# wcy199705/DfFintheWild

Hardware: AMD Instinct MI355X
Metric: focal-stacks/sec (10x3x256x256) (higher is better)
Workload: dtype bf16x3 (split-bf16 MFMA operands hi+lo, fp32 accumulate, fp32-accurate); 1 GPU; DFF_net forward, 10-slice 3x256x256 focal stacks, batch 32 per GPU (BASELINE.json config 3), dense focus_dists, synthetic weights seed 0; batch_per_gpu=32, global_batch=32, slices=10, height=256, width=256, parallelism=single GPU, precision=bf16x3, input=float32 (B,3,N,H,W), the reference's tensor contract

## Files before the change

dffinthewild_amd/csrc/dffw_device.h:

```cpp
#pragma once
#include <hip/hip_runtime.h>
#include <stdint.h>

#include <utility>

#include "dffw_internal.h"

namespace dffw {

template <class F, int... I>
__device__ __forceinline__ void static_for_impl(F &&f, std::integer_sequence<int, I...>) {
    (f(std::integral_constant<int, I>{}), ...);
}
template <int N, class F>
__device__ __forceinline__ void static_for(F &&f) {
    static_for_impl(f, std::make_integer_sequence<int, N>{});
}

typedef __attribute__((ext_vector_type(8))) short short8;
typedef __attribute__((ext_vector_type(4))) short short4v;
typedef __attribute__((ext_vector_type(8))) __bf16 bf16x8;
typedef __attribute__((ext_vector_type(8))) _Float16 f16x8;
typedef __attribute__((ext_vector_type(4))) float f32x4;

// ... 227 lines not shown
        if (a.res0) wide_add(a.res0, pre0);
        if (a.res1) wide_add(a.res1, pre1);
        if (a.relu == 1) {
#pragma unroll
            for (int i = 0; i < 4; ++i) v[i] = relu_bits(v[i]);
        }
        if (a.cls_w && cvalid) {
#pragma unroll
            for (int i = 0; i < 4; ++i) cls_partial = fmaf(a.cls_w[c0 + i], v[i], cls_partial);
        }
        if (a.out) wide_store(a.out);
    } else {
        const bool ok = pvalid && cvalid;
        const int64_t eo = FAST ? (int64_t)(voff + nt * 16) : opix * Cout + c0;
        auto store4 = [&](uint16_t *base_) {
            uint16_t *base = FAST ? base_ + ubase : base_;
            uint32_t h01, h23, l01, l23;
            Fmt<PREC>::split2(v[0], v[1], h01, l01);
            Fmt<PREC>::split2(v[2], v[3], h23, l23);
            if (ok) *reinterpret_cast<uint2 *>(base + eo) = make_uint2(h01, h23);
        };
        auto add4 = [&](const uint16_t *base_, uint4 q) {
            const uint16_t *base = FAST ? base_ + (a.res_bcast ? rbase : ubase) : base_;
            int64_t ro = eo;
            if (a.res_bcast) {
                if constexpr (FAST) ro = (int64_t)(rvoff + nt * 16);
                else {
                    const int64_t hw = (int64_t)a.Ho * a.Wo;
                    ro = ((opix / a.outf_plane) * hw + opix % hw) * Cout + c0;
                }
            }
            if constexpr (!PRE) {
                q = make_uint4(0, 0, 0, 0);
                if (ok) {
                    const uint2 h = *reinterpret_cast<const uint2 *>(base + ro);
                    q.x = h.x;
                    q.y = h.y;
                }
            }
            float r0, r1, r2, r3;
            Fmt<PREC>::join2(q.x, 0, r0, r1);
            Fmt<PREC>::join2(q.y, 0, r2, r3);
            v[0] += r0;
            v[1] += r1;
            v[2] += r2;
            v[3] += r3;
        };
        if (a.out_pre) store4(a.out_pre);
        if (a.relu == 2) {
#pragma unroll
            for (int i = 0; i < 4; ++i) v[i] = relu_bits(v[i]);
        }
        if (a.res0) add4(a.res0, pre0);
        if (a.res1) add4(a.res1, pre1);
        if (a.relu == 1) {
#pragma unroll
            for (int i = 0; i < 4; ++i) v[i] = relu_bits(v[i]);
        }
        if (a.cls_w && cvalid) {
#pragma unroll
            for (int i = 0; i < 4; ++i) cls_partial = fmaf(a.cls_w[c0 + i], v[i], cls_partial);
        }
        if (a.out) store4(a.out);
    }
}

__device__ __forceinline__ void dffw_store16(char *p, uint4 v) { *reinterpret_cast<uint4 *>(p) = v; }

template <int PREC, bool RES, bool CLS = false>
__device__ __forceinline__ float epilogue_lean(uint16_t *__restrict__ out, uint16_t *__restrict__ out_pre, int voff, const f32x4 &acc, uint4 rq,
                                               bool relu, const f32x4 &clsw) {
    static_assert(Fmt<PREC>::PARTS == 2, "split-bf16 storage only");
    float v0 = acc[0], v1 = acc[1], v2 = acc[2], v3 = acc[3];
    auto store = [&](uint16_t *base) {
        uint32_t h01, h23, l01, l23;
        Fmt<PREC>::split2(v0, v1, h01, l01);
        Fmt<PREC>::split2(v2, v3, h23, l23);
        swap16(h01, l01);
        swap16(h23, l23);
        dffw_store16(reinterpret_cast<char *>(base) + (uint32_t)(voff * 2), make_uint4(h01, h23, l01, l23));
    };
    if (out_pre) store(out_pre);
    if constexpr (RES) {
        swap16(rq.x, rq.z);
        swap16(rq.y, rq.w);
        float r0, r1, r2, r3;
        Fmt<PREC>::join2(rq.x, rq.z, r0, r1);
        Fmt<PREC>::join2(rq.y, rq.w, r2, r3);
        v0 += r0;
        v1 += r1;
        v2 += r2;
        v3 += r3;
    }
    if (relu) {
        v0 = relu_bits(v0);
        v1 = relu_bits(v1);
        v2 = relu_bits(v2);
        v3 = relu_bits(v3);
    }
    float cls = 0.f;
    if constexpr (CLS) {
        cls = fmaf(clsw[0], v0, cls);
        cls = fmaf(clsw[1], v1, cls);
        cls = fmaf(clsw[2], v2, cls);
        cls = fmaf(clsw[3], v3, cls);
    }
    if (out) store(out);
    return cls;
}

template <int PREC>
__device__ __forceinline__ void epilogue_lean_t(uint16_t *__restrict__ out, uint16_t *__restrict__ out_pre, int voff, float v0, float v1, float v2,
                                                float v3, bool has_res, uint4 rq, bool relu, bool has_cls, const f32x4 &clsw, float &cls, bool pv) {
    static_assert(Fmt<PREC>::PARTS == 2, "split-bf16 storage only");
    auto store = [&](uint16_t *base) {
        uint32_t h01, h23, l01, l23;
        Fmt<PREC>::split2(v0, v1, h01, l01);
        Fmt<PREC>::split2(v2, v3, h23, l23);
        swap16(h01, l01);
        swap16(h23, l23);
        if (pv) dffw_store16(reinterpret_cast<char *>(base) + (uint32_t)(voff * 2), make_uint4(h01, h23, l01, l23));
    };
    if (out_pre) store(out_pre);
    if (has_res) {
        swap16(rq.x, rq.z);
        swap16(rq.y, rq.w);
        float r0, r1, r2, r3;
        Fmt<PREC>::join2(rq.x, rq.z, r0, r1);
        Fmt<PREC>::join2(rq.y, rq.w, r2, r3);
        v0 += r0;
        v1 += r1;
        v2 += r2;
        v3 += r3;
    }
    if (relu) {
        v0 = relu_bits(v0);
        v1 = relu_bits(v1);
        v2 = relu_bits(v2);
        v3 = relu_bits(v3);
    }
    if (has_cls) {
        cls = fmaf(clsw[0], v0, cls);
        cls = fmaf(clsw[1], v1, cls);
        cls = fmaf(clsw[2], v2, cls);
        cls = fmaf(clsw[3], v3, cls);
    }
    if (out) store(out);
}

__device__ __forceinline__ void epilogue_cls(const ConvArgs &a, float partial, int g, int64_t opix, bool pvalid, int rows = 4) {
    if (!a.cls_w) return;
    partial += __shfl_xor(partial, 16);
    if (rows == 4) partial += __shfl_xor(partial, 32);
    if ((g & (rows - 1)) == 0 && pvalid) a.cls_out[opix] = partial;
}

__device__ __forceinline__ float softplus_fast(float v) {
    const float L2E = 1.44269502162933349609375f, L2E_LO = 1.925963033500414e-08f, LN2 = 0.693147182464599609375f;
    const float hi = v * L2E;
    const float lo = __builtin_fmaf(v, L2E, -hi) + v * L2E_LO;
    float e = __builtin_amdgcn_exp2f(hi);
    e = __builtin_fmaf(e, lo * LN2, e);
    const float w = 1.f + e, d = w - 1.f;
    const float r = (__builtin_amdgcn_logf(w) * LN2) * (e * __builtin_amdgcn_rcpf(d));
    const float sp = d == 0.f ? e : r;
    return v > 20.f ? v : sp;
}

__device__ __forceinline__ float sigmoid_fast(float v) {
    const float L2E = 1.44269502162933349609375f, L2E_LO = 1.925963033500414e-08f, LN2 = 0.693147182464599609375f;
    const float hi = v * L2E;
    const float lo = __builtin_fmaf(v, L2E, -hi) + v * L2E_LO;
    float e = __builtin_amdgcn_exp2f(hi);
    e = __builtin_fmaf(e, lo * LN2, e);
    return v > 20.f ? 1.f : e * __builtin_amdgcn_rcpf(1.f + e);
}

struct WarpPoint {
    float fx, fy, sx, sy;
};
__device__ __forceinline__ WarpPoint warp_point(int xx, int yy, int H, int W, float f, float a1, float a2) {
    const float stepx = 2.0f / (float)(W > 1 ? W - 1 : 1), stepy = 2.0f / (float)(H > 1 ? H - 1 : 1);
    const float lx = xx < W / 2 ? -1.0f + (float)xx * stepx : 1.0f - (float)(W - 1 - xx) * stepx;
    const float ly = yy < H / 2 ? -1.0f + (float)yy * stepy : 1.0f - (float)(H - 1 - yy) * stepy;
    WarpPoint p;
    p.fx = (float)(W / 2) * (f - 1.0f) * lx + a1;
    p.fy = (float)(H / 2) * (f - 1.0f) * ly + a2;
    const float gx = 2.0f * ((float)xx - p.fx) / (float)(W > 1 ? W - 1 : 1) - 1.0f;
    const float gy = 2.0f * ((float)yy - p.fy) / (float)(H > 1 ? H - 1 : 1) - 1.0f;
    p.sx = ((gx + 1.0f) * 0.5f) * (float)(W - 1);
    p.sy = ((gy + 1.0f) * 0.5f) * (float)(H - 1);
    return p;
}


struct SimWarpPoint {
    float sx, sy;
};
__device__ __forceinline__ SimWarpPoint sim_warp_point(int xx, int yy, int H, int W, float fm1, float beta, float gamma) {
#pragma clang fp contract(off)
    const float stepx = 2.0f / (float)(W - 1), stepy = 2.0f / (float)(H - 1);
    const float lx = xx < W / 2 ? fmaf(stepx, (float)xx, -1.0f) : fmaf(-stepx, (float)(W - 1 - xx), 1.0f);
    const float ly = yy < H / 2 ? fmaf(stepy, (float)yy, -1.0f) : fmaf(-stepy, (float)(H - 1 - yy), 1.0f);
    const float g2x = (float)(W / 2) * (fm1 * lx) - beta;
    const float g2y = (float)(H / 2) * (fm1 * ly) - gamma;
    const float gx = 2.0f * ((float)xx - g2x) / (float)(W - 1) - 1.0f;
    const float gy = 2.0f * ((float)yy - g2y) / (float)(H - 1) - 1.0f;
    SimWarpPoint p;
    p.sx = (gx + 1.0f) * ((float)(W - 1) / 2.0f);
    p.sy = (gy + 1.0f) * ((float)(H - 1) / 2.0f);
    return p;
}


template <int PREC>
__device__ __forceinline__ void warp_octet(const uint16_t *__restrict__ slice, int C, int H, int W, const WarpPoint &wp, float (&v)[8]) {
    constexpr int PARTS = Fmt<PREC>::PARTS;
    const float x0f = floorf(wp.sx), y0f = floorf(wp.sy);
    const int x0 = (int)x0f, y0 = (int)y0f;
    const float wx1 = wp.sx - x0f, wy1 = wp.sy - y0f;
    const float wx[2] = {1.0f - wx1, wx1}, wy[2] = {1.0f - wy1, wy1};
#pragma unroll
    for (int dy = 0; dy < 2; ++dy) {
        const int yc = y0 + dy;
        if (yc < 0 || yc >= H) continue;
#pragma unroll
        for (int dx = 0; dx < 2; ++dx) {
            const int xc = x0 + dx;
            if (xc < 0 || xc >= W) continue;
            const uint16_t *rec = slice + ((int64_t)yc * W + xc) * (PARTS * C);
            const uint4 h = *reinterpret_cast<const uint4 *>(rec);
            uint4 l = make_uint4(0, 0, 0, 0);
            if constexpr (PARTS == 2) l = *reinterpret_cast<const uint4 *>(rec + C);
            const float wgt = wx[dx] * wy[dy];
            float a, c;
            Fmt<PREC>::join2(h.x, l.x, a, c); v[0] += a * wgt; v[1] += c * wgt;
            Fmt<PREC>::join2(h.y, l.y, a, c); v[2] += a * wgt; v[3] += c * wgt;
            Fmt<PREC>::join2(h.z, l.z, a, c); v[4] += a * wgt; v[5] += c * wgt;
            Fmt<PREC>::join2(h.w, l.w, a, c); v[6] += a * wgt; v[7] += c * wgt;
        }
    }
}

}
```

dffinthewild_amd/csrc/dffw_dispatch.cpp:

```cpp
#include "dffw_run.h"
#include "dffw_stem.h"

namespace dffw {
namespace {

struct ConvLaunch {
    char kernel[96];
    const char *suffix;
    ConvArgs a;
    RollArgs r;
    int v0, v1;
    double flops, bytes;
};

enum { F_TILE = 100, F_GATHER = 101 };

struct ConvPlan {
    int family = -1;
    int n = 0;
    ConvLaunch l[4];
    bool clear_scores = false;
    const TileCfg *cfg = nullptr;
    TileArgs t;
    bool stem_pipe = false;
    int64_t partial_bytes = 0;
    int64_t M_out = 0;
    double finish_bytes = 0;
    int err = DFFW_OK;
    char msg[192];
};

struct Cols {
    int tiles_y, tiles_x;
    int64_t n;
    bool whole;
};

struct Planner;
struct StreamFamily {
    bool (Planner::*plan)(ConvPlan &p) const;
    void (*name)(int prec, const ConvLaunch &l, char *buf, int n);
    hipError_t (*go)(int prec, const ConvLaunch &l, hipStream_t s);
    bool step_trace;
};
extern const StreamFamily kStream[];
constexpr int kStreamBeforeStemPair = 5, kStreamCount = 10;

struct Planner {
    const std::string &name;
    const PackedConv &pc;
    const LayerDef &L;
    const Act &in0;
    const ConvOpt &o;
    const Switches &sw;
    const int prec;
    const Act &out;
    ConvArgs a;
    const int No, Ho, Wo, cin_pad;
    const double eb, opx, in_b;
    int fam = 0;

    double out_b(int k) const { return opx * L.cout * eb * k; }
    double w_b(double taps) const { return taps * L.cin * L.cout * eb; }
    double cls_b() const { return o.cls ? opx * 4.0 : 0.0; }
    double sums_b() const { return opx / 16.0 * 3.0 * L.cout * 4.0; }
    double mac(double points, double taps) const { return 2.0 * points * taps * L.cin * L.cout; }
    int res(const Act *r) const { return r ? 1 : 0; }

    Cols columns(bool in_grid, int ty, int tx) const {
        const int H = in_grid ? in0.H : Ho, W = in_grid ? in0.W : Wo;
        Cols g;
        g.tiles_y = (H + ty - 1) / ty;
        g.tiles_x = (W + tx - 1) / tx;
        g.n = (int64_t)g.tiles_y * g.tiles_x;
        g.whole = H % ty == 0 && W % tx == 0;
        return g;
    }
    ConvArgs on_grid(bool in_grid) const {
        ConvArgs g = a;
        g.Ng = in_grid ? in0.N : No;
        g.Hg = in_grid ? in0.H : Ho;
        g.Wg = in_grid ? in0.W : Wo;
        g.M = (int64_t)g.B * g.Ng * g.Hg * g.Wg;
        return g;
    }
    static ConvArgs masked(ConvArgs g) {
        g.dbg &= (6 | DFFW_ARGS_NO_LEAN_TILE | DFFW_ARGS_NO_LEAN_ROLL | DFFW_ARGS_NO_ROLLX | DFFW_ARGS_NO_ROLLK | DFFW_ARGS_NO_SLICE32);
        return g;
    }
    int zsplit(int64_t units, int64_t below) const {
        int z = (units < below && No >= 8) ? 2 : 1;
        if (sw.roll_zsplit >= 1 && sw.roll_zsplit <= No) z = sw.roll_zsplit;
        return z;
    }
    void add(ConvPlan &p, const ConvArgs &g, const uint16_t *filter, const Cols &c, int zs, int pair, double flops, double bytes,
             const char *suffix = "", int v0 = 0, int v1 = 0) const {
        p.family = fam;
        ConvLaunch &l = p.l[p.n++];
        l.a = g;
        l.r = roll_args(filter, in0.B, c.tiles_y, c.tiles_x, zs, sw.roll_wgs, pair);
        l.suffix = suffix;
        l.v0 = v0;
        l.v1 = v1;
        l.flops = flops;
        l.bytes = bytes;
        kStream[fam].name(prec, l, l.kernel, sizeof l.kernel);
    }

    bool rollt(ConvPlan &p) const {
        if (!(pc.wrollt && !o.in1 && !sw.on(SW_NO_ROLL) && !sw.on(SW_NO_ROLLT))) return false;
        int ty, tx;
        rollt_tile(L.cout, &ty, &tx);
        const Cols c = columns(true, ty, tx);
        const ConvArgs g = on_grid(true);
        const int64_t units = (int64_t)in0.B * c.n * std::max(1, L.cout / 32);
        const bool four = cin_pad == 32 && L.cout != 16;
        if (!(units >= (int64_t)sw.rollt_min_units * (four ? 3 : 2) / 2 && rollt_ok(prec, g))) return false;
        p.clear_scores = g.cls_w != nullptr;
        add(p, g, pc.wrollt, c, 1, 0, mac((double)g.M, 27.0),
            in_b + out_b((o.discard ? 0 : 1) + (o.out_pre ? 1 : 0) + res(o.res0)) + cls_b() + w_b(27.0));
        return true;
    }
    bool roll_t32(ConvPlan &p) const {
        if (!(pc.wroll_t32 && (in0.C == 32 || in0.C == 16) && !o.in1 && !o.res_bcast && !o.res1 && !o.outf && in0.H % 8 == 0 && in0.W % 16 == 0 &&
              (int64_t)in0.B * (in0.H / 8) * (in0.W / 16) >= sw.roll_min_units && !sw.on(SW_NO_ROLL)))
            return false;
        const ConvArgs g = masked(on_grid(true));
        for (int py = 0; py < 2; ++py) {
            int ty, tx;
            roll_t32_tile(py, &ty, &tx);
            const Cols c = columns(true, ty, tx);
            add(p, g, pc.wroll_t32 + (size_t)(py ? ROLL_CHUNKS_T32_0 : 0) * prec_parts(prec) * 512, c, 1, 0, mac((double)g.M, py ? 18.0 : 9.0),
                in_b + 0.5 * out_b((o.discard ? 0 : 1) + (o.out_pre ? 1 : 0) + res(o.res0)) + 0.5 * cls_b(), py ? " (odd rows)" : " (even rows)", py);
        }
        return true;
    }
    bool roll_s2(ConvPlan &p) const {
        if (!(pc.wroll_s2 && !L.transposed && L.sh == 2 && (in0.C == 16 || in0.C == 32) && !o.in1 && !o.res1 && !o.res_bcast && !o.outf && !o.out_pre &&
              !o.cls && !sw.on(SW_NO_ROLL) && !sw.on(SW_NO_ROLL_S2) &&
              (L.cout <= 32 || !sw.on(SW_NO_ROLL_S2_WIDE))))
            return false;
        const int khn = in0.C / 16;
        const int ntk = (khn == 2 || L.cout >= 32) ? 2 : 1;
        const int nlaunch = (L.cout / 16 + ntk - 1) / ntk;
        int ty, tx;
        s2_roll_tile(ntk, &ty, &tx);
        const Cols c = columns(false, ty, tx);
        if (!((L.cout / 16) % ntk == 0 && c.whole && in0.H == 2 * Ho && in0.W == 2 * Wo && (int64_t)in0.B * c.n >= sw.roll_min_units)) return false;
        const ConvArgs g = masked(on_grid(false));
        for (int li = 0; li < nlaunch; ++li)
            add(p, g, pc.wroll_s2, c, 1, li * ntk, mac(opx, 27.0) / nlaunch, in_b + out_b(1 + res(o.res0)) / nlaunch + w_b(27.0) / nlaunch,
                nlaunch > 1 ? (li ? " (upper output channels)" : " (lower output channels)") : "", ntk, khn);
        return true;
    }
    bool roll_efd(ConvPlan &p) const {
        int ty, tx;
        efd_roll_tile(&ty, &tx);
        const Cols c = columns(false, ty, tx);
        if (!(pc.wroll8 && !L.transposed && L.sh == 2 && in0.C == 8 && !o.in1 && !o.res0 && !o.res1 && !o.res_bcast && !o.outf && !o.out_pre &&
              !o.cls && c.whole && (int64_t)in0.B * c.n >= sw.roll_min_units && !sw.on(SW_NO_ROLL) && !sw.on(SW_NO_ROLL_S2)))
            return false;
        add(p, masked(on_grid(false)), pc.wroll8, c, 1, 0, mac(opx, 27.0), in_b + out_b(1) + w_b(27.0));
        return true;
    }
    bool roll_t(ConvPlan &p) const {
        int ty, tx;
        roll_tile(&ty, &tx);
        const Cols c = columns(true, ty, tx);
        if (!(pc.wroll_t && c.whole && in0.C == 16 && !o.in1 && !o.res_bcast && !o.res1 && !o.outf &&
              (int64_t)in0.B * c.n >= sw.roll_min_units && !sw.on(SW_NO_ROLL)))
            return false;
        const ConvArgs g = on_grid(true);
        add(p, g, pc.wroll_t, c, zsplit((int64_t)in0.B * c.n, 1024), 1, mac((double)g.M, 27.0),
            in_b + out_b((o.discard ? 0 : 1) + (o.out_pre ? 1 : 0)) + out_b(res(o.res0)) + cls_b() + w_b(27.0));
        return true;
    }
    bool rollx_k2(ConvPlan &p) const {
        const Cols c = columns(false, 8, 16);
        const bool halves = o.in1 ? (in0.C == 16 && o.in1->C == 16) : in0.C == 32;
        if (!(pc.wroll_k2 && halves && c.whole && (int64_t)in0.B * c.n >= sw.roll_min_units && !sw.on(SW_NO_ROLL) && !sw.on(SW_NO_ROLLX))) return false;
        const ConvArgs g = on_grid(false);
        if (!rollx_k2_ok(prec, g)) return false;
        add(p, g, pc.wroll_k2, c, zsplit((int64_t)in0.B * c.n, 512), 0, mac(opx, 27.0), in_b + out_b(1) + w_b(27.0));
        return true;
    }
    bool slice32(ConvPlan &p) const {
        if (!(pc.wslice32 && !o.in1 && !sw.on(SW_NO_ROLL) && !sw.on(SW_NO_SLICE32))) return false;
        int ty, tx;
        slice32_tile(&ty, &tx);
        const Cols c = columns(false, ty, tx);
        const ConvArgs g = on_grid(false);
        if (!(c.whole && (int64_t)in0.B * c.n >= sw.roll_min_units && slice32_ok(prec, g))) return false;
        add(p, g, pc.wslice32, c, 1, 0, mac(opx, 9.0), in_b + (o.sums ? sums_b() : out_b(1 + res(o.res0))) + w_b(9.0));
        return true;
    }
    bool slice64(ConvPlan &p) const {
        if (!(pc.wslice64 && (pc.slice_cat ? (o.in1 && o.in1->C == 32) : !o.in1) && !sw.on(SW_NO_ROLL) && !sw.on(SW_NO_SLICE32))) return false;
        int ty, tx;
        slice32_tile(&ty, &tx);
        const Cols c = columns(false, ty, tx);
        const ConvArgs g = on_grid(false);
        if (!(c.whole && (int64_t)in0.B * c.n >= sw.roll_min_units && slice64_ok(prec, g))) return false;
        add(p, g, pc.wslice64, c, 1, 0, mac(opx, 9.0), in_b + (o.sums ? sums_b() : out_b(1)) + w_b(9.0));
        return true;
    }
    bool rollk(ConvPlan &p) const {
        if (!(pc.wrollk && !sw.on(SW_NO_ROLL) && !sw.on(SW_NO_ROLLK))) return false;
        int ty, tx;
        rollk_tile(&ty, &tx);
        const Cols c = columns(false, ty, tx);
        const ConvArgs g = on_grid(false);
        const int npair = L.cout / 32;
        const bool merged = npair == 2 && (int64_t)in0.B * c.n < sw.rollk_merge_below;
        const int64_t units = (int64_t)in0.B * c.n * (merged ? npair : 1);
        if (!(units >= sw.roll_min_units && rollk_waves(prec, g) == cin_pad / 8)) return false;
        const int nlaunch = merged ? 1 : npair;
        for (int op = 0; op < nlaunch; ++op)
            add(p, g, pc.wrollk + (size_t)op * (cin_pad / 8) * ROLLK_CHUNKS * 2 * prec_parts(prec) * 512, c, zsplit(units, cin_pad == 64 && merged ? 256 : 512),
                merged ? -1 : op * 2, mac(opx, 27.0) / nlaunch, in_b + out_b(1 + res(o.res0)) / nlaunch + w_b(27.0) / nlaunch,
                nlaunch > 1 ? (op ? " (upper output channels)" : " (lower output channels)") : "");
        return true;
    }
    bool roll(ConvPlan &p) const {
        int ty, tx;
        roll_tile(&ty, &tx);
        const Cols c = columns(false, ty, tx);
        if (!(pc.wroll && c.whole && in0.C % 8 == 0 && (!o.in1 || o.in1->C == in0.C) && !o.res_bcast && !o.res1 &&
              (int64_t)in0.B * c.n >= sw.roll_min_units && !sw.on(SW_NO_ROLL)))
            return false;
        add(p, on_grid(false), pc.wroll, c, zsplit((int64_t)in0.B * c.n, 1024), pc.roll_pair ? 1 : 0, mac(opx, 27.0),
            in_b + (o.outf ? opx * L.cout * 4.0 : out_b(o.out_pre ? 2 : 1)) + out_b(res(o.res0) + res(o.res1)) + w_b(27.0), "", pc.roll_pair);
        return true;
    }

    void tile(ConvPlan &p, const TilePack &tp, bool stem_pair, int gH, int gW);
    void gather(ConvPlan &p);
};

const StreamFamily kStream[kStreamCount] = {
    {&Planner::rollt, [](int, const ConvLaunch &l, char *b, int n) { conv_rollt_kernel_name(l.a, b, n); },
     [](int, const ConvLaunch &l, hipStream_t s) { return launch_conv_rollt(l.a, l.r, s); }, false},
    {&Planner::roll_t32, [](int prec, const ConvLaunch &l, char *b, int n) { conv_roll_t32_kernel_name(prec, l.v0, l.a, b, n); },
     [](int prec, const ConvLaunch &l, hipStream_t s) { return launch_conv_roll_t32(prec, l.v0, l.a, l.r, s); }, false},
    {&Planner::roll_s2, [](int prec, const ConvLaunch &l, char *b, int n) { conv_roll_s2_kernel_name(prec, l.v0, l.v1, l.a, b, n); },
     [](int prec, const ConvLaunch &l, hipStream_t s) { return launch_conv_roll_s2(prec, l.v0, l.v1, l.a, l.r, s); }, false},
    {&Planner::roll_efd, [](int prec, const ConvLaunch &l, char *b, int n) { conv_roll_efd_kernel_name(prec, l.a, false, b, n); },
     [](int prec, const ConvLaunch &l, hipStream_t s) { return launch_conv_roll_efd(prec, l.a, l.r, s); }, false},
    {&Planner::roll_t, [](int prec, const ConvLaunch &l, char *b, int n) { conv_roll_t_kernel_name(prec, l.a, b, n); },
     [](int prec, const ConvLaunch &l, hipStream_t s) { return launch_conv_roll_t(prec, l.a, l.r, s); }, false},
    {&Planner::rollx_k2, [](int, const ConvLaunch &l, char *b, int n) { conv_rollx_k2_kernel_name(l.a, b, n); },
     [](int, const ConvLaunch &l, hipStream_t s) { return launch_conv_rollx_k2(l.a, l.r, s); }, false},
    {&Planner::slice32, [](int, const ConvLaunch &l, char *b, int n) { conv_slice32_kernel_name(l.a, b, n); },
     [](int, const ConvLaunch &l, hipStream_t s) { return launch_conv_slice32(l.a, l.r, s); }, false},
    {&Planner::slice64, [](int, const ConvLaunch &l, char *b, int n) { conv_slice64_kernel_name(l.a, b, n); },
     [](int, const ConvLaunch &l, hipStream_t s) { return launch_conv_slice64(l.a, l.r, s); }, false},
    {&Planner::rollk, [](int, const ConvLaunch &l, char *b, int n) { conv_rollk_kernel_name(l.a, b, n); },
     [](int, const ConvLaunch &l, hipStream_t s) { return launch_conv_rollk(l.a, l.r, s); }, false},
    {&Planner::roll, [](int prec, const ConvLaunch &l, char *b, int n) { conv_roll_kernel_name(prec, l.a, l.v0 != 0, b, n); },
     [](int prec, const ConvLaunch &l, hipStream_t s) { return launch_conv_roll(prec, l.a, l.r, s); }, true},
};

void Planner::tile(ConvPlan &p, const TilePack &tp, bool stem_pair, int gH, int gW) {
    const TileCfg *cfg = tp.cfg;
    a.Ng = L.transposed ? in0.N : No;
    a.Hg = gH;
    a.Wg = gW;
    a.sy = a.sx = L.transposed ? 1 : L.sh;
    a.osy = a.osx = L.transposed ? 2 : 1;
    a.M = (int64_t)a.B * a.Ng * a.Hg * a.Wg;
    TileArgs &t = p.t;
    memset(&t, 0, sizeof t);
    t.npass = tp.npass;
    t.nstage = tp.nstage;
    double flops = 0;
    for (int ps = 0; ps < tp.npass; ++ps) {
        t.KC[ps] = tp.KC[ps];
        t.tab[ps] = tp.tab[ps];
        t.wpk[ps] = tp.wpk[ps];
        t.ooy[ps] = tp.ooy[ps];
        t.oox[ps] = tp.oox[ps];
        flops += 2.0 * (double)a.M * (L.transposed ? tp.ntaps[ps] : L.kd * L.kh * L.kw) * L.cin * L.cout;
    }
    t.nt_total = pc.nt;
    t.nsplit = pc.nt / cfg->nt;
    auto set_tiles = [&](const TileCfg *c) {
        t.tiles_z = (a.Ng + c->tz - 1) / c->tz;
        t.tiles_y = (a.Hg + c->ty - 1) / c->ty;
        t.tiles_x = (a.Wg + c->tx - 1) / c->tx;
        t.total_tiles = a.B * t.tiles_z * t.tiles_y * t.tiles_x;
        t.grid = 8 * ((t.total_tiles + 7) / 8);
        t.warm = (t.total_tiles * t.nsplit <= sw.warm_max_wgs) ? 1 : 0;
    };
    auto team_wgs = [&](const TileCfg *c, int nsplit, int npass) {
        return (int64_t)a.B * ((a.Ng + c->tz - 1) / c->tz) * ((a.Hg + c->ty - 1) / c->ty) * ((a.Wg + c->tx - 1) / c->tx) * nsplit * npass;
    };
    set_tiles(cfg);
    const int split_below = (cfg->geo == G3T && pc.nt >= 4) ? sw.split_t64 : (cfg->geo == G3S1 && pc.nt == 4) || (cfg->geo == G3S2 && pc.nt >= 8) ? sw.split_s64 : ((cfg->geo == G3S1 || cfg->geo == G3T) ? 257 : 256);
    if (t.total_tiles < split_below && pc.nt > 1 && !o.cls && !sw.on(SW_NO_SPLIT)) {
        const int want = (256 + t.total_tiles - 1) / t.total_tiles;
        for (int nts = pc.nt / 2; nts >= 1; nts /= 2) {
            const TileCfg *c2 = pc.nt % nts == 0 ? tile_cfg_find_like(tp.cfg, nts) : nullptr;
            if (!c2) continue;
            cfg = c2;
            t.nsplit = pc.nt / nts;
            if (t.nsplit >= want) break;
        }
        set_tiles(cfg);
    }
    t.ksplit = 1;
    p.M_out = (int64_t)out.B * No * Ho * Wo;
    const int thr = sw.split_wg;
    t.pass_split = (L.transposed && t.total_tiles * t.nsplit <= thr && !sw.on(SW_NO_SPLITK)) ? 1 : 0;
    if (t.pass_split && tp.nstage >= 2 && !sw.on(SW_NO_TEAMS)) {
        for (int nts = cfg->nt; nts <= pc.nt && nts <= 2; nts *= 2) {
            const TileCfg *team = pc.nt % nts == 0 ? tile_cfg_find_team(cfg, tp.nstage, nts) : nullptr;
            if (!team || team_wgs(team, pc.nt / nts, 4) > sw.team_max_wgs) continue;
            cfg = team;
            t.nsplit = pc.nt / nts;
            set_tiles(cfg);
            break;
        }
    }
    if (!t.pass_split && tile_cfg_has_splitk(cfg) && t.total_tiles * t.nsplit <= thr * 3 / 4 && tp.nstage >= 2 && !o.cls && !o.out_pre && !o.outf && !o.discard && !o.res_bcast && L.cout % 4 == 0 &&
        !sw.on(SW_NO_SPLITK)) {
        const int want = (sw.ksplit_target + t.total_tiles * t.nsplit - 1) / (t.total_tiles * t.nsplit);
        t.ksplit = std::max(1, std::min(std::min(tp.nstage, want), 8));
        const TileCfg *team = (t.ksplit > 1 && !sw.on(SW_NO_TEAMS)) ? tile_cfg_find_team(cfg, tp.nstage, cfg->nt) : nullptr;
        if (team) {
            const int64_t wgs = team_wgs(team, t.nsplit, 1);
            if (wgs < sw.team_min_wgs || wgs > sw.team_max_wgs) team = nullptr;
        }
        if (team) {
            cfg = team;
            t.ksplit = 1;
            set_tiles(cfg);
        }
        if (t.ksplit > 1) {
            t.partial_stride = p.M_out * (int64_t)pc.nt * 16;
            p.partial_bytes = t.ksplit * t.partial_stride * (int64_t)sizeof(float);
            p.finish_bytes = (double)p.M_out * L.cout * (4.0 * t.ksplit + eb * (o.res0 ? 2 : 1));
        }
    }
    p.stem_pipe = stem_pair && !sw.on(SW_NO_STEM_PIPE) && !sw.tracing(name) && stem_pipe_ok(prec, cfg, a, t);
    p.family = F_TILE;
    p.cfg = cfg;
    p.n = 1;
    ConvLaunch &l = p.l[0];
    l.a = a;
    l.suffix = "";
    l.flops = flops;
    l.bytes = in_b + (o.outf ? opx * L.cout * 4.0 : out_b(o.out_pre ? 2 : 1)) + out_b(res(o.res0) + res(o.res1)) + w_b((double)L.kd * L.kh * L.kw);
    if (p.stem_pipe) stem_pipe_kernel_name(a, l.kernel, sizeof l.kernel);
    else conv_tile_kernel_name(prec, cfg, a, t, l.kernel, sizeof l.kernel);
}

void Planner::gather(ConvPlan &p) {
    p.family = F_GATHER;
    for (const Variant &v : pc.variants) {
        a.KC = v.KC;
        a.tab = v.tab;
        a.wpk = v.wpk;
        if (L.transposed) {
            a.Ng = in0.N; a.Hg = in0.H; a.Wg = in0.W;
            a.sy = a.sx = 1;
            a.osy = a.osx = 2;
            a.ooy = v.ooy; a.oox = v.oox;
        } else {
            a.Ng = No; a.Hg = Ho; a.Wg = Wo;
            a.sy = L.sh; a.sx = L.sw;
            a.osy = a.osx = 1;
            a.ooy = a.oox = 0;
        }
        a.M = (int64_t)a.B * a.Ng * a.Hg * a.Wg;
        if (sw.on(SW_NO_SMALL)) a.dbg |= DFFW_ARGS_NO_SMALL;
        ConvLaunch &l = p.l[p.n++];
        l.a = a;
        l.suffix = "";
        conv_kernel_name_for(prec, a, l.kernel, 64);
        const double nv = (double)pc.variants.size();
        const double px = (double)a.M;
        l.flops = 2.0 * (double)a.M * v.ntaps * L.cin * L.cout;
        l.bytes = in_b / nv
                  + px * L.cout * (o.outf ? 4.0 : eb * (o.out_pre ? 2 : 1))
                  + px * L.cout * eb * (res(o.res0) + res(o.res1))
                  + (double)v.ntaps * L.cin * L.cout * eb;
    }
}

void plan_conv(const std::string &name, const PackedConv &pc, const PackedConv *cls, const Act &in0, const ConvOpt &o, const Act &out, const Switches &sw,
               int prec, ConvPlan &p) {
    const LayerDef &L = pc.def;
    const int No = out.N, Ho = out.H, Wo = out.W;
    auto reject = [&](const char *fmt, const char *x, const char *y) {
        p.err = DFFW_EINVAL;
        snprintf(p.msg, sizeof p.msg, fmt, x, y);
    };
    if (o.cls && (!cls || !cls->w32 || cls->def.cin != L.cout || cls->def.cout != 1)) return reject("cannot fuse classifier %s into %s", o.cls, name.c_str());
    if (o.res_bcast && !(L.kd == 1 && L.kh == 3 && !L.transposed && L.sh == 1 && L.cout >= 16))
        return reject("slice-broadcast residual is only implemented for the per-slice 1x3x3 convs (layer %s)%s", name.c_str(), "");

    const double eb = 2.0 * prec_parts(prec);
    Planner pl{name, pc, L, in0, o, sw, prec, out, ConvArgs(), No, Ho, Wo, pc.cin_all, eb, (double)out.B * No * Ho * Wo, (double)in0.pixels() * L.cin * eb};
    ConvArgs &a = pl.a;
    memset(&a, 0, sizeof a);
    a.in0 = in0.p;
    a.C0 = in0.C;
    a.in1 = o.in1 ? o.in1->p : in0.p;
    a.C1 = o.in1 ? o.in1->C : 0;
    a.B = in0.B; a.Ni = in0.N; a.Hi = in0.H; a.Wi = in0.W;
    a.No = No; a.Ho = Ho; a.Wo = Wo;
    a.Cout = L.cout;
    a.bias = pc.bias;
    a.res0 = o.res0 ? o.res0->p : nullptr;
    a.res1 = o.res1 ? o.res1->p : nullptr;
    a.res_bcast = o.res_bcast ? 1 : 0;
    a.out = out.p;
    a.out_pre = o.out_pre ? o.out_pre->p : nullptr;
    a.outf = o.outf;
    a.fs32 = o.fs32;
    a.outf_ch = o.outf_ch;
    a.outf_plane = (int64_t)No * Ho * Wo;
    a.cls_w = cls ? cls->w32 : nullptr;
    a.cls_out = o.cls_out;
    a.relu = o.relu;
    a.dbg = (sw.debug_flags & 6) | sw.path_bits();
    if (o.raw) a.dbg |= DFFW_ARGS_RAW;
    if (o.sums) {
        if (!conv_sums_ok(pc, sw, in0.B, in0.N, in0.H, in0.W) || o.relu != 1 || o.res0 || o.res1 || o.cls || o.out_pre || o.in1)
            return reject("layer %s has no row-sums kernel for this shape / epilogue%s", name.c_str(), "");
        a.outf = o.sums;
        a.dbg |= DFFW_ARGS_SUMS;
    }

    for (pl.fam = 0; pl.fam < kStreamBeforeStemPair; ++pl.fam)
        if ((pl.*kStream[pl.fam].plan)(p)) return;
    const bool stem_pair = o.fs32 && pc.tile_pair.cfg && pc.bias_pair && Wo % pc.tile_pair.cfg->tx == 0 && Ho % pc.tile_pair.cfg->ty == 0 &&
                           !sw.on(SW_NO_STEM_PAIR);
    if (stem_pair) a.bias = pc.bias_pair;
    for (; pl.fam < kStreamCount; ++pl.fam)
        if ((pl.*kStream[pl.fam].plan)(p)) return;

    const int gW = L.transposed ? in0.W : Wo, gH = L.transposed ? in0.H : Ho;
    const bool narrow_splits = pc.tile_narrow.cfg && pc.nt > pc.tile_narrow.cfg->nt;
    const int gN = L.transposed ? in0.N : No;
    bool narrow = !stem_pair && pc.tile_narrow.cfg && !sw.on(SW_NO_NARROW) && !(narrow_splits && (o.cls || sw.on(SW_NO_SPLIT))) &&
                  (int64_t)in0.B * ((gN + 4) / 5) * ((gH + 7) / 8) * ((gW + 7) / 8) * pc.nt >= 256;
    if (narrow && !(gW <= 8 && gH <= 8)) narrow = !L.transposed && pc.nt >= 8 && gW <= sw.narrow_max && gH <= sw.narrow_max;
    const TilePack &tp = stem_pair ? pc.tile_pair : (narrow ? pc.tile_narrow : pc.tile);
    const int64_t small_units = ((int64_t)in0.B * gN * gH * gW + 15) / 16 * pc.nt;
    const bool prefer_small = small_units <= sw.small_max_units && !o.cls && !o.fs32 && !sw.on(SW_NO_SMALL) && !stem_pair;
    const bool use_tile = tp.cfg && !sw.on(SW_NO_TILE) && gW * 2 >= tp.cfg->tx && gH * 2 >= tp.cfg->ty &&
                          in0.C % 8 == 0 && (!o.in1 || o.in1->C % 8 == 0) && !prefer_small;
    if (use_tile) pl.tile(p, tp, stem_pair, gH, gW);
    else pl.gather(p);
}

}

Act Run::conv(const std::string &name, const Act &in0, const ConvOpt &o) {
    Act out;
    if (!ok()) return out;
    auto it = e->convs.find(name);
    if (it == e->convs.end()) {
        err = fail(DFFW_EINVAL, "no packed layer %s", name.c_str());
        return out;
    }
    const PackedConv &pc = it->second;
    const LayerDef &L = pc.def;
    const int cin = in0.C + (o.in1 ? o.in1->C : 0);
    if (cin != pc.cin_all) {
        err = fail(DFFW_EINVAL, "layer %s expects %d input channels, got %d", name.c_str(), pc.cin_all, cin);
        return out;
    }
    int Ho, Wo;
    if (L.transposed) {
        Ho = in0.H * 2;
        Wo = in0.W * 2;
    } else {
        const int win = (L.kh == 9 && L.cin == 3) ? in0.W - 2 : in0.W;
        Ho = (in0.H + 2 * L.ph - L.dh * (L.kh - 1) - 1) / L.sh + 1;
        Wo = (win + 2 * L.pw - L.dw * (L.kw - 1) - 1) / L.sw + 1;
    }
    const int No = in0.N + 2 * L.pd - (L.kd - 1);
    if (o.outf == nullptr && !o.discard && !o.sums) out = act(in0.B, No, Ho, Wo, L.cout);
    else { out.B = in0.B; out.N = No; out.H = Ho; out.W = Wo; out.C = L.cout; }
    if (o.out_pre) *o.out_pre = act(in0.B, No, Ho, Wo, L.cout);
    if (!ok()) return out;

    const PackedConv *cls = nullptr;
    if (o.cls) {
        auto ic = e->convs.find(o.cls);
        if (ic != e->convs.end()) cls = &ic->second;
    }
    ConvPlan p;
    plan_conv(name, pc, cls, in0, o, out, sw, e->prec, p);
    if (p.err != DFFW_OK) {
        err = fail(p.err, "%s", p.msg);
        return out;
    }
    float *partial = p.partial_bytes ? (float *)raw(p.partial_bytes) : nullptr;
    if (!ok()) return out;
    if (dry) {
        drop_raw(partial);
        return out;
    }

    const uint16_t *zero = zero_page();
    if (!zero) return out;
    if (p.clear_scores) check(hipMemsetAsync(o.cls_out, 0, (size_t)out.pixels() * 4, s), "score memset");
    const StreamFamily *f = p.family < kStreamCount ? &kStream[p.family] : nullptr;
    const size_t trace_words = p.family == F_TILE ? (size_t)p.t.total_tiles * 8 : (f && f->step_trace) ? STEP_TRACE_WORDS : 0;
    p.t.partial = partial;
    for (int i = 0; i < p.n; ++i) {
        ConvLaunch &l = p.l[i];
        l.a.zero = zero;
        launch(l.kernel, name, l.suffix, l.flops, l.bytes, name.c_str(), trace_words, [&](unsigned long long *trace) {
            l.a.trace = trace;
            if (f) return f->go(e->prec, l, s);
            if (p.family == F_GATHER) return launch_conv(e->prec, l.a, s);
            return p.stem_pipe ? launch_stem_pipe(l.a, p.t, sw.roll_wgs, s) : launch_conv_tile(e->prec, p.cfg, l.a, p.t, s);
        });
    }
    if (partial) {
        launch_unnamed("dffw::splitk_finish_kernel", name, " (split-K finish)", 0.0, p.finish_bytes, "splitk_finish", 0, [&](unsigned long long *) {
#if defined(DFFW_ABL_BUILD) && defined(DFFW_EXP_SKIP_FINISH)
            return hipSuccess;
#endif
            return launch_splitk_finish(e->prec, partial, p.t.ksplit, p.t.partial_stride, p.M_out, pc.nt * 16, L.cout, pc.bias, p.l[0].a.res0, o.relu, out.p, s);
        });
        drop_raw(partial);
    }
    trace_end();
    return out;
}

}
```

dffinthewild_amd/csrc/dffw_engine.cpp:

```cpp
#include <algorithm>
#include <cmath>
#include <cstdarg>
#include <cstdio>
#include <cstdlib>
#include <cstring>
#include <map>
#include <memory>
#include <string>
#include <vector>

#include "dffw_run.h"
#include "dffw_srd_roll.h"
#include "dffw_stem.h"

namespace dffw {

static thread_local std::string g_err;
static thread_local std::string g_last_kernel;
static thread_local std::string g_last_op_kernels;
}
int dffw_fail(int code, const char *fmt, ...) {
    char buf[1024];
    va_list ap;
    va_start(ap, fmt);
// ... 275 lines not shown
    };
    auto args = [&](int cout, uint16_t *out) {
        ConvArgs a;
        memset(&a, 0, sizeof a);
        a.in0 = x.p; a.C0 = x.C;
        a.in1 = pooled->p; a.C1 = x.C;
        a.B = x.B; a.Ni = x.N; a.Hi = x.H; a.Wi = x.W;
        a.Ng = x.N; a.Hg = Ho; a.Wg = Wo;
        a.No = x.N; a.Ho = Ho; a.Wo = Wo;
        a.Cout = cout;
        a.bias = ca->second.bias;
        a.out = out;
        a.relu = 1;
        a.M = (int64_t)x.B * x.N * Ho * Wo;
        return a;
    };
    int ty, tx;
    efd_roll_tile(&ty, &tx);
    if (fused(8, ty, tx) && ca->second.wroll8 && cb->second.wroll8) {
        Act out = r.act(x.B, x.N, Ho, Wo, 16);
        if (r.ok() && !r.dry) {
            ConvArgs a = args(16, out.p);
            if (!(a.zero = r.zero_page())) return out;
            a.dbg = (r.sw.debug_flags & 6) | r.sw.path_bits();
            RollArgs t = roll_args(ca->second.wroll8, x.B, Ho / ty, Wo / tx, 1, r.sw.roll_wgs);
            t.wroll2 = cb->second.wroll8;
            t.bias2 = cb->second.bias;
            char kn[64];
            conv_roll_efd_kernel_name(r.e->prec, a, true, kn, sizeof kn);
            r.launch(kn, p, "", 2.0 * opx * 27.0 * 8 * 16 * 2, ((double)x.pixels() * 8 + opx * 8 + opx * 16) * r.elem_bytes(), "conv_roll_efd", 0,
                     [&](unsigned long long *) { return launch_conv_roll_efd(r.e->prec, a, t, r.s); });
        }
        r.drop(*pooled);
        return out;
    }
    efd16_tile(&ty, &tx);
    if (fused(16, ty, tx) && ca->second.wroll_s2 && cb->second.wroll15 && ca->second.def.cout == 32) {
        ConvArgs a = args(32, (uint16_t *)16);
        RollArgs t = roll_args(ca->second.wroll_s2, x.B, Ho / ty, Wo / tx, 1, r.sw.roll_wgs);
        t.wroll2 = cb->second.wroll15;
        t.bias2 = cb->second.bias;
        if (efd16_ok(r.e->prec, a, t)) {
            Act out = r.act(x.B, x.N, Ho, Wo, 32);
            if (r.ok() && !r.dry) {
                a.out = out.p;
                char kn[64];
                conv_efd16_kernel_name(kn, sizeof kn);
                r.launch(kn, p, "", 2.0 * opx * 27.0 * 16 * 32 * 2, ((double)x.pixels() * 16 + opx * 16 + opx * 32) * r.elem_bytes(), "conv_efd16", 0,
                         [&](unsigned long long *) { return launch_conv_efd16(a, t, r.s); });
            }
            r.drop(*pooled);
            return out;
        }
    }
    Act a = r.conv(p + ".stride_conv.0", x);
    Act m = (pooled && pooled->p) ? *pooled : r.pool(x, 0, 2);
    ConvOpt o; o.relu = 1; o.res0 = &a;
    Act out = r.conv(p + ".max_pooling.1.0", m, o);
    r.drop(m);
    r.drop(a);
    return out;
}

static Act pyramid_scale(Run &r, const std::string &S, const char *tag, Act &t) {
    const std::string d = S + ".dres" + tag;
    ConvOpt rl; rl.relu = 1;
    Act a = r.conv(d + "_0.0.0", t, rl);
    Act r0 = r.conv(d + "_0.2.0", a, rl);
    r.drop(a);
    Act b = r.conv(d + "_1.0.0", r0, rl);
    ConvOpt o; o.res0 = &r0;
    Act out = r.conv(d + "_1.2.0", b, o);
    r.drop(b);
    r.drop(r0);
    return out;
}

static Act pyramid(Run &r, const std::string &S, const Act &v3) {
    ConvOpt rl; rl.relu = 1;
    Act p8, p16, p32;
    if (v3.H % 8 == 0 && v3.W % 8 == 0 && !r.sw.on(SW_NO_POOL3)) {
        p8 = r.act(v3.B, v3.N, v3.H / 2, v3.W / 2, v3.C);
        p16 = r.act(v3.B, v3.N, v3.H / 4, v3.W / 4, v3.C);
        p32 = r.act(v3.B, v3.N, v3.H / 8, v3.W / 8, v3.C);
        if (r.ok() && !r.dry) {
            char kn[48];
            snprintf(kn, sizeof kn, "dffw::pool3_kernel<%d>", r.e->prec);
            r.launch_unnamed(kn, "avgpool (1,2,2)+(1,4,4)+(1,8,8)", "", 0.0, (double)(v3.pixels() + p8.pixels() + p16.pixels() + p32.pixels()) * v3.C * r.elem_bytes(), "pool3", 0,
                             [&](unsigned long long *) { return launch_pool3(r.e->prec, v3.p, p8.p, p16.p, p32.p, v3.B, v3.N, v3.H, v3.W, v3.C, r.s); });
        }
    } else {
        p8 = r.pool(v3, 1, 2);
        p16 = r.pool(v3, 1, 4);
        p32 = r.pool(v3, 1, 8);
    }
    r.forked = r.concurrent;
    r.fork(0);
    r.fork(1);
    Act s8 = pyramid_scale(r, S, "8", p8);
    r.drop(p8);
    r.on(0);
    Act s16 = pyramid_scale(r, S, "16", p16);
    r.drop(p16);
    r.on(1);
    Act s32 = pyramid_scale(r, S, "32", p32);
    r.drop(p32);
    r.on(-1);
    r.join(0);
    r.join(1);
    r.forked = false;
    r.release_deferred();
    const bool redir_side = r.concurrent && (r.sw.redir_side == 1 || (r.sw.redir_side < 0 && (int64_t)v3.B * v3.N * v3.H * v3.W * 16 >= (2 << 20)));
    r.forked = redir_side;
    if (redir_side) {
        r.fork(0);
        r.on(0);
    }
    Act rd1 = r.conv(S + ".redir1.0", s8);
    r.on(-1);
    Act d1 = r.conv(S + ".conv1", s8);
    r.drop(s8);
    ConvOpt c1 = rl; c1.in1 = &s16;
    Act m1 = r.conv(S + ".combine1.0.0", d1, c1);
    r.drop(d1); r.drop(s16);
    Act c2 = r.conv(S + ".conv2.0.0", m1, rl);
    r.drop(m1);
    if (redir_side) {
        r.fork(1);
        r.on(1);
    }
    Act rd2 = r.conv(S + ".redir2.0", c2);
    r.on(-1);
    Act d2 = r.conv(S + ".conv3", c2);
    r.drop(c2);
    ConvOpt cc2 = rl; cc2.in1 = &s32;
    Act m2 = r.conv(S + ".combine2.0.0", d2, cc2);
    r.drop(d2); r.drop(s32);
    Act c4 = r.conv(S + ".conv4.0.0", m2, rl);
    r.drop(m2);
    if (redir_side) r.join(1);
    ConvOpt u8o = rl; u8o.res0 = &rd2;
    Act u8 = r.conv(S + ".conv8.0", c4, u8o);
    r.drop(c4); r.drop(rd2);
    if (redir_side) r.join(0);
    ConvOpt u9o = rl; u9o.res0 = &rd1;
    Act u9 = r.conv(S + ".conv9.0", u8, u9o);
    r.drop(u8); r.drop(rd1);
    r.forked = false;
    r.release_deferred();
    return u9;
}

static Act hourglass(Run &r, const std::string &p, const Act &xa, const Act &xb, const Act *presqu, const Act *postsqu,
                     const Act &skip, Act *pre1_out, Act *out_raw, const std::string &cls, float *cls_out, bool discard_sum) {
    ConvOpt rl; rl.relu = 1;
    ConvOpt c0 = rl; c0.in1 = &xb;
    Act pre1 = r.conv(p + ".conv0.0.0", xa, c0);
    Act o1 = r.conv(p + ".conv1.0.0", pre1, rl);
    ConvOpt c2 = rl; c2.res0 = postsqu;
    Act pre = r.conv(p + ".conv2.0", o1, c2);
    r.drop(o1);
    Act o3 = r.conv(p + ".conv3.0.0", pre, rl);
    Act o4 = r.conv(p + ".conv4.0.0", o3, rl);
    r.drop(o3);
    ConvOpt c5 = rl; c5.res0 = presqu ? presqu : &pre;
    Act o5 = r.conv(p + ".conv5.0", o4, c5);
    r.drop(o4); r.drop(pre);
    ConvOpt c6; c6.res0 = &skip; c6.out_pre = out_raw; c6.cls = cls.c_str(); c6.cls_out = cls_out; c6.discard = discard_sum;
    Act sum = r.conv(p + ".conv6.0", o5, c6);
    r.drop(o5);
    if (pre1_out) *pre1_out = pre1; else r.drop(pre1);
    return sum;
}

struct RegressQueue {
    RegressHeads hd{};
    void *keep[4] = {nullptr, nullptr, nullptr, nullptr};
    int nkeep = 0;
    double bytes = 0.0;
};
static void regress(Run &r, RegressQueue &q, const char *tag, float *score, int B, int N, int h, int w, int H, int W, const float *fd,
                    const int64_t fst[4], float *out, bool merge) {
    if (!merge) {
        if (r.ok() && !r.dry && out)
            r.launch_unnamed("dffw::regress_kernel", tag, "", 0.0, (double)B * N * h * w * 4.0 + (double)B * H * W * 4.0, tag, 0,
                             [&](unsigned long long *) { return launch_regress(score, B, N, h, w, H, W, fd, fst[0], fst[1], fst[2], fst[3], out, r.s); });
        r.drop_raw(score);
        return;
    }
    q.keep[q.nkeep++] = score;
    if (!out || r.dry) return;
    const int k = q.hd.n++;
    q.hd.score[k] = score;
    q.hd.depth[k] = out;
    q.hd.h[k] = h;
    q.hd.w[k] = w;
    q.bytes += (double)B * N * h * w * 4.0 + (double)B * H * W * 4.0;
}
static void flush_regress(Run &r, RegressQueue &q, int B, int N, int H, int W, const float *fd, const int64_t fst[4]) {
    if (q.hd.n && r.ok() && !r.dry) {
        q.hd.nofuse = r.sw.on(SW_NO_REGRESS_FUSED) ? 1 : 0;
        const bool fused = regress_form(q.hd, B, N, H, W) != 0;
        const double bytes = q.bytes + ((fst[2] || fst[3]) ? (double)B * N * H * W * 4.0 : 0.0);
        r.launch_unnamed(fused ? "dffw::regress_fused_kernel" : "dffw::regress_kernel", "regress.mid_out+pred1+pred2+pred3", "", 0.0, bytes, "regress", 0,
                         [&](unsigned long long *) { return launch_regress_heads(q.hd, B, N, H, W, fd, fst[0], fst[1], fst[2], fst[3], r.s); });
    }
    for (int k = 0; k < q.nkeep; ++k) r.drop_raw(q.keep[k]);
    q.hd.n = 0;
    q.nkeep = 0;
}

int run_depth(Run &r, const float *FS, const float *fd, const int64_t fst[4], int B, int N, int H, int W, float *const out[4], const RawStack *raw) {
    const std::string P = "DFF_net";
    const int prec = r.e->prec;
    ConvOpt rl; rl.relu = 1;
    {
        const int64_t z = r.sw.concurrent_max_pixels;
        const int64_t px = (int64_t)B * N * H * W;
        if ((z < 0 || px < z) && px >= r.sw.concurrent_min_pixels && !r.sw.on(SW_NO_CONCURRENT) && !r.e->profiling) r.enable_concurrency();
    }

    const std::string stem_name = P + ".FM_measure.Focus_extraction.0.0";
    Act stem;
    if (r.tiled(stem_name, H, W) && !r.sw.on(SW_NO_FUSED_STEM)) {
        Act geom;
        geom.B = B; geom.N = N; geom.H = H; geom.W = W + 2; geom.C = 8;
        ConvOpt so = rl;
        so.fs32 = FS;
        RawStack *rdev = nullptr;
        if (raw) {
            rdev = (RawStack *)r.raw(256);
            if (r.ok() && !r.dry) r.check(launch_set_raw(*raw, rdev, r.s), "set_raw");
            so.fs32 = (const float *)rdev;
            so.raw = true;
        }
        stem = r.conv(stem_name, geom, so);
        r.drop_raw(rdev);
    } else {
        float *tmp = nullptr;
        if (raw) {
            tmp = (float *)r.raw((int64_t)B * 3 * N * H * W * (int64_t)sizeof(float));
            if (r.ok() && !r.dry) {
                const int64_t st[5] = {raw->sb, raw->sn, raw->sy, raw->sx, raw->sc};
                if (dffw_pack_stack(r.e->device, raw->p, raw->dtype, st, B, N, raw->h, raw->w, H, W, tmp, r.s) != DFFW_OK) r.err = DFFW_EHIP;
            }
            FS = tmp;
        }
        Act in = r.act(B, N, H, W + 2, 8);
        if (r.ok() && !r.dry) {
            char kn[48];
            snprintf(kn, sizeof kn, "dffw::stack_in_kernel<%d>", prec);
            r.launch_unnamed(kn, "stack_in", "", 0.0, (double)B * N * H * W * 3 * 4.0 + (double)B * N * H * (W + 2) * 8 * r.elem_bytes(), "stack_in", 0,
                             [&](unsigned long long *) { return launch_stack_in(prec, FS, in.p, B, N, H, W, r.s); });
        }
        stem = r.conv(stem_name, in, rl);
        r.drop(in);
        r.drop_raw(tmp);
    }
    r.tap("stem", stem);
    Act v1p, v2p;
    Act v1 = srd(r, P + ".FM_measure.Focus_extraction.2", stem, true, &v1p);
    r.tap("V1", v1);
    Act e1 = efd(r, P + ".FM_conv1.0", v1, &v1p);
    r.tap("E1", e1);
    Act v2 = srd(r, P + ".FM_conv1.1", e1, true, &v2p);
    r.tap("V2", v2);
    Act e2 = efd(r, P + ".FM_conv2.0", v2, &v2p);
    r.tap("E2", e2);
    Act v3 = srd(r, P + ".FM_conv2.1", e2, true);
    r.tap("V3", v3);

    Act vol = pyramid(r, P + ".SPP_module", v3);
    r.tap("FS_volume", vol);

    RegressQueue rq;
    const bool merge_heads = true;
    const int h8 = H / 8, w8 = W / 8;
    float *conf = (float *)r.raw((int64_t)B * N * h8 * w8 * sizeof(float));
    const bool conf_side = r.concurrent && (int64_t)B * N * H * W < (16 << 20) && !r.sw.on(SW_NO_CONF_FORK);
    r.forked = conf_side;
    if (conf_side) {
        r.fork(0);
        r.on(0);
    }
    {
        Act c = r.conv(P + ".confidence.0.0", vol, rl);
        ConvOpt of; of.outf = conf;
        r.conv(P + ".confidence.2", c, of);
        r.drop(c);
        r.tap_f32("conf", conf, (int64_t)B * N * h8 * w8);
        regress(r, rq, "regress.mid_out", conf, B, N, h8, w8, H, W, fd, fst, out[0], merge_heads);
    }
    r.on(-1);

    Act d0 = r.conv(P + ".dres0.0.0", vol, rl);
    r.drop(vol);
    Act d1 = r.conv(P + ".dres0.2.0", d0, rl);
    r.drop(d0);
    Act x1 = r.conv(P + ".deconv_1.0", d1);
    r.drop(d1);
    if (conf_side) r.join(0);
    r.forked = false;
    r.release_deferred();

    Act pre_a, out_a;
    const int h4 = H / 4, w4 = W / 4;
    float *cost1 = (float *)r.raw((int64_t)B * N * h4 * w4 * sizeof(float));
    Act s1 = hourglass(r, P + ".dres2", x1, v3, nullptr, nullptr, x1, &pre_a, &out_a, P + ".classif1.0", cost1, false);
    r.drop(x1); r.drop(v3);
    r.tap_f32("cost1", cost1, (int64_t)B * N * h4 * w4);
    regress(r, rq, "regress.pred1", cost1, B, N, h4, w4, H, W, fd, fst, out[1], merge_heads);

    Act x2 = r.conv(P + ".deconv_2.0", s1);
    r.drop(s1);
    Act pre_b, out_b;
    const int h2 = H / 2, w2 = W / 2;
    float *cost2 = (float *)r.raw((int64_t)B * N * h2 * w2 * sizeof(float));
    Act s2 = hourglass(r, P + ".dres3", x2, v2, &pre_a, &out_a, x2, &pre_b, &out_b, P + ".classif2.0", cost2, false);
    r.drop(x2); r.drop(v2); r.drop(pre_a); r.drop(out_a);
    r.tap_f32("cost2", cost2, (int64_t)B * N * h2 * w2);
    regress(r, rq, "regress.pred2", cost2, B, N, h2, w2, H, W, fd, fst, out[2], merge_heads);

    Act x3 = r.conv(P + ".deconv_3.0", s2);
    r.drop(s2);
    float *cost3 = (float *)r.raw((int64_t)B * N * H * W * sizeof(float));
    Act s3 = hourglass(r, P + ".dres4", x3, v1, &pre_b, &out_b, x3, nullptr, nullptr, P + ".classif3.0", cost3, true);
    r.drop(x3); r.drop(v1); r.drop(pre_b); r.drop(out_b);
    r.drop(s3);
    r.tap_f32("cost3", cost3, (int64_t)B * N * H * W);
    regress(r, rq, "regress.pred3", cost3, B, N, H, W, H, W, fd, fst, out[3], merge_heads);
    flush_regress(r, rq, B, N, H, W, fd, fst);
    return r.err;
}

static int check_dims(int B, int N, int H, int W) {
    if (B < 1 || N < 1) return fail(DFFW_EINVAL, "B and N must be >= 1 (got B=%d N=%d)", B, N);
    if (H < 32 || W < 32 || H % 32 || W % 32)
        return fail(DFFW_EINVAL, "H and W must be positive multiples of 32 (got %dx%d); pad with -1 as the reference loaders do", H, W);
    return DFFW_OK;
}

}

extern "C" {

const char *dffw_version(void) { return "dffw 0.1 (gfx950)"; }
const char *dffw_last_error(void) { return g_err.c_str(); }
const char *dffw_last_conv_kernel(void) { return g_last_kernel.c_str(); }

int dffw_param_count(int net) {
    if (!known_net(net)) return fail(DFFW_EINVAL, "unknown net %d", net);
    return (int)table_for(net).params.size();
}

int dffw_param_info(int net, int index, const char **name, int64_t shape[5], int *ndim, int *flags) {
    if (!known_net(net)) return fail(DFFW_EINVAL, "unknown net %d", net);
    const Table &t = table_for(net);
    if (index < 0 || index >= (int)t.params.size()) return fail(DFFW_EINVAL, "param index %d out of range", index);
    const ParamInfo &p = t.params[index];
    if (name) *name = p.name.c_str();
    if (shape) memcpy(shape, p.shape, sizeof p.shape);
    if (ndim) *ndim = p.ndim;
    if (flags) *flags = p.flags;
    return DFFW_OK;
}

int dffw_engine_create(int device, int net, const dffw_tensor *tensors, int n_tensors, int precision, dffw_engine **out) {
    if (!out) return fail(DFFW_EINVAL, "out is null");
    *out = nullptr;
    if (!known_net(net)) return fail(DFFW_EINVAL, "unknown net %d", net);
    if (precision < 0 || precision > 2) return fail(DFFW_EINVAL, "unknown precision %d", precision);
    if (!tensors || n_tensors <= 0) return fail(DFFW_EINVAL, "no tensors given");
    HIPCHK(hipSetDevice(device));
    std::map<std::string, const dffw_tensor *> by;
    for (int i = 0; i < n_tensors; ++i) {
        if (!tensors[i].name) return fail(DFFW_EINVAL, "tensor %d has no name", i);
        std::string nm = tensors[i].name;
        if (nm.rfind("module.", 0) == 0) nm = nm.substr(7);
        by[nm] = &tensors[i];
    }
    auto need = [&](const std::string &nm, int64_t numel, const float **p) -> int {
        auto it = by.find(nm);
        if (it == by.end()) return fail(DFFW_EMISSING, "state dict has no entry '%s'", nm.c_str());
        if (it->second->numel != numel)
            return fail(DFFW_EINVAL, "'%s' has %lld elements, expected %lld", nm.c_str(), (long long)it->second->numel, (long long)numel);
        if (!it->second->data) return fail(DFFW_EINVAL, "'%s' has null data", nm.c_str());
        *p = it->second->data;
        return DFFW_OK;
    };
    std::unique_ptr<dffw_engine> e(new dffw_engine);
    e->device = device;
    e->net = net;
    e->prec = precision;
    const Table &t = table_for(net);
    for (const LayerDef &L : t.layers) {
        if (!L.live) continue;
        const float *w = nullptr, *cb = nullptr, *sw = nullptr;
        int scin = 0;
        if (!L.shortcut.empty()) {
            const LayerDef &S = t.layers[t.by_name.at(L.shortcut)];
            scin = S.cin;
            int rc2 = need(S.conv + ".weight", (int64_t)S.cin * S.cout, &sw);
            if (rc2) return rc2;
        }
        if (L.folded) continue;
        int rc = need(L.conv + ".weight", (int64_t)L.cin * L.cout * L.kd * L.kh * L.kw, &w);
        if (rc) return rc;
        if (L.bias && (rc = need(L.conv + ".bias", L.cout, &cb))) return rc;
        std::vector<float> bn;
        if (!L.bn.empty()) {
            const char *sfx[4] = {".weight", ".bias", ".running_mean", ".running_var"};
            bn.resize(4 * (size_t)L.cout);
            for (int k = 0; k < 4; ++k) {
                const float *p = nullptr;
                if ((rc = need(L.bn + sfx[k], L.cout, &p))) return rc;
                memcpy(bn.data() + (size_t)k * L.cout, p, L.cout * sizeof(float));
            }
        }
        PackedConv &pc = e->convs[L.conv];
        rc = pack_conv(L, precision, w, bn.empty() ? nullptr : bn.data(), cb, pc, sw, scin);
        if (rc) return rc;
        if (L.head_split > 0 && !bn.empty()) {
            const int C = L.head_split, kv = L.kd * L.kh * L.kw;
            auto slice = [&](int c0, int c1) {
                std::vector<float> ws((size_t)L.cout * (c1 - c0) * kv);
                for (int co = 0; co < L.cout; ++co)
                    memcpy(ws.data() + (size_t)co * (c1 - c0) * kv, w + ((size_t)co * L.cin + c0) * kv, (size_t)(c1 - c0) * kv * sizeof(float));
                return ws;
            };
            LayerDef Lr = L, Lc = L;
            Lr.conv = L.conv + "#ref"; Lr.cin = C; Lr.head_split = 0;
            Lc.conv = L.conv + "#cur"; Lc.cin = L.cin - C; Lc.head_split = 0;
            std::vector<float> bn_scale_only = bn;
            for (int c = 0; c < L.cout; ++c) bn_scale_only[L.cout + c] = bn_scale_only[2 * L.cout + c] = 0.f;
            const std::vector<float> wr = slice(0, C), wc = slice(C, L.cin);
            if ((rc = pack_conv(Lr, precision, wr.data(), bn_scale_only.data(), nullptr, e->convs[Lr.conv]))) return rc;
            if ((rc = pack_conv(Lc, precision, wc.data(), bn.data(), nullptr, e->convs[Lc.conv]))) return rc;
        }
    }
    *out = e.release();
    return DFFW_OK;
}

void dffw_engine_destroy(dffw_engine *e) {
    if (!e) return;
    (void)hipSetDevice(e->device);
    delete e;
}

int dffw_engine_precision(const dffw_engine *e) { return e ? e->prec : fail(DFFW_EINVAL, "null engine"); }

int64_t dffw_workspace_bytes(const dffw_engine *e, int B, int N, int H, int W) {
    if (!e) return fail(DFFW_EINVAL, "null engine");
    int rc = check_dims(B, N, H, W);
    if (rc) return rc;
    if (e->net == DFFW_NET_E2E && N != DFFW_E2E_SLICES)
        return fail(DFFW_EINVAL, "the alignment network is built for %d focal slices (End_to_End.py:46), got %d", DFFW_E2E_SLICES, N);
    Run r(const_cast<dffw_engine *>(e), nullptr, true, nullptr, INT64_MAX / 2);
    const int64_t st[4] = {0, 0, 0, 0};
    float *outs[4] = {nullptr, nullptr, nullptr, nullptr};
    rc = e->net == DFFW_NET_E2E ? run_e2e(r, nullptr, nullptr, st, nullptr, B, N, H, W, outs, nullptr)
                                : run_depth(r, nullptr, nullptr, st, B, N, H, W, outs);
    if (rc) return rc;
    return r.arena.peak();
}

int dffw_forward_e2e(dffw_engine *e, const float *FS, const float *focus_dists, const int64_t fd_strides[4], const float *fovs,
                     int B, int N, int H, int W, float *const out[4], float *aligned, void *workspace, int64_t workspace_bytes,
                     void *hip_stream, const dffw_tap *taps, int n_taps) {
    if (!e || !FS || !focus_dists || !fd_strides || !fovs || !out || !aligned) return fail(DFFW_EINVAL, "null argument");
    if (e->net != DFFW_NET_E2E) return fail(DFFW_EINVAL, "engine was not created with DFFW_NET_E2E");
    int rc = check_dims(B, N, H, W);
    if (rc) return rc;
    if (N != DFFW_E2E_SLICES)
        return fail(DFFW_EINVAL, "the alignment network is built for %d focal slices (End_to_End.py:46), got %d", DFFW_E2E_SLICES, N);
    if (!workspace) return fail(DFFW_ENOMEM, "workspace is null");
    HIPCHK(hipSetDevice(e->device));
    if (e->profiling) e->clear_recs();
    Run r(e, (hipStream_t)hip_stream, false, (char *)workspace, workspace_bytes);
// ... 74 lines not shown
```

dffinthewild_amd/csrc/dffw_internal.h:

```cpp
#pragma once
#include <hip/hip_runtime.h>
#include <stdint.h>

int dffw_fail(int code, const char *fmt, ...);
void dffw_set_last_op_kernels(const char *names);

namespace dffw {

struct Act {
    uint16_t *p = nullptr;
    int B = 0, N = 0, H = 0, W = 0, C = 0;
    int64_t pixels() const { return (int64_t)B * N * H * W; }
};

enum Prec { P_BF16X3 = 0, P_FP16 = 1, P_BF16 = 2 };
inline int prec_parts(int prec) { return prec == P_BF16X3 ? 2 : 1; }

struct TapEntry {
    int dz, dy, dx;
    int coff;
};
static_assert(sizeof(TapEntry) == 16, "TapEntry must be 16 bytes");

#define DFFW_TAP_INVALID (1 << 20)

struct RawStack {
    const void *p;
    int dtype;
    int64_t sb, sn, sy, sx, sc;
    int h, w;
};

#define DFFW_RAW_NORM_F64_BIT 16
#define DFFW_ARGS_RAW 8
#define DFFW_ARGS_SUMS 128
#define DFFW_ARGS_NO_SMALL 32
#define DFFW_ARGS_NO_LEAN_TILE 16
#define DFFW_ARGS_NO_LEAN_ROLL 64
#define DFFW_ARGS_NO_ROLLX 256
#define DFFW_ARGS_NO_SLICE32 1024
#define DFFW_ARGS_NO_ROLLT 2048
#define DFFW_ARGS_NO_ROLLK 512
struct ConvArgs {
    const uint16_t *in0, *in1;
    int C0, C1;
    int B, Ni, Hi, Wi;
    int Ng, Hg, Wg;
    int sy, sx;
    int No, Ho, Wo;
    int osy, osx, ooy, oox;
    int Cout, KC;
    const TapEntry *tab;
    const uint16_t *wpk;
    const float *bias;
    const uint16_t *res0, *res1;
    int res_bcast;
    uint16_t *out;
    uint16_t *out_pre;
    float *outf;
    int outf_ch;
    int64_t outf_plane;
    const float *cls_w;
    float *cls_out;
    int relu;
    int dbg;
    const uint16_t *zero;
    const float *fs32;
    unsigned long long *trace;
    int64_t M;
};

int conv_nt_for(int cout);
hipError_t launch_conv(int prec, const ConvArgs &a, hipStream_t s);
void conv_kernel_name_for(int prec, const ConvArgs &a, char *buf, int n);
hipError_t launch_set_raw(const RawStack &rs, RawStack *dst, hipStream_t s);
hipError_t launch_stack_in(int prec, const float *FS, uint16_t *out, int B, int N, int H, int W, hipStream_t s);
hipError_t launch_from_ncdhw(int prec, const float *x, uint16_t *out, int B, int C, int N, int H, int W, hipStream_t s);
hipError_t launch_to_ncdhw(int prec, const uint16_t *x, float *out, int B, int C, int N, int H, int W, hipStream_t s);
hipError_t launch_pool(int prec, int mode, int k, const uint16_t *x, uint16_t *out, int B, int N, int H, int W, int C, hipStream_t s);
hipError_t launch_pool3(int prec, const uint16_t *x, uint16_t *o2, uint16_t *o4, uint16_t *o8, int B, int N, int H, int W, int C, hipStream_t s);
bool srd_attention_supported(int C);
hipError_t launch_srd_attention(int prec, const uint16_t *feat, uint16_t *out, const float *w3, const float *w1, int B, int N,
                                int H, int W, int C, uint16_t *pooled, hipStream_t s);
hipError_t launch_splitk_finish(int prec, const float *partial, int ksplit, int64_t stride, int64_t M, int cpad, int Cout,
                                const float *bias, const uint16_t *res0, int relu, uint16_t *out, hipStream_t s);
hipError_t launch_from_ncdhw_pad(int prec, const float *x, uint16_t *out, int B, int Cs, int C, int N, int H, int W, hipStream_t s);
hipError_t launch_flow_volume(int prec, const uint16_t *fe, uint16_t *out, const float *alpha, const float *fov, int B, int N,
                              int H, int W, int C, int mode, hipStream_t s);
hipError_t launch_alpha_mean(const float *head, float *alpha, float *raw, int B, int N, int64_t hw, hipStream_t s);
int head_tail_chunks(int B, int N, int64_t hw);
hipError_t launch_head_tail_rows(const float *rows, double *seg, int tiles_x, const float *w, float *alpha, float *raw, int B, int N, int H, int W,
                                 int C, hipStream_t s);
int64_t head_tail_tiles_scratch_bytes(int B, int N, int C);
hipError_t launch_head_tail_tiles(const float *tsum, double *seg, int tiles_y, int tiles_x, const float *w, float *alpha, float *raw, int B,
                                  int N, int H, int W, int C, hipStream_t s);
hipError_t launch_head_tail(int prec, const uint16_t *v, double *partial, const float *w, float *alpha, float *raw, int B, int N, int H, int W,
                            int C, hipStream_t s);
hipError_t launch_fov_warp(const float *x, const float *alpha, const float *fov, float *out, float *flow, int B, int C, int N,
                           int H, int W, int alpha_from_sample0, hipStream_t s);
struct RegressHeads {
    const float *score[4];
    float *depth[4];
    int h[4], w[4];
    int n;
    int nofuse;
};
int regress_form(const RegressHeads &hd, int B, int N, int H, int W);
const char *regress_kernel_name(const RegressHeads &hd, int B, int N, int H, int W);
hipError_t launch_regress_heads(const RegressHeads &hd, int B, int N, int H, int W, const float *fd, int64_t fsb, int64_t fsn, int64_t fsh,
                                int64_t fsw, hipStream_t s);
hipError_t launch_regress(const float *score, int B, int N, int h, int w, int H, int W, const float *fd,
                          int64_t fsb, int64_t fsn, int64_t fsh, int64_t fsw, float *depth, hipStream_t s);

}
```

dffinthewild_amd/csrc/dffw_ops.cpp:

```cpp
#include <functional>
#include <string>
#include <vector>

#include "dffw_bn.h"
#include "dffw_conv_pw_wgrad.h"
#include "dffw_conv_wgrad.h"
#include "dffw_pool_grad.h"
#include "dffw_run.h"
#include "dffw_score_grad.h"
#include "dffw_stem_wgrad.h"

using namespace dffw;

namespace {

struct OpEngine : dffw_engine {
    OpEngine(int device_, int prec_) { device = device_; prec = prec_; }
};

struct OpBlock {
    char *p = nullptr;
    hipStream_t s;
    explicit OpBlock(hipStream_t s_) : s(s_) {}
    OpBlock(const OpBlock &) = delete;
    OpBlock &operator=(const OpBlock &) = delete;
    hipError_t alloc(int64_t bytes) { return hipMalloc((void **)&p, bytes); }
    ~OpBlock() {
        if (!p) return;
        (void)hipStreamSynchronize(s);
        (void)hipFree(p);
    }
};

int run_op(dffw_engine &eng, hipStream_t s, bool record, const std::function<void(Run &)> &body) {
    int64_t need;
    {
        Run d(&eng, s, true, nullptr, INT64_MAX / 2);
        body(d);
        if (!d.ok()) return d.err;
        need = d.arena.peak();
    }
    const int64_t bytes = need + 65536;
    OpBlock ws(s);
    HIPCHK(ws.alloc(bytes));
    HIPCHK(hipMemsetAsync(ws.p, 0xFF, bytes, s));
    eng.profiling = record;
    int rc;
    {
        Run r(&eng, s, false, ws.p, bytes);
        body(r);
        rc = r.err;
    }
    const hipError_t se = hipStreamSynchronize(s);
    if (rc == DFFW_OK && se != hipSuccess) rc = fail(DFFW_EHIP, "sync: %s", hipGetErrorString(se));
    if (record) {
        std::string names;
        for (const ProfRec &pr : eng.recs) names += (names.empty() ? "" : ";") + pr.kernel;
        dffw_set_last_op_kernels(names.c_str());
    }
    return rc;
}

bool real(const Run &r) { return r.ok() && !r.dry; }

Act stage_in(Run &r, const float *x, int B, int C, int N, int H, int W) {
    Act a = r.act(B, N, H, W, C);
    if (real(r)) r.check(launch_from_ncdhw(r.e->prec, x, a.p, B, C, N, H, W, r.s), "from_ncdhw");
    return a;
}
void stage_out(Run &r, const Act &a, float *y) {
    if (real(r)) r.check(launch_to_ncdhw(r.e->prec, a.p, y, a.B, a.C, a.N, a.H, a.W, r.s), "to_ncdhw");
}
void copy_out(Run &r, const float *score, float *y, int64_t n) {
    if (real(r)) r.check(hipMemcpyAsync(y, score, n * sizeof(float), hipMemcpyDeviceToDevice, r.s), "copy");
}

std::vector<float> adjoint_filter(const float *weight, int Cout, int Cin, int64_t taps) {
    std::vector<float> wa((size_t)Cin * Cout * taps);
    for (int co = 0; co < Cout; ++co)
        for (int ci = 0; ci < Cin; ++ci)
            for (int64_t t = 0; t < taps; ++t) wa[((size_t)ci * Cout + co) * taps + (taps - 1 - t)] = weight[((size_t)co * Cin + ci) * taps + t];
    return wa;
}

struct Staged {
    const float *t;
    int C, H, W;
};
int run_wgrad_op(int device, int precision, int B, int N, Staged x, Staged gy, int64_t wsb, hipStream_t s,
                 const std::function<int(const void *, const void *, void *, hipStream_t)> &call) {
    HIPCHK(hipSetDevice(device));
    OpEngine eng(device, precision);
    return run_op(eng, s, false, [&](Run &r) {
        Act xa = x.t ? stage_in(r, x.t, B, x.C, N, x.H, x.W) : Act(), ya = gy.t ? stage_in(r, gy.t, B, gy.C, N, gy.H, gy.W) : Act();
        void *ws = r.raw(wsb);
        if (real(r)) r.err = call(xa.p, ya.p, ws, r.s);
    });
}
int run_wgrad_op(int device, int precision, int B, int N, Staged xa, Staged xb, Staged gy, int64_t wsb, hipStream_t s,
                 const std::function<int(const void *, const void *, const void *, void *, hipStream_t)> &call) {
    HIPCHK(hipSetDevice(device));
    OpEngine eng(device, precision);
    return run_op(eng, s, false, [&](Run &r) {
        Act aa = stage_in(r, xa.t, B, xa.C, N, xa.H, xa.W), ba = stage_in(r, xb.t, B, xb.C, N, xb.H, xb.W), ya = stage_in(r, gy.t, B, gy.C, N, gy.H, gy.W);
        void *ws = r.raw(wsb);
        if (real(r)) r.err = call(aa.p, ba.p, ya.p, ws, r.s);
    });
}

}

extern "C" {

int dffw_op_conv3d(int device, int precision, const float *x, int B, int Cin, int N, int H, int W, const float *weight,
                   int Cout, const int kernel[3], const int stride[3], const int pad[3], const int dilation[3], int transposed,
                   const float *bn, const float *conv_bias, const float *residual, int relu, float *y, void *hip_stream) {
    return dffw_op_conv3d_ex(device, precision, x, B, Cin, N, H, W, weight, Cout, kernel, stride, pad, dilation, transposed, bn, conv_bias, residual, relu, y,
                             nullptr, nullptr, nullptr, hip_stream);
}

int dffw_op_conv3d_ex(int device, int precision, const float *x, int B, int Cin, int N, int H, int W, const float *weight,
                      int Cout, const int kernel[3], const int stride[3], const int pad[3], const int dilation[3], int transposed,
                      const float *bn, const float *conv_bias, const float *residual, int relu, float *y, float *y_pre, const float *cls_weight,
                      float *cls_score, void *hip_stream) {
    if (!x || !weight || !y || !kernel || !stride || !pad || !dilation) return fail(DFFW_EINVAL, "null argument");
    if (precision < 0 || precision > 2) return fail(DFFW_EINVAL, "unknown precision %d", precision);
    if (stride[0] != 1 || dilation[0] != 1) return fail(DFFW_EINVAL, "slice stride/dilation must be 1");
    if (stride[1] != stride[2] || dilation[1] != dilation[2]) return fail(DFFW_EINVAL, "row/col stride and dilation must match");
    if (Cout != 1 && Cout % 4) return fail(DFFW_EINVAL, "Cout must be 1 or a multiple of 4");
    if (Cout > 128) return fail(DFFW_EINVAL, "Cout > 128 unsupported");
    HIPCHK(hipSetDevice(device));
    LayerDef L{"op", "", Cin, Cout, kernel[0], kernel[1], kernel[2], stride[1], stride[2], pad[0], pad[1], pad[2],
               dilation[1], dilation[2], transposed != 0, true, false};
    if (transposed && !(kernel[0] == 3 && kernel[1] == 3 && kernel[2] == 3 && stride[1] == 2 && pad[0] == 1 && pad[1] == 1 && pad[2] == 1))
        return fail(DFFW_EINVAL, "transposed conv supports only k3 s(1,2,2) p1 op(0,1,1)");
    OpEngine eng(device, precision);
    int rc = pack_conv(L, precision, weight, bn, conv_bias, eng.convs["op"]);
    if (rc) return rc;
    if ((cls_weight != nullptr) != (cls_score != nullptr)) return fail(DFFW_EINVAL, "cls_weight and cls_score go together");
    if ((y_pre || cls_weight) && (Cout == 1 || Cout % 8)) return fail(DFFW_EINVAL, "second output / fused classifier need Cout %% 8 == 0");
    if (cls_weight) {
        LayerDef C{"cls", "", Cout, 1, 1, 1, 1, 1, 1, 0, 0, 0, 1, 1, false, true, false};
        rc = pack_conv(C, precision, cls_weight, nullptr, nullptr, eng.convs["cls"]);
        if (rc) return rc;
    }
    const int cpad = (Cin + 7) / 8 * 8;
    const bool stem = (!transposed && kernel[0] == 1 && kernel[1] == 9 && kernel[2] == 9 && dilation[1] == 2 && pad[0] == 0 && pad[1] == 8 &&
                       stride[1] == 1 && Cin == 3);
    return run_op(eng, (hipStream_t)hip_stream, false, [&](Run &r) {
        Act in = r.act(B, N, H, stem ? W + 2 : W, cpad);
        const int64_t plane = (int64_t)N * H * W;
        float *xp = !stem && cpad != Cin ? (float *)r.raw(B * cpad * plane * (int64_t)sizeof(float)) : nullptr;
        if (real(r)) {
            if (stem || xp) r.check(hipMemsetAsync(in.p, 0, (size_t)in.pixels() * prec_parts(precision) * cpad * 2, r.s), "input memset");
            if (stem) {
                r.check(launch_stack_in(precision, x, in.p, B, N, H, W, r.s), "stack_in");
            } else if (!xp) {
                r.check(launch_from_ncdhw(precision, x, in.p, B, Cin, N, H, W, r.s), "from_ncdhw");
            } else {
                r.check(hipMemsetAsync(xp, 0, (size_t)B * cpad * plane * sizeof(float), r.s), "input memset");
                for (int b = 0; b < B && r.ok(); ++b)
                    r.check(hipMemcpyAsync(xp + (int64_t)b * cpad * plane, x + (int64_t)b * Cin * plane, (size_t)Cin * plane * sizeof(float),
                                           hipMemcpyDeviceToDevice, r.s), "copy");
                if (r.ok()) r.check(launch_from_ncdhw(precision, xp, in.p, B, cpad, N, H, W, r.s), "from_ncdhw");
            }
        }
        const int No = N + 2 * pad[0] - (kernel[0] - 1);
        const int Ho = transposed ? 2 * H : (H + 2 * pad[1] - dilation[1] * (kernel[1] - 1) - 1) / stride[1] + 1;
        const int Wo = transposed ? 2 * W : (W + 2 * pad[2] - dilation[2] * (kernel[2] - 1) - 1) / stride[2] + 1;
        const int64_t opix = (int64_t)B * No * Ho * Wo;
        ConvOpt o;
        o.relu = relu;
        Act res, pre;
        if (Cout == 1) {
            o.outf = (float *)r.raw(opix * sizeof(float));
        } else if (residual) {
            res = stage_in(r, residual, B, Cout, No, Ho, Wo);
            o.res0 = &res;
        }
        if (y_pre) o.out_pre = &pre;
        if (cls_weight) {
            o.cls = "cls";
            o.cls_out = (float *)r.raw(opix * sizeof(float));
        }
        Act out = r.conv("op", in, o);
        if (Cout == 1) copy_out(r, o.outf, y, opix);
        else stage_out(r, out, y);
        if (y_pre) stage_out(r, pre, y_pre);
        if (cls_weight) copy_out(r, o.cls_out, cls_score, opix);
    });
}

int dffw_op_pool(int device, int precision, int mode, int k, const float *x, int B, int C, int N, int H, int W, float *y,
                 void *hip_stream) {
    if (!x || !y) return fail(DFFW_EINVAL, "null argument");
    if (precision < 0 || precision > 2) return fail(DFFW_EINVAL, "unknown precision %d", precision);
    if (C % 8 || k < 1 || H % k || W % k) return fail(DFFW_EINVAL, "pool needs C %% 8 == 0 and H,W divisible by k");
    HIPCHK(hipSetDevice(device));
    OpEngine eng(device, precision);
    return run_op(eng, (hipStream_t)hip_stream, false, [&](Run &r) {
        Act in = stage_in(r, x, B, C, N, H, W);
        stage_out(r, r.pool(in, mode, k), y);
    });
}

int dffw_op_srd(int device, int precision, const float *x, int B, int C, int N, int H, int W, const float *w0, const float *bn0,
                const float *w2, const float *bn2, const float *w3, const float *w1, float *y, float *pooled, void *hip_stream) {
    dffw_set_last_op_kernels("");
    if (!x || !w0 || !bn0 || !w2 || !bn2 || !w3 || !w1 || !y) return fail(DFFW_EINVAL, "null argument");
    if (precision < 0 || precision > 2) return fail(DFFW_EINVAL, "unknown precision %d", precision);
    if (C != 8 && C != 16 && C != 32) return fail(DFFW_EINVAL, "the SRD blocks have 8, 16 or 32 channels, got %d", C);
    if (B < 1 || N < 1 || H < 1 || W < 1) return fail(DFFW_EINVAL, "bad shape");
    if (pooled && (H % 2 || W % 2)) return fail(DFFW_EINVAL, "the pooled copy needs even H and W, got %dx%d", H, W);
    HIPCHK(hipSetDevice(device));
    const std::string p = C == 8 ? "DFF_net.FM_measure.Focus_extraction.2" : C == 16 ? "DFF_net.FM_conv1.1" : "DFF_net.FM_conv2.1";
    const std::vector<LayerDef> layers = srd_layers(p, C);
    const float *const wts[4] = {w0, w2, w3, w1}, *const bns[4] = {bn0, bn2, nullptr, nullptr};
    OpEngine eng(device, precision);
    for (int i = 0; i < 4; ++i) {
        const int rc = pack_conv(layers[i], precision, wts[i], bns[i], nullptr, eng.convs[layers[i].conv]);
        if (rc) return rc;
    }
    return run_op(eng, (hipStream_t)hip_stream, true, [&](Run &r) {
        Act in = stage_in(r, x, B, C, N, H, W);
        Act pl;
        Act out = srd(r, p, in, true, pooled ? &pl : nullptr);
        if (pooled && !pl.p) pl = r.pool(out, 0, 2);
        stage_out(r, out, y);
        if (pooled) stage_out(r, pl, pooled);
    });
}

int dffw_op_efd(int device, int precision, const float *x, int B, int Cin, int N, int H, int W, const float *ws, const float *bns,
                const float *wp, const float *bnp, int pooled_at_hand, float *y, void *hip_stream) {
    dffw_set_last_op_kernels("");
    if (!x || !ws || !bns || !wp || !bnp || !y) return fail(DFFW_EINVAL, "null argument");
    if (precision < 0 || precision > 2) return fail(DFFW_EINVAL, "unknown precision %d", precision);
    if (Cin != 8 && Cin != 16) return fail(DFFW_EINVAL, "the EFD blocks have 8 or 16 input channels, got %d", Cin);
    if (B < 1 || N < 1 || H < 2 || W < 2 || H % 2 || W % 2) return fail(DFFW_EINVAL, "bad shape (H and W must be even)");
    HIPCHK(hipSetDevice(device));
    const std::string p = Cin == 8 ? "DFF_net.FM_conv1.0" : "DFF_net.FM_conv2.0";
    const std::vector<LayerDef> layers = efd_layers(p, Cin, 2 * Cin);
    const float *const wts[2] = {ws, wp}, *const bnv[2] = {bns, bnp};
    OpEngine eng(device, precision);
    for (int i = 0; i < 2; ++i) {
        const int rc = pack_conv(layers[i], precision, wts[i], bnv[i], nullptr, eng.convs[layers[i].conv]);
        if (rc) return rc;
    }
    return run_op(eng, (hipStream_t)hip_stream, true, [&](Run &r) {
        Act in = stage_in(r, x, B, Cin, N, H, W);
        Act m;
        if (pooled_at_hand) m = r.pool(in, 0, 2);
        stage_out(r, efd(r, p, in, &m), y);
    });
}

int dffw_op_of_block(int device, int precision, const float *x, int B, int Cin, int N, int H, int W, int Cout, int stride,
                     const float *w0, const float *bn0, const float *w2, const float *bn2, const float *wf, float *y, void *hip_stream) {
    dffw_set_last_op_kernels("");
    if (!x || !w0 || !bn0 || !w2 || !bn2 || !wf || !y) return fail(DFFW_EINVAL, "null argument");
    if (precision < 0 || precision > 2) return fail(DFFW_EINVAL, "unknown precision %d", precision);
    static const struct { int cin, cout, s; const char *name; } blocks[] = {
        {3, 8, 1, "OF_feature.0"}, {8, 8, 1, "OF_feature.1"}, {8, 16, 2, "OF_feature1.0"},
        {16, 16, 1, "OF_feature1.1"}, {16, 32, 2, "OF_feature2.0"}, {32, 32, 1, "OF_feature2.1"}};
    const char *name = nullptr;
    for (const auto &b : blocks)
        if (b.cin == Cin && b.cout == Cout && b.s == stride) name = b.name;
    if (!name) return fail(DFFW_EINVAL, "no alignment feature block has (Cin, Cout, stride) = (%d, %d, %d)", Cin, Cout, stride);
    if (B < 1 || N < 1 || H < 1 || W < 1 || H % stride || W % stride) return fail(DFFW_EINVAL, "bad shape (H and W must be multiples of the stride)");
    HIPCHK(hipSetDevice(device));
    const std::string p = std::string("optical_flow_aggregation.") + name;
    OpEngine eng(device, precision);
    for (const LayerDef &L : of_block_layers(p, Cin, Cout, stride)) {
        if (L.folded) continue;
        const bool sc = !L.shortcut.empty();
        const float *w = L.conv == p + ".conv.0.0" ? w0 : L.conv == p + ".conv.2.0" ? w2 : wf;
        const float *bn = L.conv == p + ".conv.0.0" ? bn0 : L.conv == p + ".conv.2.0" ? bn2 : nullptr;
        const int rc = pack_conv(L, precision, w, bn, nullptr, eng.convs[L.conv], sc ? wf : nullptr, sc ? Cin : 0);
        if (rc) return rc;
    }
    return run_op(eng, (hipStream_t)hip_stream, true, [&](Run &r) {
        Act out;
        if (Cin == 3) {
            out = of_first_block(r, p, x, B, N, H, W);
        } else {
            Act in = stage_in(r, x, B, Cin, N, H, W);
            out = of_block(r, p, in);
        }
        stage_out(r, out, y);
    });
}

int dffw_op_head_tail(int device, int precision, const float *x, int B, int C, int N, int H, int W, const float *w2, const float *bn2,
                      const float *w4, const float *bn4, const float *w6, const float *bias6, int start, float *alpha, float *raw, void *hip_stream) {
    dffw_set_last_op_kernels("");
    if (!x || !w2 || !bn2 || !w4 || !bn4 || !w6 || !bias6 || !alpha || !raw) return fail(DFFW_EINVAL, "null argument");
    if (precision < 0 || precision > 2) return fail(DFFW_EINVAL, "unknown precision %d", precision);
    if (C != 16 && C != 32 && C != 64) return fail(DFFW_EINVAL, "the alpha heads have 16, 32 or 64 channels, got %d", C);
    if (start != 0 && start != 2) return fail(DFFW_EINVAL, "start must be 0 (x is y0) or 2 (x is y2), got %d", start);
    if (B < 1 || N < 1 || H < 1 || W < 1) return fail(DFFW_EINVAL, "bad shape B=%d N=%d H=%d W=%d", B, N, H, W);
    if ((int64_t)B * N * 3 > 65535) return fail(DFFW_EINVAL, "B * N * 3 = %lld planes do not fit one launch grid dimension (65535)", (long long)B * N * 3);
    HIPCHK(hipSetDevice(device));
    const char *head = C == 16 ? "conv3" : C == 32 ? "conv2" : "conv1";
    const std::string hp = std::string("optical_flow_aggregation.") + head, label = std::string("flow.") + head;
    OpEngine eng(device, precision);
    for (const LayerDef &L : alpha_head_layers(hp, C + 2, C)) {
        const bool l2 = L.conv == hp + ".2.0", l4 = L.conv == hp + ".4.0", l6 = L.conv == hp + ".6";
        if (!l2 && !l4 && !l6) continue;
        const int rc = pack_conv(L, precision, l2 ? w2 : l4 ? w4 : w6, l2 ? bn2 : l4 ? bn4 : nullptr, l6 ? bias6 : nullptr, eng.convs[L.conv]);
        if (rc) return rc;
    }
    return run_op(eng, (hipStream_t)hip_stream, true, [&](Run &r) {
        Act in = stage_in(r, x, B, C, N, H, W);
        if (start == 0) head_tail(r, hp, label, in, alpha, raw);
        else head_tail_stored(r, hp, label, in, alpha, raw);
    });
}

static int regress_check(int n_heads, const float *const *score, const int *h, const int *w, float *const *depth, int B, int N, int H, int W,
                         const float *focus_dists, const int64_t *fd_strides) {
    if (!score || !h || !w || !depth || !focus_dists || !fd_strides) return fail(DFFW_EINVAL, "null argument");
    if (n_heads < 1 || n_heads > 4) return fail(DFFW_EINVAL, "n_heads must be 1..4, got %d", n_heads);
    if (B < 1 || N < 1 || H < 1 || W < 1) return fail(DFFW_EINVAL, "bad shape B=%d N=%d H=%d W=%d", B, N, H, W);
    for (int k = 0; k < n_heads; ++k) {
        if (!score[k] || !depth[k]) return fail(DFFW_EINVAL, "null argument (head %d)", k);
        if (h[k] < 1 || w[k] < 1) return fail(DFFW_EINVAL, "bad shape: head %d is %dx%d", k, h[k], w[k]);
    }
    return DFFW_OK;
}

int dffw_op_regress(int device, const float *score, int B, int N, int h, int w, int H, int W, const float *focus_dists,
                    const int64_t fd_strides[4], float *depth, void *hip_stream) {
    if (int rc = regress_check(1, &score, &h, &w, &depth, B, N, H, W, focus_dists, fd_strides)) return rc;
    HIPCHK(hipSetDevice(device));
    hipStream_t s = (hipStream_t)hip_stream;
    HIPCHK(launch_regress(score, B, N, h, w, H, W, focus_dists, fd_strides[0], fd_strides[1], fd_strides[2], fd_strides[3], depth, s));
    HIPCHK(hipStreamSynchronize(s));
    return DFFW_OK;
}

int dffw_op_regress_heads(int device, int n_heads, const float *const score[4], const int h[4], const int w[4], float *const depth[4], int B, int N,
                          int H, int W, const float *focus_dists, const int64_t fd_strides[4], int fused, void *hip_stream) {
    dffw_set_last_op_kernels("");
// ... 249 lines not shown
```

dffinthewild_amd/csrc/dffw_run.h:

```cpp
#pragma once
#include <algorithm>
#include <climits>
#include <cstdio>
#include <cstdlib>
#include <cstring>
#include <initializer_list>
#include <map>
#include <string>
#include <vector>

#include "../../include/dffw.h"
#include "dffw_align.h"
#include "dffw_conv_roll.h"
#include "dffw_conv_tile.h"
#include "dffw_internal.h"
#include "dffw_pack.h"

void dffw_set_last_conv_kernel(const char *name);

extern "C" char **environ;

namespace dffw {

static constexpr auto &fail = dffw_fail;
int check_volume(const char *family, int precision, int B, int N, int H, int W, std::initializer_list<int> channels, int div, int64_t units, const char *unit);

inline bool aligned(const void *p, uintptr_t n) { return ((uintptr_t)p & (n - 1)) == 0; }

#define HIPCHK(expr)                                                                          \
    do {                                                                                      \
        hipError_t _e = (expr);                                                               \
        if (_e != hipSuccess) return dffw::fail(DFFW_EHIP, "%s -> %s", #expr, hipGetErrorString(_e)); \
    } while (0)

class Arena {
  public:
    explicit Arena(int64_t cap = INT64_MAX) { free_.push_back({0, cap}); }
    int64_t alloc(int64_t bytes) {
        bytes = (bytes + 255) & ~(int64_t)255;
        for (size_t i = 0; i < free_.size(); ++i) {
            if (free_[i].second >= bytes) {
                const int64_t off = free_[i].first;
                free_[i].first += bytes;
                free_[i].second -= bytes;
                if (free_[i].second == 0) free_.erase(free_.begin() + i);
                live_[off] = bytes;
                peak_ = std::max(peak_, off + bytes);
                return off;
            }
        }
        return -1;
    }
    void release(int64_t off) {
        auto it = live_.find(off);
        if (it == live_.end()) return;
        std::pair<int64_t, int64_t> blk{off, it->second};
        live_.erase(it);
        auto pos = std::lower_bound(free_.begin(), free_.end(), blk);
        pos = free_.insert(pos, blk);
        size_t i = pos - free_.begin();
        if (i + 1 < free_.size() && free_[i].first + free_[i].second == free_[i + 1].first) {
            free_[i].second += free_[i + 1].second;
            free_.erase(free_.begin() + i + 1);
        }
        if (i > 0 && free_[i - 1].first + free_[i - 1].second == free_[i].first) {
            free_[i - 1].second += free_[i].second;
            free_.erase(free_.begin() + i);
        }
    }
    int64_t peak() const { return peak_; }

  private:
    int64_t peak_ = 0;
    std::vector<std::pair<int64_t, int64_t>> free_;
    std::map<int64_t, int64_t> live_;
};

}

struct ProfRec {
    std::string kernel, layer;
    double flops = 0, bytes = 0;
    hipEvent_t e0 = nullptr, e1 = nullptr;
};

struct dffw_engine {
    int device = 0, net = 0, prec = 0;
    std::map<std::string, dffw::PackedConv> convs;
    bool profiling = false;
    std::vector<ProfRec> recs;
    uint16_t *zero_page = nullptr;
    static constexpr int NSIDE = 2, NEV = 16;
    hipStream_t side[NSIDE] = {nullptr, nullptr};
    hipEvent_t ev[NEV] = {};
    int ensure_side() {
        if (side[0]) return DFFW_OK;
        for (int i = 0; i < NSIDE; ++i) HIPCHK(hipStreamCreateWithFlags(&side[i], hipStreamNonBlocking));
        for (int i = 0; i < NEV; ++i) HIPCHK(hipEventCreateWithFlags(&ev[i], hipEventDisableTiming));
        return DFFW_OK;
    }
    int ensure_zero_page() {
        if (zero_page) return DFFW_OK;
        HIPCHK(hipMalloc((void **)&zero_page, 256));
        HIPCHK(hipMemset(zero_page, 0, 256));
        return DFFW_OK;
    }
    void clear_recs() {
        for (auto &r : recs) {
            if (r.e0) (void)hipEventDestroy(r.e0);
            if (r.e1) (void)hipEventDestroy(r.e1);
        }
        recs.clear();
    }
    ~dffw_engine() {
        clear_recs();
        if (zero_page) (void)hipFree(zero_page);
        for (int i = 0; i < NSIDE; ++i)
            if (side[i]) (void)hipStreamDestroy(side[i]);
        for (int i = 0; i < NEV; ++i)
            if (ev[i]) (void)hipEventDestroy(ev[i]);
        for (auto &kv : convs) dffw::free_packed(kv.second);
    }
};

namespace dffw {

inline bool getenv_flag(const char *name) {
    const char *v = getenv(name);
    return v && *v && *v != '0';
}

#define DFFW_SWITCHES(X)                                                                                                 \
    X(NO_CONCURRENT) X(NO_CONF_FORK) X(NO_FUSED_ATTENTION) X(NO_FUSED_EFD) X(NO_FUSED_OF) X(NO_FUSED_POOL) X(NO_FUSED_SRD) \
    X(NO_FUSED_STEM) X(NO_HEAD_SPLIT) X(NO_ROLL) X(NO_ROLL_S2) X(NO_SPLIT) X(NO_SPLITK)  \
    X(NO_STEM_PAIR) X(NO_TILE) X(NO_SMALL) X(NO_ROLL_S2_WIDE) X(NO_HEAD_SUMS) X(NO_HEAD_SUMS_FUSED) X(NO_HEAD_WARP) X(NO_OF_FIRST) \
    X(NO_LEAN_TILE) X(NO_LEAN_ROLL) X(NO_ROLLX) X(NO_ROLLK) X(NO_ROLLT) X(NO_TEAMS) X(NO_SLICE32) X(NO_REGRESS_FUSED) X(NO_STEM_PIPE) X(NO_POOL3) X(NO_NARROW)
enum SwitchId {
#define X_ID(n) SW_##n,
    DFFW_SWITCHES(X_ID)
#undef X_ID
    SW_COUNT
};
#define DFFW_INT_KNOBS(X)                                                                                                                                  \
    X(ROLL_WGS, roll_wgs, 8, 0)                                                                                                                            \
    X(SRD_WGS, srd_wgs, 8, 0)                                                                                                                              \
                                                                                                                                         \
    X(SMALL_MAX_UNITS, small_max_units, 0, 0)                                                                                                              \
    X(ROLL_ZSPLIT, roll_zsplit, 1, 0)                                                                                                                      \
    X(KSPLIT_TARGET, ksplit_target, 1, 512)                                                                                                                \
                                                                  \
    X(REDIR_SIDE, redir_side, 0, -1)                                                                                                                       \
    X(TEAM_MIN_WGS, team_min_wgs, 0, 0)                                                                                                                    \
    X(TEAM_MAX_WGS, team_max_wgs, 1, 320)                                                                                                                  \
     \
    X(SPLIT_S64, split_s64, 1, 1025)                                                                                                                       \
                                                 \
    X(SPLIT_T64, split_t64, 1, 1025)                                                                                                                       \
                                   \
    X(NARROW_MAX, narrow_max, 1, 40)                                                                                                                       \
                                      \
    X(WARM_MAX_WGS, warm_max_wgs, 0, 1024)                                                                                                                 \
                                                                                            \
    X(ROLLK_MERGE_BELOW, rollk_merge_below, 0, 1 << 30)                                                                                                    \
                                                                                                \
    X(ROLLT_MIN_UNITS, rollt_min_units, 1, 128)                                                                                                            \
                                                                                                                \
    X(ROLL_MIN_UNITS, roll_min_units, 1, 192)                                                                                                              \
                                                                                                     \
    X(SPLIT_WG, split_wg, INT_MIN, 256)                                                                                                                    \
                        \
    X(WGRAD_WGS, wgrad_wgs, 8, 0)                                                                                                                          \
    X(WGRAD_FLUSH_UNITS, wgrad_flush_units, 1, 256)                                                                                                        \
                                                                 \
    X(PWGRAD_WGS, pwgrad_wgs, 8, 0)                                                                                                                        \
    X(PWGRAD_FLUSH_STEPS, pwgrad_flush_steps, 1, 512)                                                                                                      \
                                                                                                                       \
    X(BN_WGS, bn_wgs, 1, 0)                                                                                                                                \
                                                                                               \
    X(SCORE_WGS, score_wgs, 1, 0)                                                                                                                          \
    X(DEBUG_FLAGS, debug_flags, INT_MIN, 0)
#define DFFW_INT64_KNOBS(X)                                                                                                                                \
                                                                                                                                        \
    X(CONCURRENT_MAX_PIXELS, concurrent_max_pixels, -1)                                                                                                    \
                            \
    X(CONCURRENT_MIN_PIXELS, concurrent_min_pixels, 400000)

inline void warn_unknown_switches() {
    static const bool once = [] {
        static const char *const known[] = {
#define X_NM(n) "DFFW_" #n,
            DFFW_SWITCHES(X_NM)
#undef X_NM
#define X_NM(n, ...) "DFFW_" #n,
            DFFW_INT_KNOBS(X_NM) DFFW_INT64_KNOBS(X_NM)
#undef X_NM
            "DFFW_SRD_PIPE", "DFFW_TRACE_LAYER", "DFFW_TRACE_OUT", "DFFW_RCCL_LIB", "DFFW_LIB_PATH", "DFFW_NO_PROBE", "DFFW_PRECISION",
            "DFFW_BENCH_ONE_DEVICE", "DFFW_BENCH_TIMEOUT_S",
            "DFFW_SRD_ABL", "DFFW_ROLLX_ABL", "DFFW_ROLLX_NTS", "DFFW_ROLLK_ABL", "DFFW_ROLLK_SKEW"};
        for (char **e = ::environ; e && *e; ++e) {
            if (strncmp(*e, "DFFW_", 5) != 0) continue;
            const char *eq = strchr(*e, '=');
            const size_t n = eq ? (size_t)(eq - *e) : strlen(*e);
            bool ok = false;
            for (const char *k : known) ok = ok || (strlen(k) == n && strncmp(k, *e, n) == 0);
            if (!ok) fprintf(stderr, "libdffw: environment variable %.*s is not a switch this library reads (retired or misspelt?) -- ignored\n", (int)n, *e);
        }
        return true;
    }();
    (void)once;
}

struct Switches {
    bool f[SW_COUNT];
#define X_FIELD(n, field, lo, dflt) int field = dflt;
    DFFW_INT_KNOBS(X_FIELD)
#undef X_FIELD
#define X_FIELD(n, field, dflt) int64_t field = dflt;
    DFFW_INT64_KNOBS(X_FIELD)
#undef X_FIELD
    bool srd_pipe = false;
    const char *trace_layer = nullptr, *trace_out = nullptr;
    bool on(int id) const { return f[id]; }
    bool tracing(const std::string &layer) const { return trace_layer && trace_out && layer == trace_layer; }
    int path_bits() const;
    static Switches read() {
        Switches s;
        int i = 0;
#define X_RD(n) s.f[i++] = getenv_flag("DFFW_" #n);
        DFFW_SWITCHES(X_RD)
#undef X_RD
#define X_RD(n, field, lo, dflt) if (const char *z = getenv("DFFW_" #n)) if (atoi(z) >= lo) s.field = atoi(z);
        DFFW_INT_KNOBS(X_RD)
#undef X_RD
#define X_RD(n, field, dflt) if (const char *z = getenv("DFFW_" #n)) s.field = atoll(z);
        DFFW_INT64_KNOBS(X_RD)
#undef X_RD
        s.rollt_min_units = std::min(s.rollt_min_units, s.roll_min_units);
        s.srd_pipe = getenv_flag("DFFW_SRD_PIPE");
        warn_unknown_switches();
        s.trace_layer = getenv("DFFW_TRACE_LAYER");
        s.trace_out = getenv("DFFW_TRACE_OUT");
        return s;
    }
};

inline int Switches::path_bits() const {
    return (f[SW_NO_LEAN_TILE] ? DFFW_ARGS_NO_LEAN_TILE : 0) | (f[SW_NO_LEAN_ROLL] ? DFFW_ARGS_NO_LEAN_ROLL : 0) | (f[SW_NO_ROLLX] ? DFFW_ARGS_NO_ROLLX : 0) |
           (f[SW_NO_ROLLK] ? DFFW_ARGS_NO_ROLLK : 0) | (f[SW_NO_SLICE32] ? DFFW_ARGS_NO_SLICE32 : 0) | (f[SW_NO_ROLLT] ? DFFW_ARGS_NO_ROLLT : 0);
}

struct ConvOpt {
    const Act *in1 = nullptr;
    const Act *res0 = nullptr, *res1 = nullptr;
    bool res_bcast = false;
    int relu = 0;
    Act *out_pre = nullptr;
    float *outf = nullptr;
    int outf_ch = 1;
    const float *fs32 = nullptr;
    bool raw = false;
    float *sums = nullptr;
    const char *cls = nullptr;
    float *cls_out = nullptr;
    bool discard = false;
};

inline bool conv_tiled(const PackedConv &pc, const Switches &sw, int gH, int gW) {
    const TileCfg *c = pc.tile.cfg;
    return c && !sw.on(SW_NO_TILE) && gW * 2 >= c->tx && gH * 2 >= c->ty;
}
inline bool conv_sums_ok(const PackedConv &pc, const Switches &sw, int B, int N, int H, int W) {
    if (!conv_tiled(pc, sw, H, W)) return false;
    const TileCfg *c = pc.tile.cfg;
    if (!tile_cfg_has_sums(c) || W % c->tx) return false;
    const int64_t tiles = (int64_t)B * ((N + c->tz - 1) / c->tz) * ((H + c->ty - 1) / c->ty) * (W / c->tx);
    return tiles >= 256;
}

inline RollArgs roll_args(const uint16_t *filter, int B, int tiles_y, int tiles_x, int zsplit, int wgs, int pair = 0) {
    RollArgs t;
    memset(&t, 0, sizeof t);
    t.wroll = filter;
    t.tiles_y = tiles_y;
    t.tiles_x = tiles_x;
    t.zsplit = zsplit;
    t.total_tiles = B * zsplit * tiles_y * tiles_x;
    t.wgs = wgs;
    t.pair = pair;
    return t;
}

inline SrdArgs srd_args(const uint16_t *x, uint16_t *out, const PackedConv &c0, const PackedConv &c2, int B, int N, int H, int W, int ty, int tx, int wgs) {
    SrdArgs a;
    memset(&a, 0, sizeof a);
    a.x = x; a.out = out;
    a.w0 = c0.wsrd; a.w2 = c2.wsrd;
    a.b0 = c0.bias; a.b2 = c2.bias;
    a.B = B; a.N = N; a.H = H; a.W = W;
    a.tiles_y = H / ty; a.tiles_x = W / tx;
    a.total_tiles = B * a.tiles_y * a.tiles_x;
    a.wgs = wgs;
    return a;
}
inline HeadWarpArgs head_warp_args(const Act &fe, const uint16_t *ref, uint16_t *out, const PackedConv &cur, const float *alpha, const float *fov, int wgs) {
    HeadWarpArgs a;
    memset(&a, 0, sizeof a);
    a.fe = fe.p; a.ref = ref; a.out = out;
    a.w = cur.wsrd; a.bias = cur.bias;
    a.alpha = alpha; a.fov = fov;
    a.B = fe.B; a.N = fe.N; a.H = fe.H; a.W = fe.W;
    a.tiles_y = fe.H / 8; a.tiles_x = fe.W / 16;
    a.total_tiles = fe.B * a.tiles_y * a.tiles_x;
    a.wgs = wgs;
    return a;
}

struct Run {
    dffw_engine *e;
    hipStream_t s;
    Arena arena;
    bool dry;
    char *ws;
    int err = DFFW_OK;
    const dffw_tap *taps = nullptr;
    int n_taps = 0;

    hipStream_t main_s;
    bool concurrent = false;
    bool forked = false;
    int ev_next = 0;
    unsigned side_open = 0;
    std::vector<void *> deferred;

    const Switches sw;

    Run(dffw_engine *e_, hipStream_t s_, bool dry_, char *ws_, int64_t cap)
        : e(e_), s(s_), arena(cap), dry(dry_), ws(ws_), main_s(s_), sw(Switches::read()) {
        if (sw.debug_flags & 1) err = fail(DFFW_EINVAL, "DFFW_DEBUG_FLAGS bit 0 (skip the footprint fill) is not supported; use 2 (no MFMA loop), 4 (no stores) or 6");
    }

    bool ok() const { return err == DFFW_OK; }

    void enable_concurrency() {
        concurrent = true;
        if (!dry && ok() && e->ensure_side() != DFFW_OK) err = DFFW_EHIP;
    }
    void fork(int k) {
        if (!concurrent || dry || !ok()) return;
        hipEvent_t v = e->ev[ev_next++ % dffw_engine::NEV];
        check(hipEventRecord(v, main_s), "fork record");
        check(hipStreamWaitEvent(e->side[k], v, 0), "fork wait");
        fork_mark(k);
    }
    void on(int k) { s = (concurrent && !dry && k >= 0) ? e->side[k] : main_s; }
    void fork_mark(int k) { side_open |= 1u << k; }
    void join(int k) {
        if (!concurrent || dry || !e->side[k]) return;
        hipEvent_t v = e->ev[ev_next++ % dffw_engine::NEV];
        const hipError_t h1 = hipEventRecord(v, e->side[k]);
        const hipError_t h2 = h1 == hipSuccess ? hipStreamWaitEvent(main_s, v, 0) : h1;
        side_open &= ~(1u << k);
        if (ok()) check(h2, "join");
    }
    ~Run() {
        for (int k = 0; k < dffw_engine::NSIDE; ++k)
            if (side_open & (1u << k)) join(k);
    }
    void release_deferred() {
        for (void *p : deferred) arena.release(dry ? (int64_t)(uintptr_t)p - 256 : (int64_t)((char *)p - ws));
        deferred.clear();
    }

    void *raw(int64_t bytes) {
        if (!ok()) return nullptr;
        const int64_t off = arena.alloc(bytes);
        if (off < 0) {
            err = fail(DFFW_ENOMEM, "workspace too small (need more than the %lld bytes given)", (long long)bytes);
            return nullptr;
        }
        return dry ? (void *)(uintptr_t)(off + 256) : (void *)(ws + off);
    }
    void drop_raw(void *p) {
        if (!p) return;
        if (forked) {
            deferred.push_back(p);
            return;
        }
        arena.release(dry ? (int64_t)(uintptr_t)p - 256 : (int64_t)((char *)p - ws));
    }
    Act act(int B, int N, int H, int W, int C) {
        Act a;
        a.B = B; a.N = N; a.H = H; a.W = W; a.C = C;
        a.p = (uint16_t *)raw(a.pixels() * prec_parts(e->prec) * C * (int64_t)sizeof(uint16_t));
        return a;
    }
    void drop(Act &a) {
        drop_raw(a.p);
        a.p = nullptr;
    }
    void check(hipError_t h, const char *what) {
        if (ok() && h != hipSuccess) err = fail(DFFW_EHIP, "%s: %s", what, hipGetErrorString(h));
    }
    void prof_begin(const char *kernel, const std::string &layer, double flops, double bytes, const char *suffix = "") {
        if (!e->profiling || dry || !ok()) return;
        ProfRec pr;
        pr.kernel = kernel;
        pr.layer = layer + suffix;
        pr.flops = flops;
        pr.bytes = bytes;
        check(hipEventCreate(&pr.e0), "hipEventCreate");
        check(hipEventCreate(&pr.e1), "hipEventCreate");
        if (ok()) check(hipEventRecord(pr.e0, s), "hipEventRecord");
        e->recs.push_back(pr);
    }
    void prof_end() {
        if (!e->profiling || dry || !ok() || e->recs.empty()) return;
        check(hipEventRecord(e->recs.back().e1, s), "hipEventRecord");
    }
    double elem_bytes() const { return 2.0 * prec_parts(e->prec); }
    template <class Go>
    void launch_unnamed(const char *kernel, const std::string &layer, const char *suffix, double flops, double bytes, const char *what, size_t trace_words, Go &&go) {
        prof_begin(kernel, layer, flops, bytes, suffix);
        unsigned long long *trace = trace_words ? trace_begin(layer, trace_words) : nullptr;
        check(go(trace), what);
        prof_end();
    }
    template <class Go>
    void launch(const char *kernel, const std::string &layer, const char *suffix, double flops, double bytes, const char *what, size_t trace_words, Go &&go) {
        dffw_set_last_conv_kernel(kernel);
        launch_unnamed(kernel, layer, suffix, flops, bytes, what, trace_words, go);
    }
    const uint16_t *zero_page() {
        if (e->ensure_zero_page() != DFFW_OK) err = DFFW_EHIP;
        return ok() ? e->zero_page : nullptr;
    }
    const PackedConv *layer(const std::string &name) const {
        auto it = e->convs.find(name);
        return it == e->convs.end() ? nullptr : &it->second;
    }

    unsigned long long *trace_dev = nullptr;
    size_t trace_n = 0;
    static constexpr size_t STEP_TRACE_WORDS = (size_t)1024 * 4 * 32 * 8;
    unsigned long long *trace_begin(const std::string &layer, size_t words) {
        if (dry || !ok() || !sw.tracing(layer)) return nullptr;
        trace_n = words;
        check(hipMalloc((void **)&trace_dev, trace_n * 8), "trace alloc");
        if (ok()) check(hipMemsetAsync(trace_dev, 0, trace_n * 8, s), "trace memset");
        return ok() ? trace_dev : nullptr;
    }
    void trace_end() {
        if (!trace_dev) return;
        if (ok()) {
            std::vector<unsigned long long> host(trace_n);
            check(hipStreamSynchronize(s), "trace sync");
            check(hipMemcpy(host.data(), trace_dev, trace_n * 8, hipMemcpyDeviceToHost), "trace copy");
            if (FILE *f = fopen(sw.trace_out, "wb")) {
                fwrite(host.data(), 8, host.size(), f);
                fclose(f);
            }
        }
        (void)hipFree(trace_dev);
        trace_dev = nullptr;
    }

    bool tiled(const std::string &name, int gH, int gW) const {
        const PackedConv *pc = layer(name);
        return pc && conv_tiled(*pc, sw, gH, gW);
    }
    bool sums_conv_ok(const std::string &name, int B, int N, int H, int W) const {
        const PackedConv *pc = layer(name);
        return pc && conv_sums_ok(*pc, sw, B, N, H, W);
    }

    Act conv(const std::string &name, const Act &in0, const ConvOpt &o = ConvOpt());

    Act pool(const Act &x, int mode, int k) {
        Act out = act(x.B, x.N, x.H / k, x.W / k, x.C);
        if (ok() && !dry) {
            char kn[48];
            snprintf(kn, sizeof kn, "dffw::pool_kernel<%d>", e->prec);
            launch_unnamed(kn, mode == 0 ? "maxpool" : "avgpool", "", 0.0, (double)(x.pixels() + out.pixels()) * x.C * elem_bytes(), "pool", 0,
                           [&](unsigned long long *) { return launch_pool(e->prec, mode, k, x.p, out.p, x.B, x.N, x.H, x.W, x.C, s); });
        }
        return out;
    }

    void tap(const char *name, const Act &a) {
        if (!ok() || dry) return;
        for (int i = 0; i < n_taps; ++i)
            if (!strcmp(taps[i].name, name)) {
                const int64_t n = a.pixels() * a.C;
                if (taps[i].numel != n) {
                    err = fail(DFFW_EINVAL, "tap %s holds %lld elements, caller gave %lld", name, (long long)n, (long long)taps[i].numel);
                    return;
                }
                check(launch_to_ncdhw(e->prec, a.p, taps[i].dst, a.B, a.C, a.N, a.H, a.W, s), name);
            }
    }
    void tap_f32(const char *name, const float *p, int64_t n) {
        if (!ok() || dry) return;
        for (int i = 0; i < n_taps; ++i)
            if (!strcmp(taps[i].name, name)) {
                if (taps[i].numel != n) {
                    err = fail(DFFW_EINVAL, "tap %s holds %lld elements, caller gave %lld", name, (long long)n, (long long)taps[i].numel);
                    return;
                }
                check(hipMemcpyAsync(taps[i].dst, p, n * sizeof(float), hipMemcpyDeviceToDevice, s), name);
            }
    }
};

int run_depth(Run &r, const float *FS, const float *fd, const int64_t fst[4], int B, int N, int H, int W, float *const out[4], const RawStack *raw = nullptr);
int run_e2e(Run &r, const float *FS, const float *fd, const int64_t fst[4], const float *fov, int B, int N, int H, int W, float *const out[4], float *aligned);
Act of_block(Run &r, const std::string &p, const Act &x);
Act of_first_block(Run &r, const std::string &p0, const float *FS, int B, int N, int H, int W);
void head_tail(Run &r, const std::string &hp, const std::string &label, Act &y0, float *alpha, float *rawh);
void head_tail_stored(Run &r, const std::string &hp, const std::string &label, Act &y2, float *alpha, float *rawh);
Act srd(Run &r, const std::string &p, Act &x, bool drop_x, Act *pooled = nullptr);
Act efd(Run &r, const std::string &p, const Act &x, Act *pooled = nullptr);
std::vector<LayerDef> srd_layers(const std::string &p, int c);
std::vector<LayerDef> efd_layers(const std::string &p, int cin, int cout);
std::vector<LayerDef> of_block_layers(const std::string &p, int cin, int cout, int s);
std::vector<LayerDef> alpha_head_layers(const std::string &p, int cin, int c);

}
```

dffinthewild_amd/engine.py:

```python
import ctypes
import os
import threading
import types
from ctypes import POINTER, byref, c_char_p, c_float, c_int, c_int64, c_void_p

import numpy as np
import torch

_HERE = os.path.dirname(os.path.abspath(__file__))
LIB_PATH = os.environ.get("DFFW_LIB_PATH") or os.path.join(_HERE, "libdffw.so")

PRECISIONS = {"bf16x3": 0, "fp16": 1, "bf16": 2}
NET_DEPTH = 0
NET_E2E = 1


class DffwError(RuntimeError):
    pass


class _Tensor(ctypes.Structure):
    _fields_ = [("name", c_char_p), ("data", POINTER(c_float)), ("numel", c_int64)]


class _Tap(ctypes.Structure):
    _fields_ = [("name", c_char_p), ("dst", c_void_p), ("numel", c_int64)]


class _Prof(ctypes.Structure):
    _fields_ = [("kernel", c_char_p), ("layer", c_char_p), ("flops", ctypes.c_double), ("bytes", ctypes.c_double),
                ("ms", c_float)]


class AdamTensor(ctypes.Structure):
    _fields_ = [("param", c_void_p), ("grad", c_void_p), ("exp_avg", c_void_p), ("exp_avg_sq", c_void_p), ("numel", c_int64)]


assert ctypes.sizeof(AdamTensor) == 40


class SimParams(ctypes.Structure):
    _fields_ = [("pixel_per_meter", ctypes.c_double), ("min_depth", ctypes.c_double), ("max_depth", ctypes.c_double),
                ("min_focus", ctypes.c_double), ("max_focus", ctypes.c_double), ("num_planes", c_int), ("max_radius", c_int)]


def _load():
    if not os.path.exists(LIB_PATH):
        raise DffwError(
            f"{LIB_PATH} not found: build the HIP extension first "
            "(python -c 'import __graft_entry__ as g; g.build()' or make -C dffinthewild_amd/csrc). "
            "dffinthewild_amd has no CPU fallback.")
    lib = ctypes.CDLL(LIB_PATH)
    lib.dffw_version.restype = c_char_p
    lib.dffw_last_error.restype = c_char_p
    lib.dffw_last_conv_kernel.restype = c_char_p
    lib.dffw_param_count.argtypes = [c_int]
    lib.dffw_param_info.argtypes = [c_int, c_int, POINTER(c_char_p), POINTER(c_int64), POINTER(c_int), POINTER(c_int)]
    lib.dffw_engine_create.argtypes = [c_int, c_int, POINTER(_Tensor), c_int, c_int, POINTER(c_void_p)]
    lib.dffw_engine_destroy.argtypes = [c_void_p]
    lib.dffw_engine_destroy.restype = None
    lib.dffw_engine_precision.argtypes = [c_void_p]
    lib.dffw_workspace_bytes.argtypes = [c_void_p, c_int, c_int, c_int, c_int]
    lib.dffw_workspace_bytes.restype = c_int64
    fwd = [c_void_p, c_void_p, c_void_p, POINTER(c_int64), c_int, c_int, c_int, c_int,
           POINTER(c_void_p), c_void_p, c_int64, c_void_p]
    lib.dffw_forward.argtypes = fwd
    lib.dffw_forward_taps.argtypes = fwd + [POINTER(_Tap), c_int]
    lib.dffw_forward_e2e.argtypes = [c_void_p, c_void_p, c_void_p, POINTER(c_int64), c_void_p, c_int, c_int, c_int, c_int,
                                     POINTER(c_void_p), c_void_p, c_void_p, c_int64, c_void_p, POINTER(_Tap), c_int]
    lib.dffw_forward_raw.argtypes = [c_void_p, c_void_p, c_int, POINTER(c_int64), c_int, c_int, c_void_p, POINTER(c_int64), c_int, c_int, c_int,
                                     c_int, POINTER(c_void_p), c_void_p, c_int64, c_void_p]
    lib.dffw_profile_enable.argtypes = [c_void_p, c_int]
    lib.dffw_profile_collect.argtypes = [c_void_p, POINTER(_Prof), c_int]
    lib.dffw_op_conv3d.argtypes = [c_int, c_int, c_void_p, c_int, c_int, c_int, c_int, c_int, POINTER(c_float), c_int,
                                   POINTER(c_int), POINTER(c_int), POINTER(c_int), POINTER(c_int), c_int,
                                   POINTER(c_float), POINTER(c_float), c_void_p, c_int, c_void_p, c_void_p]
    lib.dffw_op_conv3d_ex.argtypes = [c_int, c_int, c_void_p, c_int, c_int, c_int, c_int, c_int, POINTER(c_float), c_int,
                                      POINTER(c_int), POINTER(c_int), POINTER(c_int), POINTER(c_int), c_int,
                                      POINTER(c_float), POINTER(c_float), c_void_p, c_int, c_void_p, c_void_p, POINTER(c_float), c_void_p, c_void_p]
    lib.dffw_op_pool.argtypes = [c_int, c_int, c_int, c_int, c_void_p, c_int, c_int, c_int, c_int, c_int, c_void_p, c_void_p]
    lib.dffw_op_srd.argtypes = [c_int, c_int, c_void_p, c_int, c_int, c_int, c_int, c_int] + [POINTER(c_float)] * 6 + [c_void_p] * 3
    lib.dffw_op_efd.argtypes = [c_int, c_int, c_void_p, c_int, c_int, c_int, c_int, c_int] + [POINTER(c_float)] * 4 + [c_int, c_void_p, c_void_p]
    lib.dffw_op_of_block.argtypes = [c_int, c_int, c_void_p] + [c_int] * 7 + [POINTER(c_float)] * 5 + [c_void_p] * 2
    lib.dffw_op_head_tail.argtypes = [c_int, c_int, c_void_p] + [c_int] * 5 + [POINTER(c_float)] * 6 + [c_int] + [c_void_p] * 3
    lib.dffw_last_op_kernels.restype = c_char_p
    lib.dffw_op_fov_warp.argtypes = [c_int, c_void_p, c_int, c_int, c_int, c_int, c_int, c_void_p, c_void_p, c_int,
                                     c_void_p, c_void_p, c_void_p]
    lib.dffw_op_regress.argtypes = [c_int, c_void_p, c_int, c_int, c_int, c_int, c_int, c_int, c_void_p,
                                    POINTER(c_int64), c_void_p, c_void_p]
    lib.dffw_op_regress_heads.argtypes = [c_int, c_int, POINTER(c_void_p), POINTER(c_int), POINTER(c_int), POINTER(c_void_p), c_int, c_int, c_int, c_int,
                                          c_void_p, POINTER(c_int64), c_int, c_void_p]
    c_u8p = POINTER(ctypes.c_uint8)
    lib.dffw_pack_stack.argtypes = [c_int, c_void_p, c_int, POINTER(c_int64), c_int, c_int, c_int, c_int, c_int, c_int, c_void_p, c_void_p]
    lib.dffw_augment_stack.argtypes = [c_int, c_void_p, c_int, POINTER(c_int64)] + [c_int] * 6 + [c_void_p, c_int] + [c_void_p] * 6 + \
                                      [c_int, c_float, c_float, c_float, c_void_p]
    lib.dffw_unpack_stack.argtypes = [c_int, c_void_p, c_int, c_int, c_int, c_int, c_int, c_int, c_void_p, c_void_p]
    lib.dffw_colorize.argtypes = [c_int, c_void_p, c_int, c_int, c_int, c_int, c_int, c_int, c_float, c_float, c_void_p, c_void_p, c_void_p]
    lib.dffw_jet_lut.argtypes = [c_u8p]
    lib.dffw_metrics_scratch_bytes.argtypes = [c_int]
    lib.dffw_metrics_scratch_bytes.restype = c_int64
    lib.dffw_metrics.argtypes = [c_int, c_void_p, c_int, c_int, c_int, c_void_p, c_void_p, c_void_p, c_int, c_int, c_void_p, c_void_p,
                                 c_int64, c_void_p]
    lib.dffw_comm_unique_id.argtypes = [ctypes.c_char_p]
    lib.dffw_comm_init_rank.argtypes = [c_int, c_int, c_int, ctypes.c_char_p, POINTER(c_void_p)]
    lib.dffw_comm_init_all.argtypes = [c_int, POINTER(c_int), POINTER(c_void_p)]
    lib.dffw_comm_destroy.argtypes = [c_void_p]
    lib.dffw_comm_destroy.restype = None
    lib.dffw_comm_rank.argtypes = [c_void_p]
    lib.dffw_comm_size.argtypes = [c_void_p]
    lib.dffw_allgather.argtypes = [c_void_p, c_void_p, c_void_p, c_int64, c_void_p]
    lib.dffw_probe_peaks.argtypes = [c_int, POINTER(c_float), POINTER(c_float), c_void_p]
    lib.dffw_sim_workspace_bytes.argtypes = [c_int, c_int, c_int, c_int, c_int]
    lib.dffw_sim_workspace_bytes.restype = c_int64
    lib.dffw_sim_render.argtypes = [c_int, SimParams, c_void_p, c_void_p, c_void_p, c_void_p, c_int, c_int, c_int, c_int] + [c_void_p] * 7 + [c_int64, c_void_p]
    lib.dffw_sim_plan_host.argtypes = [POINTER(SimParams), POINTER(ctypes.c_double), ctypes.c_double, ctypes.c_double, c_int,
                                       POINTER(ctypes.c_double), POINTER(c_int), POINTER(ctypes.c_double), POINTER(ctypes.c_double), POINTER(c_int)]
    lib.dffw_sim_disk_rows.argtypes = [c_int, POINTER(c_int)]
    lib.dffw_loss_workspace_bytes.argtypes = [c_int, c_int, c_int, c_int]
    lib.dffw_loss_workspace_bytes.restype = c_int64
    lib.dffw_loss_heads.argtypes = [c_int, c_int, POINTER(c_void_p), POINTER(c_int), POINTER(c_int), c_int, c_int, c_int, c_int, c_void_p, POINTER(c_int64),
                                    c_void_p, c_void_p, c_void_p, POINTER(c_float), c_int, c_float, c_float, POINTER(c_void_p), POINTER(c_void_p),
                                    c_void_p, c_void_p, c_int64, c_void_p]
    lib.dffw_heads_backward.argtypes = [c_int, c_int, POINTER(c_void_p), POINTER(c_int), POINTER(c_int), c_int, c_int, c_int, c_int, c_void_p, POINTER(c_int64),
                                        POINTER(c_void_p), POINTER(c_void_p), c_void_p]
    lib.dffw_op_conv3d_backward.argtypes = [c_int, c_int, c_void_p, c_int, c_int, c_int, c_int, c_int, POINTER(c_float), c_int,
                                            POINTER(c_int), POINTER(c_int), POINTER(c_int), c_int, c_void_p, c_void_p, c_void_p, c_void_p]
    lib.dffw_conv_wgrad_workspace_bytes.argtypes = [c_int] * 6 + [POINTER(c_int)] * 3 + [c_int]
    lib.dffw_conv_wgrad_workspace_bytes.restype = c_int64
    lib.dffw_conv_wgrad.argtypes = [c_int, c_int, c_void_p, c_int, c_int, c_int, c_int, c_int, c_void_p, c_int,
                                    POINTER(c_int), POINTER(c_int), POINTER(c_int), c_int, c_void_p, c_void_p, c_int64, c_void_p]
    lib.dffw_conv_cat_wgrad_workspace_bytes.argtypes = [c_int] * 7
    lib.dffw_conv_cat_wgrad_workspace_bytes.restype = c_int64
    lib.dffw_conv_cat_wgrad.argtypes = [c_int, c_int, c_void_p, c_int, c_void_p, c_int] + [c_int] * 4 + [c_void_p, c_int, c_void_p, c_void_p, c_int64, c_void_p]
    lib.dffw_op_conv_cat_backward.argtypes = [c_int, c_int, c_void_p, c_int, c_void_p, c_int] + [c_int] * 4 + [POINTER(c_float), c_int] + [c_void_p] * 5
    c_double = ctypes.c_double
    lib.dffw_bn_train_workspace_bytes.argtypes = [c_int] * 5
    lib.dffw_bn_train_workspace_bytes.restype = c_int64
    lib.dffw_bn_train_forward.argtypes = [c_int, c_int, c_void_p] + [c_int] * 5 + [c_void_p, c_void_p, c_double, c_double] + [c_void_p] * 3 + \
                                         [c_int] + [c_void_p] * 4 + [c_int64, c_void_p]
    lib.dffw_bn_train_backward.argtypes = [c_int, c_int] + [c_void_p] * 3 + [c_int] * 5 + [c_void_p] * 3 + [c_int] + [c_void_p] * 5 + [c_int64, c_void_p]
    lib.dffw_op_bn_train.argtypes = [c_int, c_int, c_void_p] + [c_int] * 5 + [c_void_p, c_void_p, c_double, c_double] + [c_void_p] * 3 + \
                                    [c_int] + [c_void_p] * 4
    lib.dffw_op_bn_train_backward.argtypes = [c_int, c_int] + [c_void_p] * 3 + [c_int] * 5 + [c_void_p] * 3 + [c_int] + [c_void_p] * 5
    lib.dffw_op_conv_pw_backward.argtypes = [c_int, c_int, c_void_p, c_int, c_int, c_int, c_int, c_int, POINTER(c_float), c_int,
                                             POINTER(c_int), POINTER(c_int), c_void_p, c_void_p, c_void_p, c_void_p]
    lib.dffw_conv_pw_wgrad_workspace_bytes.argtypes = [c_int] * 6 + [POINTER(c_int)] * 2
    lib.dffw_conv_pw_wgrad_workspace_bytes.restype = c_int64
    lib.dffw_conv_pw_wgrad.argtypes = [c_int, c_int, c_void_p, c_int, c_int, c_int, c_int, c_int, c_void_p, c_int,
                                       POINTER(c_int), POINTER(c_int), c_void_p, c_void_p, c_int64, c_void_p]
    lib.dffw_grad_combine.argtypes = [c_int, c_int] + [c_void_p] * 3 + [c_int] * 5 + [c_void_p] * 2
    lib.dffw_op_grad_combine.argtypes = [c_int, c_int] + [c_void_p] * 3 + [c_int] * 5 + [c_void_p] * 2
    lib.dffw_pool_backward.argtypes = [c_int] * 4 + [c_void_p] * 3 + [c_int] * 5 + [c_void_p] * 2
    lib.dffw_op_pool_backward.argtypes = [c_int] * 4 + [c_void_p] * 3 + [c_int] * 5 + [c_void_p] * 2
    lib.dffw_pool3_backward.argtypes = [c_int, c_int] + [c_void_p] * 4 + [c_int] * 5 + [c_void_p] * 2
    lib.dffw_op_pool3_backward.argtypes = [c_int, c_int] + [c_void_p] * 4 + [c_int] * 5 + [c_void_p] * 2
    lib.dffw_stem_wgrad_workspace_bytes.argtypes = [c_int] * 4
    lib.dffw_stem_wgrad_workspace_bytes.restype = c_int64
    lib.dffw_stem_wgrad.argtypes = [c_int, c_int, c_void_p, c_void_p] + [c_int] * 4 + [c_void_p, c_void_p, c_int64, c_void_p]
    lib.dffw_op_stem_backward.argtypes = [c_int, c_int, c_void_p, c_void_p] + [c_int] * 4 + [c_void_p, c_void_p]
    lib.dffw_score_conv_dgrad.argtypes = [c_int, c_int, c_void_p] + [c_int] * 5 + [c_void_p, POINTER(c_int), POINTER(c_int)] + [c_void_p] * 3
    lib.dffw_score_conv_wgrad_workspace_bytes.argtypes = [c_int] * 5 + [POINTER(c_int)] * 2
    lib.dffw_score_conv_wgrad_workspace_bytes.restype = c_int64
    lib.dffw_score_conv_wgrad.argtypes = [c_int, c_int, c_void_p, c_void_p] + [c_int] * 5 + [POINTER(c_int), POINTER(c_int), c_void_p, c_void_p, c_int64, c_void_p]
    lib.dffw_op_score_conv_backward.argtypes = [c_int, c_int, c_void_p] + [c_int] * 5 + [c_void_p, POINTER(c_int), POINTER(c_int)] + [c_void_p] * 5
    lib.dffw_adam_tensors_per_launch.argtypes = []
    lib.dffw_adam_step.argtypes = [c_int, POINTER(AdamTensor), c_int, c_int64, ctypes.c_double, ctypes.c_double, ctypes.c_double, ctypes.c_double, c_void_p]
    return lib


lib = _load()
ADAM_TENSORS_PER_LAUNCH = lib.dffw_adam_tensors_per_launch()
COMM_ID_BYTES = 128
RAW_NORM_F64 = 16
AUG_NPARAMS = 8

ABI_SYMBOLS = (
    "dffw_version", "dffw_last_error", "dffw_param_count", "dffw_param_info", "dffw_engine_create",
    "dffw_engine_destroy", "dffw_engine_precision", "dffw_workspace_bytes", "dffw_forward",
    "dffw_forward_taps", "dffw_profile_enable", "dffw_profile_collect", "dffw_op_conv3d", "dffw_op_conv3d_ex", "dffw_op_pool", "dffw_op_regress",
    "dffw_op_regress_heads",
    "dffw_op_fov_warp", "dffw_forward_e2e", "dffw_last_conv_kernel", "dffw_op_srd", "dffw_op_efd", "dffw_last_op_kernels",
    "dffw_op_of_block", "dffw_op_head_tail",
    "dffw_forward_raw", "dffw_pack_stack", "dffw_augment_stack", "dffw_unpack_stack", "dffw_colorize", "dffw_jet_lut", "dffw_metrics_scratch_bytes", "dffw_metrics",
    "dffw_comm_unique_id", "dffw_comm_init_rank", "dffw_comm_init_all", "dffw_comm_destroy", "dffw_comm_rank", "dffw_comm_size",
    "dffw_allgather", "dffw_comm_group_start", "dffw_comm_group_end", "dffw_probe_peaks",
    "dffw_sim_workspace_bytes", "dffw_sim_render", "dffw_sim_plan_host", "dffw_sim_disk_rows",
    "dffw_loss_workspace_bytes", "dffw_loss_heads",
    "dffw_op_conv3d_backward", "dffw_conv_wgrad_workspace_bytes", "dffw_conv_wgrad",
    "dffw_bn_train_workspace_bytes", "dffw_bn_train_forward", "dffw_bn_train_backward", "dffw_op_bn_train", "dffw_op_bn_train_backward",
    "dffw_op_conv_pw_backward", "dffw_conv_pw_wgrad_workspace_bytes", "dffw_conv_pw_wgrad", "dffw_grad_combine", "dffw_op_grad_combine",
    "dffw_pool_backward", "dffw_pool3_backward", "dffw_op_pool_backward", "dffw_op_pool3_backward",
    "dffw_stem_wgrad_workspace_bytes", "dffw_stem_wgrad", "dffw_op_stem_backward",
    "dffw_score_conv_dgrad", "dffw_score_conv_wgrad_workspace_bytes", "dffw_score_conv_wgrad", "dffw_op_score_conv_backward",
    "dffw_adam_tensors_per_launch", "dffw_adam_step",
    "dffw_conv_cat_wgrad_workspace_bytes", "dffw_conv_cat_wgrad", "dffw_op_conv_cat_backward",
    "dffw_heads_backward",
)


def _check(rc, what):
    if rc < 0:
        msg = lib.dffw_last_error().decode("utf-8", "replace")
        if rc == -1:
            raise ValueError(f"{what}: {msg}")
        raise DffwError(f"{what} failed ({rc}): {msg}")
    return rc


def param_table(net=NET_DEPTH):
    n = _check(lib.dffw_param_count(net), "dffw_param_count")
    out = []
    for i in range(n):
        name, shape, ndim, flags = c_char_p(), (c_int64 * 5)(), c_int(), c_int()
        _check(lib.dffw_param_info(net, i, byref(name), shape, byref(ndim), byref(flags)), "dffw_param_info")
        out.append((name.value.decode(), tuple(shape[:ndim.value]), flags.value))
    return out


def _stream_ptr(device):
    return c_void_p(torch.cuda.current_stream(device).cuda_stream)


def _f32(t):
    return ctypes.cast(t.data_ptr(), POINTER(c_float))


def _dev(t):
    return t.device.index if t.device.index is not None else torch.cuda.current_device()


def _ptr(t):
    return c_void_p(t.data_ptr()) if t is not None else None


class Engine:

    def __init__(self, state_dict, device, precision="bf16x3", net=NET_DEPTH):
        if precision not in PRECISIONS:
            raise ValueError(f"precision must be one of {sorted(PRECISIONS)}, got {precision!r}")
        self.device = torch.device(device)
        if self.device.type != "cuda":
            raise DffwError("the HIP engine needs a GPU device (no CPU fallback)")
        self.index = self.device.index if self.device.index is not None else torch.cuda.current_device()
        self.precision = precision
        keep, arr = [], (_Tensor * len(state_dict))()
        i = 0
        for key, t in state_dict.items():
            if not torch.is_floating_point(t):
                continue
            h = t.detach().to("cpu", torch.float32).contiguous()
            keep.append(h)
            arr[i] = _Tensor(key.encode(), _f32(h), h.numel())
            i += 1
        self._h = c_void_p()
        _check(lib.dffw_engine_create(self.index, net, arr, i, PRECISIONS[precision], byref(self._h)), "dffw_engine_create")
        self._ws = {}
        self._ws_stream = None
        self._lock = threading.Lock()

    def __copy__(self):
        raise TypeError("dffinthewild_amd.engine.Engine cannot be copied: build a new one from the state dict")

    def __deepcopy__(self, memo):
        raise TypeError("dffinthewild_amd.engine.Engine cannot be copied: build a new one from the state dict")

    def __reduce__(self):
        raise TypeError("dffinthewild_amd.engine.Engine cannot be pickled: save the model's state_dict instead")

    def __del__(self, _destroy=lib.dffw_engine_destroy):
        h = getattr(self, "_h", None)
        if h:
            _destroy(h)
            self._h = None

    def profile(self, on=True):
        _check(lib.dffw_profile_enable(self._h, int(on)), "dffw_profile_enable")

    def profile_collect(self):
        n = _check(lib.dffw_profile_collect(self._h, None, 0), "dffw_profile_collect")
        arr = (_Prof * n)()
        _check(lib.dffw_profile_collect(self._h, arr, n), "dffw_profile_collect")
        return [(e.kernel.decode(), e.layer.decode(), e.flops, e.bytes, e.ms) for e in arr]

    def workspace_bytes(self, B, N, H, W):
        return _check(lib.dffw_workspace_bytes(self._h, B, N, H, W), "dffw_workspace_bytes")

    def _workspace(self, B, N, H, W, extra=0):
        key = (B, N, H, W, extra)
        ws = self._ws.get(key)
        if ws is None:
            nbytes = self.workspace_bytes(B, N, H, W) + extra
            self._ws.clear()
            ws = torch.empty(nbytes, dtype=torch.uint8, device=self.device)
            self._ws[key] = ws
        return ws

    def _call_ws(self, B, N, H, W, extra, call):
        cur = torch.cuda.current_stream(self.index)
        if self._ws_stream is not None and self._ws_stream != cur and self._ws:
            ev = torch.cuda.Event()
            ev.record(self._ws_stream)
            cur.wait_event(ev)
        self._ws_stream = cur
        rc = call(self._workspace(B, N, H, W, extra))
        if rc == -3:
            cur.synchronize()
            self._ws.clear()
            rc = call(self._workspace(B, N, H, W, extra))
        return rc

    def forward(self, FS, focus_dists, taps=None):
        B, C, N, H, W = FS.shape
        FS = FS.contiguous()
        fd = focus_dists.expand(B, N, H, W)
        strides = (c_int64 * 4)(*fd.stride())
        outs = [torch.empty((B, H, W), dtype=torch.float32, device=FS.device) for _ in range(4)]
        optrs = (c_void_p * 4)(*[o.data_ptr() for o in outs])
        with self._lock, torch.cuda.device(self.index):
            def args(ws):
                return [self._h, _ptr(FS), _ptr(fd), strides, B, N, H, W, optrs, _ptr(ws), ws.numel(), _stream_ptr(self.index)]
            if not taps:
                _check(self._call_ws(B, N, H, W, 0, lambda ws: lib.dffw_forward(*args(ws))), "dffw_forward")
                return tuple(outs)
            shapes = _tap_shapes(B, N, H, W)
            bufs = {nm: torch.empty(shapes[nm], dtype=torch.float32, device=FS.device) for nm in taps}
            tarr = (_Tap * len(bufs))(*[_Tap(nm.encode(), _ptr(t), t.numel()) for nm, t in bufs.items()])
            _check(self._call_ws(B, N, H, W, 0, lambda ws: lib.dffw_forward_taps(*args(ws), tarr, len(bufs))), "dffw_forward_taps")
            return tuple(outs), bufs


    def forward_raw(self, raw, strides, dtype, h, w, focus_dists, B, N, H, W):
        fd = focus_dists.expand(B, N, H, W)
        fst = (c_int64 * 4)(*fd.stride())
        outs = [torch.empty((B, H, W), dtype=torch.float32, device=fd.device) for _ in range(4)]
        optrs = (c_void_p * 4)(*[o.data_ptr() for o in outs])
        with self._lock, torch.cuda.device(self.index):
            st5 = (c_int64 * 5)(*strides)
            _check(self._call_ws(B, N, H, W, B * 3 * N * H * W * 4 + 256,
                                 lambda ws: lib.dffw_forward_raw(self._h, c_void_p(raw), dtype, st5, h, w, _ptr(fd), fst,
                                                                 B, N, H, W, optrs, _ptr(ws), ws.numel(), _stream_ptr(self.index))),
                   "dffw_forward_raw")
        return tuple(outs)

    def forward_e2e(self, FS, focus_dists, fovs, taps=None):
        B, C, N, H, W = FS.shape
        FS = FS.contiguous()
        fd = focus_dists.expand(B, N, H, W)
        fov = fovs.reshape(B, N).contiguous()
        strides = (c_int64 * 4)(*fd.stride())
        outs = [torch.empty((B, H, W), dtype=torch.float32, device=FS.device) for _ in range(4)]
        aligned = torch.empty_like(FS)
        optrs = (c_void_p * 4)(*[o.data_ptr() for o in outs])
        with self._lock, torch.cuda.device(self.index):
            bufs, tarr, nt = {}, None, 0
            if taps:
                shapes = _tap_shapes(B, N, H, W)
                bufs = {nm: torch.empty(shapes[nm], dtype=torch.float32, device=FS.device) for nm in taps}
                tarr = (_Tap * len(bufs))(*[_Tap(nm.encode(), _ptr(t), t.numel()) for nm, t in bufs.items()])
                nt = len(bufs)
            _check(self._call_ws(B, N, H, W, 0,
                                 lambda ws: lib.dffw_forward_e2e(self._h, _ptr(FS), _ptr(fd), strides, _ptr(fov), B, N, H, W, optrs, _ptr(aligned),
                                                                 _ptr(ws), ws.numel(), _stream_ptr(self.index), tarr, nt)),
                   "dffw_forward_e2e")
        res = tuple(outs) + (aligned,)
        return (res, bufs) if taps else res


def _tap_shapes(B, N, H, W):
    return {
        "head3": (B, 3, N), "head2": (B, 3, N), "head1": (B, 3, N), "alpha": (B, 3, N),
        "alpha3": (B, 3, N), "alpha2": (B, 3, N),
        "fe1": (B, 8, N, H, W), "fe2": (B, 16, N, H // 2, W // 2), "fe3": (B, 32, N, H // 4, W // 4),
        "stem": (B, 8, N, H, W), "V1": (B, 8, N, H, W), "E1": (B, 16, N, H // 2, W // 2), "V2": (B, 16, N, H // 2, W // 2),
        "E2": (B, 32, N, H // 4, W // 4), "V3": (B, 32, N, H // 4, W // 4),
        "FS_volume": (B, 32, N, H // 8, W // 8), "conf": (B, N, H // 8, W // 8),
        "cost1": (B, N, H // 4, W // 4), "cost2": (B, N, H // 2, W // 2), "cost3": (B, N, H, W),
    }


def _i3(v):
    v = (v, v, v) if isinstance(v, int) else tuple(v)
    return (c_int * 3)(*v)


def op_conv3d(x, weight, *, stride=1, pad=0, dilation=1, transposed=False, bn=None, bias=None,
              residual=None, relu=0, precision="bf16x3", want_pre=False, cls_weight=None):
    B, Cin, N, H, W = x.shape
    w = weight.detach().to("cpu", torch.float32).contiguous()
    Cout = w.shape[1] if transposed else w.shape[0]
    k = tuple(w.shape[2:])
    s, p, d = _i3(stride), _i3(pad), _i3(dilation)
    if transposed:
        No, Ho, Wo = N, 2 * H, 2 * W
    else:
        No = N + 2 * p[0] - (k[0] - 1)
        Ho = (H + 2 * p[1] - d[1] * (k[1] - 1) - 1) // s[1] + 1
        Wo = (W + 2 * p[2] - d[2] * (k[2] - 1) - 1) // s[2] + 1
    bnh = None
    if bn is not None:
        bnh = torch.cat([t.detach().to("cpu", torch.float32).reshape(-1) for t in bn]).contiguous()
    bh = bias.detach().to("cpu", torch.float32).contiguous() if bias is not None else None
    y = torch.empty((B, No, Ho, Wo) if Cout == 1 else (B, Cout, No, Ho, Wo), dtype=torch.float32, device=x.device)
    x = x.contiguous()
    res = residual.contiguous() if residual is not None else None
    dev = _dev(x)
    ex = want_pre or cls_weight is not None
    y_pre = torch.empty_like(y) if want_pre else None
    cw = cls_weight.detach().to("cpu", torch.float32).reshape(-1).contiguous() if cls_weight is not None else None
    score = torch.empty((B, No, Ho, Wo), dtype=torch.float32, device=x.device) if cw is not None else None
    with torch.cuda.device(dev):
        args = (dev, PRECISIONS[precision], _ptr(x), B, Cin, N, H, W, _f32(w), Cout,
                (c_int * 3)(*k), s, p, d, int(transposed),
                _f32(bnh) if bnh is not None else None, _f32(bh) if bh is not None else None, _ptr(res), relu, _ptr(y))
        if ex:
            _check(lib.dffw_op_conv3d_ex(*args, _ptr(y_pre), _f32(cw) if cw is not None else None, _ptr(score), _stream_ptr(dev)), "dffw_op_conv3d_ex")
            return y, y_pre, score
        _check(lib.dffw_op_conv3d(*args, _stream_ptr(dev)), "dffw_op_conv3d")
    return y


def conv3d_output_shape(x_shape, weight_shape, stride, pad, transposed):
    B, Cin, N, H, W = x_shape
    k, s, p = tuple(weight_shape[2:]), tuple(_i3(stride)), tuple(_i3(pad))
    if transposed:
        return (B, weight_shape[1], N, 2 * H, 2 * W)
    return (B, weight_shape[0], N + 2 * p[0] - (k[0] - 1), (H + 2 * p[1] - k[1]) // s[1] + 1, (W + 2 * p[2] - k[2]) // s[2] + 1)


def _conv_backward(fn, x, weight, grad, need, precision, *, checks, layout, want, what, b=None, weight_on_gpu=False):
    name = fn.__name__[len("dffw_"):]
    if any(t.device.type != "cuda" for t in (x, grad, b) if t is not None):
        raise DffwError(f"{name} needs GPU tensors (no CPU fallback)")
    for check in checks:
        msg = check()
        if msg:
            raise ValueError(f"{name}: {msg}")
    w = weight.detach().to(x.device if weight_on_gpu else "cpu", torch.float32).contiguous()
    x, grad, b = (t.detach().float().contiguous() if t is not None else None for t in (x, grad, b))
    dev = _dev(x)
    gx = torch.empty_like(x) if "x" in need else None
    gw = torch.empty(tuple(w.shape), dtype=torch.float32, device=x.device) if "w" in need else None
    B, Cin, N, H, W = x.shape

    def call(with_x, with_w):
        t = types.SimpleNamespace(x=_ptr(x), w=_ptr(w) if weight_on_gpu else _f32(w), grad=_ptr(grad), b=_ptr(b) if with_x else None,
                                  gx=_ptr(gx) if with_x else None, gw=_ptr(gw) if with_w else None, B=B, Cin=Cin, N=N, H=H, W=W)
        return fn(dev, PRECISIONS[precision], *layout(t), _stream_ptr(dev))
    with torch.cuda.device(dev):
        _check(call(False, False), fn.__name__)
        if tuple(grad.shape) != want():
            raise ValueError(f"{name}: {what[0]} {tuple(grad.shape)} is not the {what[1]} {want()}")
        _check(call(gx is not None, gw is not None), fn.__name__)
    return gx, gw


def op_conv3d_backward(x, weight, grad_y, *, stride=1, pad=0, dilation=1, transposed=False, precision="bf16x3", need=("x", "w")):
    checks = (lambda: tuple(_i3(dilation)) != (1, 1, 1) and f"dilation must be 1, got {dilation}",
              lambda: (x.dim() != 5 or weight.dim() != 5 or grad_y.dim() != 5) and "x, weight and grad_y must have 5 dimensions",
              lambda: weight.shape[0 if transposed else 1] != x.shape[1] and f"weight {tuple(weight.shape)} does not take {x.shape[1]} input channels")
    return _conv_backward(
        lib.dffw_op_conv3d_backward, x, weight, grad_y, need, precision, checks=checks,
        layout=lambda t: (t.x, t.B, t.Cin, t.N, t.H, t.W, t.w, weight.shape[1 if transposed else 0], _i3(weight.shape[2:]), _i3(stride), _i3(pad),
                          int(transposed), t.grad, t.gx, t.gw),
        want=lambda: conv3d_output_shape(x.shape, weight.shape, stride, pad, transposed), what=("grad_y", "conv's output shape"))


def op_conv_pw_backward(x, weight, grad_y, *, pad, stride=1, dilation=1, precision="bf16x3", need=("x", "w")):
    checks = (lambda: (tuple(_i3(stride)) != (1, 1, 1) or tuple(_i3(dilation)) != (1, 1, 1)) and f"stride and dilation must be 1, got {stride} and {dilation}",
              lambda: (x.dim() != 5 or weight.dim() != 5 or grad_y.dim() != 5) and "x, weight and grad_y must have 5 dimensions",
              lambda: weight.shape[1] != x.shape[1] and f"weight {tuple(weight.shape)} does not take {x.shape[1]} input channels")
    return _conv_backward(
        lib.dffw_op_conv_pw_backward, x, weight, grad_y, need, precision, checks=checks,
        layout=lambda t: (t.x, t.B, t.Cin, t.N, t.H, t.W, t.w, weight.shape[0], _i3(weight.shape[2:]), _i3(pad), t.grad, t.gx, t.gw),
        want=lambda: (x.shape[0], weight.shape[0]) + tuple(x.shape[2:]), what=("grad_y", "conv's output shape"))


def op_conv_cat_backward(xa, xb, weight, grad_y, *, precision="bf16x3", need=("xa", "xb", "w")):
    name = "op_conv_cat_backward"
    checks = (lambda: any(t.dim() != 5 for t in (xa, xb, weight, grad_y)) and "xa, xb, weight and grad_y must have 5 dimensions",
              lambda: (xa.shape[0], *xa.shape[2:]) != (xb.shape[0], *xb.shape[2:]) and
              f"xa {tuple(xa.shape)} and xb {tuple(xb.shape)} differ outside the channel axis",
              lambda: tuple(weight.shape[2:]) != (3, 3, 3) and f"the conv over a concatenation is 3x3x3 stride 1 pad 1, got a {tuple(weight.shape[2:])} kernel",
              lambda: weight.shape[1] != xa.shape[1] + xb.shape[1] and
              f"weight {tuple(weight.shape)} does not take {xa.shape[1]} + {xb.shape[1]} input channels",
              lambda: tuple(grad_y.shape) != (xa.shape[0], weight.shape[0], *xa.shape[2:]) and
              f"grad_y {tuple(grad_y.shape)} is not the conv's output shape {(xa.shape[0], weight.shape[0], *xa.shape[2:])}",
              lambda: set(need) - {"xa", "xb", "w"} and f"need {tuple(need)} names something other than 'xa', 'xb', 'w'")
    for check in checks:
        msg = check()
        if msg:
            raise ValueError(f"{name}: {msg}")
    if any(t.device.type != "cuda" for t in (xa, xb, grad_y)):
        raise DffwError(f"{name} needs GPU tensors (no CPU fallback)")
    if len({t.device for t in (xa, xb, grad_y)}) != 1:
        raise ValueError(f"{name}: xa, xb and grad_y must be on one GPU")
    w = weight.detach().to("cpu", torch.float32).contiguous()
    xa, xb, grad_y = (t.detach().float().contiguous() for t in (xa, xb, grad_y))
    dev = _dev(xa)
    B, Ca, N, H, W = xa.shape
    Cb, Cout = xb.shape[1], w.shape[0]
    gxa = torch.empty_like(xa) if "xa" in need else None
    gxb = torch.empty_like(xb) if "xb" in need else None
    gw = torch.empty(tuple(w.shape), dtype=torch.float32, device=xa.device) if "w" in need else None
    with torch.cuda.device(dev):
        _check(lib.dffw_op_conv_cat_backward(dev, PRECISIONS[precision], _ptr(xa), Ca, _ptr(xb), Cb, B, N, H, W, _f32(w), Cout, _ptr(grad_y), _ptr(gxa),
                                             _ptr(gxb), _ptr(gw), _stream_ptr(dev)), "dffw_op_conv_cat_backward")
    return gxa, gxb, gw


def op_grad_combine(a, y=None, b=None, *, precision="bf16x3"):
    tensors = [a] + [t for t in (y, b) if t is not None]
    if any(t.device.type != "cuda" for t in tensors):
        raise DffwError("op_grad_combine needs GPU tensors (no CPU fallback)")
    if a.dim() != 5 or any(t.shape != a.shape for t in tensors):
        raise ValueError("op_grad_combine: a, y and b must be 5-dimensional tensors of one shape")
    if y is None and b is None:
        raise ValueError("op_grad_combine: neither a mask (y) nor a second gradient (b): a copy is no operation")
    B, C, N, H, W = a.shape
    a, y, b = (t.detach().float().contiguous() if t is not None else None for t in (a, y, b))
    dev = _dev(a)
    out = torch.empty_like(a)
    with torch.cuda.device(dev):
        _check(lib.dffw_op_grad_combine(dev, PRECISIONS[precision], _ptr(a), _ptr(y), _ptr(b), B, C, N, H, W, _ptr(out), _stream_ptr(dev)),
               "dffw_op_grad_combine")
    return out


POOL_MODES = {"max": 0, "avg": 1}


def op_pool_backward(grad_y, x=None, b=None, *, k, mode, precision="bf16x3"):
    if mode not in POOL_MODES:
        raise ValueError(f"op_pool_backward: mode must be one of {sorted(POOL_MODES)}, got {mode!r}")
    tensors = [grad_y] + [t for t in (x, b) if t is not None]
    if any(t.device.type != "cuda" for t in tensors):
        raise DffwError("op_pool_backward needs GPU tensors (no CPU fallback)")
    if grad_y.dim() != 5:
        raise ValueError("op_pool_backward: grad_y must have 5 dimensions")
    B, C, N, Ho, Wo = grad_y.shape
    k = int(k)
    shape = (B, C, N, Ho * k, Wo * k)
    for t, what in ((x, "x"), (b, "b")):
        if t is not None and tuple(t.shape) != shape:
            raise ValueError(f"op_pool_backward: {what} {tuple(t.shape)} is not the pool's input shape {shape}")
    grad_y, x, b = (t.detach().float().contiguous() if t is not None else None for t in (grad_y, x, b))
    dev = _dev(grad_y)
    out = torch.empty(shape, dtype=torch.float32, device=grad_y.device)
    with torch.cuda.device(dev):
        _check(lib.dffw_op_pool_backward(dev, PRECISIONS[precision], POOL_MODES[mode], k, _ptr(grad_y), _ptr(x), _ptr(b), B, C, N, shape[3], shape[4],
                                         _ptr(out), _stream_ptr(dev)), "dffw_op_pool_backward")
    return out


def op_pool3_backward(g2, g4, g8, b=None, *, precision="bf16x3"):
    tensors = [g2, g4, g8] + ([b] if b is not None else [])
    if any(t is None for t in tensors):
        raise ValueError("op_pool3_backward needs all of g2, g4 and g8")
    if any(t.device.type != "cuda" for t in tensors):
        raise DffwError("op_pool3_backward needs GPU tensors (no CPU fallback)")
    if g8.dim() != 5:
        raise ValueError("op_pool3_backward: g8 must have 5 dimensions")
    B, C, N, H8, W8 = g8.shape
    shape = (B, C, N, 8 * H8, 8 * W8)
    for t, what, f in ((g2, "g2", 4), (g4, "g4", 2), (b, "b", None)):
        want = shape if f is None else (B, C, N, f * H8, f * W8)
        if t is not None and tuple(t.shape) != want:
            raise ValueError(f"op_pool3_backward: {what} {tuple(t.shape)} does not go with g8 {tuple(g8.shape)}: expected {want}")
    g2, g4, g8, b = (t.detach().float().contiguous() if t is not None else None for t in (g2, g4, g8, b))
    dev = _dev(g8)
    out = torch.empty(shape, dtype=torch.float32, device=g8.device)
# ... 427 lines not shown
```

include/dffw.h:

```cpp
#ifndef DFFW_H
#define DFFW_H

#include <stdint.h>

#ifdef __cplusplus
extern "C" {
#endif

#define DFFW_OK 0
#define DFFW_EINVAL (-1)
#define DFFW_EHIP (-2)
#define DFFW_ENOMEM (-3)
#define DFFW_EMISSING (-4)

#define DFFW_PREC_BF16X3 0
#define DFFW_PREC_FP16 1
#define DFFW_PREC_BF16 2

#define DFFW_NET_DEPTH 0
#define DFFW_NET_E2E 1
#define DFFW_E2E_SLICES 10

typedef struct dffw_engine dffw_engine;

typedef struct dffw_tensor {
    const char *name;
    const float *data;
    int64_t numel;
} dffw_tensor;

typedef struct dffw_tap {
    const char *name;
    float *dst;
    int64_t numel;
} dffw_tap;

const char *dffw_version(void);
const char *dffw_last_error(void);
const char *dffw_last_conv_kernel(void);

int dffw_param_count(int net);
int dffw_param_info(int net, int index, const char **name, int64_t shape[5], int *ndim, int *flags);

int dffw_engine_create(int device, int net, const dffw_tensor *tensors, int n_tensors,
                       int precision, dffw_engine **out);
void dffw_engine_destroy(dffw_engine *e);
int dffw_engine_precision(const dffw_engine *e);

int64_t dffw_workspace_bytes(const dffw_engine *e, int B, int N, int H, int W);

int dffw_forward(dffw_engine *e, const float *FS, const float *focus_dists,
                 const int64_t fd_strides[4], int B, int N, int H, int W, float *const out[4],
                 void *workspace, int64_t workspace_bytes, void *hip_stream);

int dffw_forward_taps(dffw_engine *e, const float *FS, const float *focus_dists,
                      const int64_t fd_strides[4], int B, int N, int H, int W, float *const out[4],
                      void *workspace, int64_t workspace_bytes, void *hip_stream,
                      const dffw_tap *taps, int n_taps);

int dffw_forward_e2e(dffw_engine *e, const float *FS, const float *focus_dists,
                     const int64_t fd_strides[4], const float *fovs, int B, int N, int H, int W,
                     float *const out[4], float *aligned, void *workspace, int64_t workspace_bytes,
                     void *hip_stream, const dffw_tap *taps, int n_taps);

typedef struct dffw_prof_entry {
    const char *kernel;
    const char *layer;
    double flops;
    double bytes;
    float ms;
} dffw_prof_entry;
int dffw_profile_enable(dffw_engine *e, int on);
int dffw_profile_collect(dffw_engine *e, dffw_prof_entry *out, int capacity);


int dffw_op_conv3d(int device, int precision, const float *x, int B, int Cin, int N, int H, int W,
                   const float *weight, int Cout, const int kernel[3], const int stride[3],
                   const int pad[3], const int dilation[3], int transposed, const float *bn,
                   const float *conv_bias, const float *residual, int relu, float *y,
                   void *hip_stream);

int dffw_op_conv3d_ex(int device, int precision, const float *x, int B, int Cin, int N, int H, int W,
                      const float *weight, int Cout, const int kernel[3], const int stride[3],
                      const int pad[3], const int dilation[3], int transposed, const float *bn,
                      const float *conv_bias, const float *residual, int relu, float *y, float *y_pre,
                      const float *cls_weight, float *cls_score, void *hip_stream);

int dffw_op_pool(int device, int precision, int mode, int k, const float *x, int B, int C, int N,
                 int H, int W, float *y, void *hip_stream);

int dffw_op_srd(int device, int precision, const float *x, int B, int C, int N, int H, int W,
                const float *w0, const float *bn0, const float *w2, const float *bn2, const float *w3,
                const float *w1, float *y, float *pooled, void *hip_stream);

int dffw_op_efd(int device, int precision, const float *x, int B, int Cin, int N, int H, int W,
                const float *ws, const float *bns, const float *wp, const float *bnp, int pooled_at_hand,
                float *y, void *hip_stream);

int dffw_op_of_block(int device, int precision, const float *x, int B, int Cin, int N, int H, int W, int Cout, int stride,
                     const float *w0, const float *bn0, const float *w2, const float *bn2, const float *wf, float *y,
                     void *hip_stream);

int dffw_op_head_tail(int device, int precision, const float *x, int B, int C, int N, int H, int W, const float *w2, const float *bn2,
                      const float *w4, const float *bn4, const float *w6, const float *bias6, int start, float *alpha, float *raw,
                      void *hip_stream);

const char *dffw_last_op_kernels(void);

int dffw_op_regress(int device, const float *score, int B, int N, int h, int w, int H, int W,
                    const float *focus_dists, const int64_t fd_strides[4], float *depth,
                    void *hip_stream);

int dffw_op_regress_heads(int device, int n_heads, const float *const score[4], const int h[4], const int w[4],
                          float *const depth[4], int B, int N, int H, int W, const float *focus_dists,
                          const int64_t fd_strides[4], int fused, void *hip_stream);

int dffw_op_fov_warp(int device, const float *x, int B, int C, int N, int H, int W, const float *alpha,
                     const float *fovs, int alpha_from_sample0, float *out, float *flow, void *hip_stream);

#define DFFW_RAW_U8 0
#define DFFW_RAW_F32 1
#define DFFW_RAW_NORM_F64 16
int dffw_pack_stack(int device, const void *raw, int dtype, const int64_t strides[5], int B, int N, int h, int w,
                    int Hp, int Wp, float *FS, void *hip_stream);

#define DFFW_AUG_NPARAMS 8
enum { DFFW_AUG_Y0, DFFW_AUG_X0, DFFW_AUG_CONTRAST, DFFW_AUG_BRIGHTNESS, DFFW_AUG_GAMMA, DFFW_AUG_FLIP_X, DFFW_AUG_FLIP_Y, DFFW_AUG_ANGLE };
int dffw_augment_stack(int device, const void *raw, int dtype, const int64_t strides[5], int B, int N, int H, int W, int h, int w,
                       const double *params, int transposed, float *FS, const float *gt, const float *conf, float *gt_out,
                       uint8_t *mask_out, float *conf_out, int use_range, float lo, float hi, float sentinel, void *hip_stream);

int dffw_forward_raw(dffw_engine *e, const void *raw, int dtype, const int64_t raw_strides[5], int h, int w,
                     const float *focus_dists, const int64_t fd_strides[4], int B, int N, int H, int W,
                     float *const out[4], void *workspace, int64_t workspace_bytes, void *hip_stream);

#define DFFW_RANGE_FIXED 0
#define DFFW_RANGE_MINMAX 1
int dffw_colorize(int device, const float *depth, int B, int H, int W, int h, int w, int mode, float lo, float hi,
                  float *range, uint8_t *rgb, void *hip_stream);
int dffw_jet_lut(uint8_t *lut768);

int dffw_unpack_stack(int device, const float *warp, int B, int N, int H, int W, int h, int w, uint8_t *images, void *hip_stream);

#define DFFW_N_METRICS 12
int64_t dffw_metrics_scratch_bytes(int B);
int dffw_metrics(int device, const float *est, int B, int H, int W, const float *gt, const uint8_t *mask,
                 const float *conf, int h, int w, double *out, void *scratch, int64_t scratch_bytes, void *hip_stream);

int64_t dffw_loss_workspace_bytes(int B, int N, int H, int W);
int dffw_loss_heads(int device, int n_heads, const float *const score[4], const int h[4], const int w[4],
                    int B, int N, int H, int W, const float *focus_dists, const int64_t fd_strides[4],
                    const float *gt, const uint8_t *mask, const float *conf, const float weights[4],
                    int use_range, float lo, float hi, float *const pred[4], float *const grad[4],
                    double *losses, void *workspace, int64_t workspace_bytes, void *hip_stream);

int dffw_heads_backward(int device, int n_heads, const float *const score[4], const int h[4], const int w[4],
                        int B, int N, int H, int W, const float *focus_dists, const int64_t fd_strides[4],
                        const float *const grad_pred[4], float *const grad_score[4], void *hip_stream);

int dffw_op_conv3d_backward(int device, int precision, const float *x, int B, int Cin, int N, int H, int W, const float *weight, int Cout,
                            const int kernel[3], const int stride[3], const int pad[3], int transposed, const float *grad_y, float *grad_x,
                            float *grad_w, void *hip_stream);
int64_t dffw_conv_wgrad_workspace_bytes(int B, int Cin, int N, int H, int W, int Cout, const int kernel[3], const int stride[3],
                                        const int pad[3], int transposed);
int dffw_conv_wgrad(int device, int precision, const void *x, int B, int Cin, int N, int H, int W, const void *grad_y, int Cout,
                    const int kernel[3], const int stride[3], const int pad[3], int transposed, float *grad_w, void *workspace,
                    int64_t workspace_bytes, void *hip_stream);

int64_t dffw_bn_train_workspace_bytes(int B, int C, int N, int H, int W);
int dffw_bn_train_forward(int device, int precision, const void *x, int B, int C, int N, int H, int W, const float *gamma, const float *beta,
                          double eps, double momentum, float *running_mean, float *running_var, const void *res, int relu, void *y,
                          float *save_mean, float *save_invstd, void *workspace, int64_t workspace_bytes, void *hip_stream);
int dffw_bn_train_backward(int device, int precision, const void *x, const void *y, const void *grad_y, int B, int C, int N, int H, int W,
                           const float *gamma, const float *save_mean, const float *save_invstd, int relu, void *grad_x, void *grad_res,
                           float *grad_gamma, float *grad_beta, void *workspace, int64_t workspace_bytes, void *hip_stream);
int dffw_op_bn_train(int device, int precision, const float *x, int B, int C, int N, int H, int W, const float *gamma, const float *beta,
                     double eps, double momentum, float *running_mean, float *running_var, const float *res, int relu, float *y,
                     float *save_mean, float *save_invstd, void *hip_stream);
int dffw_op_bn_train_backward(int device, int precision, const float *x, const float *y, const float *grad_y, int B, int C, int N, int H,
                              int W, const float *gamma, const float *save_mean, const float *save_invstd, int relu, float *grad_x,
                              float *grad_res, float *grad_gamma, float *grad_beta, void *hip_stream);

int dffw_op_conv_pw_backward(int device, int precision, const float *x, int B, int Cin, int N, int H, int W, const float *weight, int Cout,
                             const int kernel[3], const int pad[3], const float *grad_y, float *grad_x, float *grad_w, void *hip_stream);
int64_t dffw_conv_pw_wgrad_workspace_bytes(int B, int Cin, int N, int H, int W, int Cout, const int kernel[3], const int pad[3]);
int dffw_conv_pw_wgrad(int device, int precision, const void *x, int B, int Cin, int N, int H, int W, const void *grad_y, int Cout,
                       const int kernel[3], const int pad[3], float *grad_w, void *workspace, int64_t workspace_bytes, void *hip_stream);
int dffw_grad_combine(int device, int precision, const void *a, const void *y, const void *b, int B, int C, int N, int H, int W, void *out,
                      void *hip_stream);
int dffw_op_grad_combine(int device, int precision, const float *a, const float *y, const float *b, int B, int C, int N, int H, int W,
                         float *out, void *hip_stream);

int dffw_pool_backward(int device, int precision, int mode, int k, const void *g, const void *x, const void *b, int B, int C, int N, int H,
                       int W, void *out, void *hip_stream);
int dffw_pool3_backward(int device, int precision, const void *g2, const void *g4, const void *g8, const void *b, int B, int C, int N, int H,
                        int W, void *out, void *hip_stream);
int dffw_op_pool_backward(int device, int precision, int mode, int k, const float *g, const float *x, const float *b, int B, int C, int N,
                          int H, int W, float *out, void *hip_stream);
int dffw_op_pool3_backward(int device, int precision, const float *g2, const float *g4, const float *g8, const float *b, int B, int C, int N,
                           int H, int W, float *out, void *hip_stream);

int64_t dffw_stem_wgrad_workspace_bytes(int B, int N, int H, int W);
int dffw_stem_wgrad(int device, int precision, const float *x, const void *grad_y, int B, int N, int H, int W, float *grad_w, void *workspace,
                    int64_t workspace_bytes, void *hip_stream);
int dffw_op_stem_backward(int device, int precision, const float *x, const float *grad_y, int B, int N, int H, int W, float *grad_w,
                          void *hip_stream);

int dffw_score_conv_dgrad(int device, int precision, const float *grad_score, int B, int Cin, int N, int h, int w, const float *weight,
                          const int kernel[3], const int pad[3], const void *b, void *out, void *hip_stream);
int64_t dffw_score_conv_wgrad_workspace_bytes(int B, int Cin, int N, int h, int w, const int kernel[3], const int pad[3]);
int dffw_score_conv_wgrad(int device, int precision, const void *x, const float *grad_score, int B, int Cin, int N, int h, int w,
                          const int kernel[3], const int pad[3], float *grad_w, void *workspace, int64_t workspace_bytes, void *hip_stream);
int dffw_op_score_conv_backward(int device, int precision, const float *x, int B, int Cin, int N, int h, int w, const float *weight,
                                const int kernel[3], const int pad[3], const float *grad_score, const float *b, float *grad_x, float *grad_w,
                                void *hip_stream);

typedef struct dffw_adam_tensor {
    float *param;
    const float *grad;
    float *exp_avg;
    float *exp_avg_sq;
    int64_t numel;
} dffw_adam_tensor;
int dffw_adam_tensors_per_launch(void);
int dffw_adam_step(int device, const dffw_adam_tensor *tensors, int n_tensors, int64_t step, double lr, double beta1, double beta2, double eps,
                   void *hip_stream);

int64_t dffw_conv_cat_wgrad_workspace_bytes(int B, int Ca, int Cb, int N, int H, int W, int Cout);
int dffw_conv_cat_wgrad(int device, int precision, const void *xa, int Ca, const void *xb, int Cb, int B, int N, int H, int W, const void *grad_y,
                        int Cout, float *grad_w, void *workspace, int64_t workspace_bytes, void *hip_stream);
int dffw_op_conv_cat_backward(int device, int precision, const float *xa, int Ca, const float *xb, int Cb, int B, int N, int H, int W,
                              const float *weight, int Cout, const float *grad_y, float *grad_xa, float *grad_xb, float *grad_w, void *hip_stream);

typedef struct dffw_sim_params {
    double pixel_per_meter;
    double min_depth, max_depth;
    double min_focus, max_focus;
    int num_planes;
    int max_radius;
// ... 37 lines not shown
```

Before: 4100 stacks/s.

## Split final classifier score across deconv_3 and conv6 via linearity

```diff
diff --git a/dffinthewild_amd/csrc/dffw_device.h b/dffinthewild_amd/csrc/dffw_device.h
--- a/dffinthewild_amd/csrc/dffw_device.h
+++ b/dffinthewild_amd/csrc/dffw_device.h
@@ -403,7 +403,10 @@
     if (!a.cls_w) return;
     partial += __shfl_xor(partial, 16);
     if (rows == 4) partial += __shfl_xor(partial, 32);
-    if ((g & (rows - 1)) == 0 && pvalid) a.cls_out[opix] = partial;
+    if ((g & (rows - 1)) == 0 && pvalid) {
+        if (a.dbg & DFFW_ARGS_CLS_ACC) unsafeAtomicAdd(a.cls_out + opix, partial);
+        else a.cls_out[opix] = partial;
+    }
 }
 
 __device__ __forceinline__ float softplus_fast(float v) {
diff --git a/dffinthewild_amd/csrc/dffw_dispatch.cpp b/dffinthewild_amd/csrc/dffw_dispatch.cpp
--- a/dffinthewild_amd/csrc/dffw_dispatch.cpp
+++ b/dffinthewild_amd/csrc/dffw_dispatch.cpp
@@ -62,7 +62,8 @@
 
     double out_b(int k) const { return opx * L.cout * eb * k; }
     double w_b(double taps) const { return taps * L.cin * L.cout * eb; }
-    double cls_b() const { return o.cls ? opx * 4.0 : 0.0; }
+    double cls_b() const { return o.cls ? opx * (o.cls_acc ? 8.0 : 4.0) : 0.0; }
+    double cls_acc_b() const { return o.cls_acc ? opx * 8.0 : 0.0; }
     double sums_b() const { return opx / 16.0 * 3.0 * L.cout * 4.0; }
     double mac(double points, double taps) const { return 2.0 * points * taps * L.cin * L.cout; }
     int res(const Act *r) const { return r ? 1 : 0; }
@@ -85,7 +86,7 @@
         return g;
     }
     static ConvArgs masked(ConvArgs g) {
-        g.dbg &= (6 | DFFW_ARGS_NO_LEAN_TILE | DFFW_ARGS_NO_LEAN_ROLL | DFFW_ARGS_NO_ROLLX | DFFW_ARGS_NO_ROLLK | DFFW_ARGS_NO_SLICE32);
+        g.dbg &= (6 | DFFW_ARGS_CLS_ACC | DFFW_ARGS_NO_LEAN_TILE | DFFW_ARGS_NO_LEAN_ROLL | DFFW_ARGS_NO_ROLLX | DFFW_ARGS_NO_ROLLK | DFFW_ARGS_NO_SLICE32);
         return g;
     }
     int zsplit(int64_t units, int64_t below) const {
@@ -116,7 +117,7 @@
         const int64_t units = (int64_t)in0.B * c.n * std::max(1, L.cout / 32);
         const bool four = cin_pad == 32 && L.cout != 16;
         if (!(units >= (int64_t)sw.rollt_min_units * (four ? 3 : 2) / 2 && rollt_ok(prec, g))) return false;
-        p.clear_scores = g.cls_w != nullptr;
+        p.clear_scores = g.cls_w != nullptr && !o.cls_acc;
         add(p, g, pc.wrollt, c, 1, 0, mac((double)g.M, 27.0),
             in_b + out_b((o.discard ? 0 : 1) + (o.out_pre ? 1 : 0) + res(o.res0)) + cls_b() + w_b(27.0));
         return true;
@@ -349,7 +350,7 @@
     l.a = a;
     l.suffix = "";
     l.flops = flops;
-    l.bytes = in_b + (o.outf ? opx * L.cout * 4.0 : out_b(o.out_pre ? 2 : 1)) + out_b(res(o.res0) + res(o.res1)) + w_b((double)L.kd * L.kh * L.kw);
+    l.bytes = in_b + (o.outf ? opx * L.cout * 4.0 : out_b(o.out_pre ? 2 : 1)) + out_b(res(o.res0) + res(o.res1)) + cls_acc_b() + w_b((double)L.kd * L.kh * L.kw);
     if (p.stem_pipe) stem_pipe_kernel_name(a, l.kernel, sizeof l.kernel);
     else conv_tile_kernel_name(prec, cfg, a, t, l.kernel, sizeof l.kernel);
 }
@@ -382,7 +383,7 @@
         l.flops = 2.0 * (double)a.M * v.ntaps * L.cin * L.cout;
         l.bytes = in_b / nv
                   + px * L.cout * (o.outf ? 4.0 : eb * (o.out_pre ? 2 : 1))
-                  + px * L.cout * eb * (res(o.res0) + res(o.res1))
+                  + px * L.cout * eb * (res(o.res0) + res(o.res1)) + cls_acc_b() / nv
                   + (double)v.ntaps * L.cin * L.cout * eb;
     }
 }
@@ -396,6 +397,7 @@
         snprintf(p.msg, sizeof p.msg, fmt, x, y);
     };
     if (o.cls && (!cls || !cls->w32 || cls->def.cin != L.cout || cls->def.cout != 1)) return reject("cannot fuse classifier %s into %s", o.cls, name.c_str());
+    if (o.cls_acc && !(o.cls && o.cls_out)) return reject("layer %s: an accumulating classifier needs a classifier and its score volume%s", name.c_str(), "");
     if (o.res_bcast && !(L.kd == 1 && L.kh == 3 && !L.transposed && L.sh == 1 && L.cout >= 16))
         return reject("slice-broadcast residual is only implemented for the per-slice 1x3x3 convs (layer %s)%s", name.c_str(), "");
 
@@ -424,6 +426,7 @@
     a.cls_out = o.cls_out;
     a.relu = o.relu;
     a.dbg = (sw.debug_flags & 6) | sw.path_bits();
+    if (o.cls_acc) a.dbg |= DFFW_ARGS_CLS_ACC;
     if (o.raw) a.dbg |= DFFW_ARGS_RAW;
     if (o.sums) {
         if (!conv_sums_ok(pc, sw, in0.B, in0.N, in0.H, in0.W) || o.relu != 1 || o.res0 || o.res1 || o.cls || o.out_pre || o.in1)
@@ -455,6 +458,38 @@
     else pl.gather(p);
 }
 
+Act conv_out_geom(const LayerDef &L, const Act &in0) {
+    Act out;
+    if (L.transposed) {
+        out.H = in0.H * 2;
+        out.W = in0.W * 2;
+    } else {
+        const int win = (L.kh == 9 && L.cin == 3) ? in0.W - 2 : in0.W;
+        out.H = (in0.H + 2 * L.ph - L.dh * (L.kh - 1) - 1) / L.sh + 1;
+        out.W = (win + 2 * L.pw - L.dw * (L.kw - 1) - 1) / L.sw + 1;
+    }
+    out.B = in0.B;
+    out.N = in0.N + 2 * L.pd - (L.kd - 1);
+    out.C = L.cout;
+    return out;
+}
+
+}
+
+bool Run::conv_keeps_family(const std::string &name, const Act &in0, const ConvOpt &o, const ConvOpt &base, bool streaming) const {
+    const PackedConv *pc = layer(name);
+    if (!pc || in0.C + (o.in1 ? o.in1->C : 0) != pc->cin_all) return false;
+    Act out = conv_out_geom(pc->def, in0);
+    ConvPlan p[2];
+    const ConvOpt *opt[2] = {&o, &base};
+    for (int k = 0; k < 2; ++k) {
+        const PackedConv *cls = opt[k]->cls ? layer(opt[k]->cls) : nullptr;
+        out.p = (opt[k]->discard || opt[k]->outf || opt[k]->sums) ? nullptr : (uint16_t *)(uintptr_t)256;
+        plan_conv(name, *pc, cls, in0, *opt[k], out, sw, e->prec, p[k]);
+        if (p[k].err != DFFW_OK) return false;
+        if (k == 0 && streaming && p[0].family >= kStreamCount) return false;
+    }
+    return p[0].family == p[1].family && (p[0].family != F_GATHER || strcmp(p[0].l[0].kernel, p[1].l[0].kernel) == 0);
 }
 
 Act Run::conv(const std::string &name, const Act &in0, const ConvOpt &o) {
@@ -472,16 +507,8 @@
         err = fail(DFFW_EINVAL, "layer %s expects %d input channels, got %d", name.c_str(), pc.cin_all, cin);
         return out;
     }
-    int Ho, Wo;
-    if (L.transposed) {
-        Ho = in0.H * 2;
-        Wo = in0.W * 2;
-    } else {
-        const int win = (L.kh == 9 && L.cin == 3) ? in0.W - 2 : in0.W;
-        Ho = (in0.H + 2 * L.ph - L.dh * (L.kh - 1) - 1) / L.sh + 1;
-        Wo = (win + 2 * L.pw - L.dw * (L.kw - 1) - 1) / L.sw + 1;
-    }
-    const int No = in0.N + 2 * L.pd - (L.kd - 1);
+    const Act geom = conv_out_geom(L, in0);
+    const int No = geom.N, Ho = geom.H, Wo = geom.W;
     if (o.outf == nullptr && !o.discard && !o.sums) out = act(in0.B, No, Ho, Wo, L.cout);
     else { out.B = in0.B; out.N = No; out.H = Ho; out.W = Wo; out.C = L.cout; }
     if (o.out_pre) *o.out_pre = act(in0.B, No, Ho, Wo, L.cout);
diff --git a/dffinthewild_amd/csrc/dffw_engine.cpp b/dffinthewild_amd/csrc/dffw_engine.cpp
--- a/dffinthewild_amd/csrc/dffw_engine.cpp
+++ b/dffinthewild_amd/csrc/dffw_engine.cpp
@@ -451,7 +451,7 @@
 }
 
 static Act hourglass(Run &r, const std::string &p, const Act &xa, const Act &xb, const Act *presqu, const Act *postsqu,
-                     const Act &skip, Act *pre1_out, Act *out_raw, const std::string &cls, float *cls_out, bool discard_sum) {
+                     const Act &skip, Act *pre1_out, Act *out_raw, const std::string &cls, float *cls_out, bool discard_sum, bool skip_scored = false) {
     ConvOpt rl; rl.relu = 1;
     ConvOpt c0 = rl; c0.in1 = &xb;
     Act pre1 = r.conv(p + ".conv0.0.0", xa, c0);
@@ -465,7 +465,8 @@
     ConvOpt c5 = rl; c5.res0 = presqu ? presqu : &pre;
     Act o5 = r.conv(p + ".conv5.0", o4, c5);
     r.drop(o4); r.drop(pre);
-    ConvOpt c6; c6.res0 = &skip; c6.out_pre = out_raw; c6.cls = cls.c_str(); c6.cls_out = cls_out; c6.discard = discard_sum;
+    ConvOpt c6; c6.res0 = skip_scored ? nullptr : &skip; c6.out_pre = out_raw; c6.cls = cls.c_str(); c6.cls_out = cls_out; c6.discard = discard_sum;
+    c6.cls_acc = skip_scored;
     Act sum = r.conv(p + ".conv6.0", o5, c6);
     r.drop(o5);
     if (pre1_out) *pre1_out = pre1; else r.drop(pre1);
@@ -620,10 +621,32 @@
     r.tap_f32("cost2", cost2, (int64_t)B * N * h2 * w2);
     regress(r, rq, "regress.pred2", cost2, B, N, h2, w2, H, W, fd, fst, out[2], merge_heads);
 
-    Act x3 = r.conv(P + ".deconv_3.0", s2);
-    r.drop(s2);
-    float *cost3 = (float *)r.raw((int64_t)B * N * H * W * sizeof(float));
-    Act s3 = hourglass(r, P + ".dres4", x3, v1, &pre_b, &out_b, x3, nullptr, nullptr, P + ".classif3.0", cost3, true);
+    const std::string cls3 = P + ".classif3.0";
+    bool score_split = !r.sw.on(SW_NO_SCORE_SPLIT);
+    if (score_split) {
+        float *const some = (float *)(uintptr_t)256;
+        ConvOpt d3; d3.cls = cls3.c_str(); d3.cls_out = some;
+        Act o5 = s2;
+        Act skip; skip.B = B; skip.N = N; skip.H = H; skip.W = W; skip.C = 8; skip.p = (uint16_t *)(uintptr_t)256;
+        ConvOpt c6; c6.cls = cls3.c_str(); c6.cls_out = some; c6.discard = true;
+        ConvOpt c6s = c6; c6s.cls_acc = true;
+        c6.res0 = &skip;
+        score_split = r.conv_keeps_family(P + ".deconv_3.0", s2, d3, ConvOpt(), true) && r.conv_keeps_family(P + ".dres4.conv6.0", o5, c6s, c6, true);
+    }
+    float *cost3 = nullptr;
+    Act x3;
+    if (score_split) {
+        cost3 = (float *)r.raw((int64_t)B * N * H * W * sizeof(float));
+        ConvOpt d3; d3.cls = cls3.c_str(); d3.cls_out = cost3;
+        x3 = r.conv(P + ".deconv_3.0", s2, d3);
+        r.drop(s2);
+    } else {
+        x3 = r.conv(P + ".deconv_3.0", s2);
+        r.drop(s2);
+        cost3 = (float *)r.raw((int64_t)B * N * H * W * sizeof(float));
+    }
+    r.tap("x3", x3);
+    Act s3 = hourglass(r, P + ".dres4", x3, v1, &pre_b, &out_b, x3, nullptr, nullptr, cls3, cost3, true, score_split);
     r.drop(x3); r.drop(v1); r.drop(pre_b); r.drop(out_b);
     r.drop(s3);
     r.tap_f32("cost3", cost3, (int64_t)B * N * H * W);
diff --git a/dffinthewild_amd/csrc/dffw_internal.h b/dffinthewild_amd/csrc/dffw_internal.h
--- a/dffinthewild_amd/csrc/dffw_internal.h
+++ b/dffinthewild_amd/csrc/dffw_internal.h
@@ -40,6 +40,7 @@
 #define DFFW_ARGS_NO_ROLLX 256
 #define DFFW_ARGS_NO_SLICE32 1024
 #define DFFW_ARGS_NO_ROLLT 2048
+#define DFFW_ARGS_CLS_ACC 4096
 #define DFFW_ARGS_NO_ROLLK 512
 struct ConvArgs {
     const uint16_t *in0, *in1;
diff --git a/dffinthewild_amd/csrc/dffw_ops.cpp b/dffinthewild_amd/csrc/dffw_ops.cpp
--- a/dffinthewild_amd/csrc/dffw_ops.cpp
+++ b/dffinthewild_amd/csrc/dffw_ops.cpp
@@ -110,20 +110,11 @@
 
 }
 
-extern "C" {
-
-int dffw_op_conv3d(int device, int precision, const float *x, int B, int Cin, int N, int H, int W, const float *weight,
-                   int Cout, const int kernel[3], const int stride[3], const int pad[3], const int dilation[3], int transposed,
-                   const float *bn, const float *conv_bias, const float *residual, int relu, float *y, void *hip_stream) {
-    return dffw_op_conv3d_ex(device, precision, x, B, Cin, N, H, W, weight, Cout, kernel, stride, pad, dilation, transposed, bn, conv_bias, residual, relu, y,
-                             nullptr, nullptr, nullptr, hip_stream);
-}
-
-int dffw_op_conv3d_ex(int device, int precision, const float *x, int B, int Cin, int N, int H, int W, const float *weight,
-                      int Cout, const int kernel[3], const int stride[3], const int pad[3], const int dilation[3], int transposed,
-                      const float *bn, const float *conv_bias, const float *residual, int relu, float *y, float *y_pre, const float *cls_weight,
-                      float *cls_score, void *hip_stream) {
-    if (!x || !weight || !y || !kernel || !stride || !pad || !dilation) return fail(DFFW_EINVAL, "null argument");
+static int conv3d_op(int device, int precision, const float *x, int B, int Cin, int N, int H, int W, const float *weight,
+                     int Cout, const int kernel[3], const int stride[3], const int pad[3], const int dilation[3], int transposed,
+                     const float *bn, const float *conv_bias, const float *residual, int relu, float *y, float *y_pre, const float *cls_weight,
+                     float *cls_score, bool cls_acc, void *hip_stream) {
+    if (!x || !weight || (!y && !cls_acc) || !kernel || !stride || !pad || !dilation) return fail(DFFW_EINVAL, "null argument");
     if (precision < 0 || precision > 2) return fail(DFFW_EINVAL, "unknown precision %d", precision);
     if (stride[0] != 1 || dilation[0] != 1) return fail(DFFW_EINVAL, "slice stride/dilation must be 1");
     if (stride[1] != stride[2] || dilation[1] != dilation[2]) return fail(DFFW_EINVAL, "row/col stride and dilation must match");
@@ -182,13 +173,43 @@
         if (cls_weight) {
             o.cls = "cls";
             o.cls_out = (float *)r.raw(opix * sizeof(float));
+            o.cls_acc = cls_acc;
+            if (cls_acc && real(r)) r.check(hipMemcpyAsync(o.cls_out, cls_score, opix * sizeof(float), hipMemcpyDeviceToDevice, r.s), "copy");
         }
+        o.discard = !y;
         Act out = r.conv("op", in, o);
-        if (Cout == 1) copy_out(r, o.outf, y, opix);
-        else stage_out(r, out, y);
+        if (y && Cout == 1) copy_out(r, o.outf, y, opix);
+        else if (y) stage_out(r, out, y);
         if (y_pre) stage_out(r, pre, y_pre);
         if (cls_weight) copy_out(r, o.cls_out, cls_score, opix);
     });
+}
+
+extern "C" {
+
+int dffw_op_conv3d(int device, int precision, const float *x, int B, int Cin, int N, int H, int W, const float *weight,
+                   int Cout, const int kernel[3], const int stride[3], const int pad[3], const int dilation[3], int transposed,
+                   const float *bn, const float *conv_bias, const float *residual, int relu, float *y, void *hip_stream) {
+    return dffw_op_conv3d_ex(device, precision, x, B, Cin, N, H, W, weight, Cout, kernel, stride, pad, dilation, transposed, bn, conv_bias, residual, relu, y,
+                             nullptr, nullptr, nullptr, hip_stream);
+}
+
+int dffw_op_conv3d_ex(int device, int precision, const float *x, int B, int Cin, int N, int H, int W, const float *weight,
+                      int Cout, const int kernel[3], const int stride[3], const int pad[3], const int dilation[3], int transposed,
+                      const float *bn, const float *conv_bias, const float *residual, int relu, float *y, float *y_pre, const float *cls_weight,
+                      float *cls_score, void *hip_stream) {
+    if (!y) return fail(DFFW_EINVAL, "null argument");
+    return conv3d_op(device, precision, x, B, Cin, N, H, W, weight, Cout, kernel, stride, pad, dilation, transposed, bn, conv_bias, residual, relu, y, y_pre,
+                     cls_weight, cls_score, false, hip_stream);
+}
+
+int dffw_op_conv3d_cls_acc(int device, int precision, const float *x, int B, int Cin, int N, int H, int W, const float *weight,
+                           int Cout, const int kernel[3], const int stride[3], const int pad[3], const int dilation[3], int transposed,
+                           const float *bn, const float *conv_bias, const float *residual, int relu, float *y, const float *cls_weight,
+                           float *cls_score, void *hip_stream) {
+    if (!cls_weight || !cls_score) return fail(DFFW_EINVAL, "the accumulating classifier needs cls_weight and cls_score");
+    return conv3d_op(device, precision, x, B, Cin, N, H, W, weight, Cout, kernel, stride, pad, dilation, transposed, bn, conv_bias, residual, relu, y, nullptr,
+                     cls_weight, cls_score, true, hip_stream);
 }
 
 int dffw_op_pool(int device, int precision, int mode, int k, const float *x, int B, int C, int N, int H, int W, float *y,
diff --git a/dffinthewild_amd/csrc/dffw_run.h b/dffinthewild_amd/csrc/dffw_run.h
--- a/dffinthewild_amd/csrc/dffw_run.h
+++ b/dffinthewild_amd/csrc/dffw_run.h
@@ -134,7 +134,8 @@
     X(NO_CONCURRENT) X(NO_CONF_FORK) X(NO_FUSED_ATTENTION) X(NO_FUSED_EFD) X(NO_FUSED_OF) X(NO_FUSED_POOL) X(NO_FUSED_SRD) \
     X(NO_FUSED_STEM) X(NO_HEAD_SPLIT) X(NO_ROLL) X(NO_ROLL_S2) X(NO_SPLIT) X(NO_SPLITK)  \
     X(NO_STEM_PAIR) X(NO_TILE) X(NO_SMALL) X(NO_ROLL_S2_WIDE) X(NO_HEAD_SUMS) X(NO_HEAD_SUMS_FUSED) X(NO_HEAD_WARP) X(NO_OF_FIRST) \
-    X(NO_LEAN_TILE) X(NO_LEAN_ROLL) X(NO_ROLLX) X(NO_ROLLK) X(NO_ROLLT) X(NO_TEAMS) X(NO_SLICE32) X(NO_REGRESS_FUSED) X(NO_STEM_PIPE) X(NO_POOL3) X(NO_NARROW)
+    X(NO_LEAN_TILE) X(NO_LEAN_ROLL) X(NO_ROLLX) X(NO_ROLLK) X(NO_ROLLT) X(NO_TEAMS) X(NO_SLICE32) X(NO_REGRESS_FUSED) X(NO_STEM_PIPE) X(NO_POOL3) X(NO_NARROW) \
+    X(NO_SCORE_SPLIT)
 enum SwitchId {
 #define X_ID(n) SW_##n,
     DFFW_SWITCHES(X_ID)
@@ -262,6 +263,7 @@
     float *sums = nullptr;
     const char *cls = nullptr;
     float *cls_out = nullptr;
+    bool cls_acc = false;
     bool discard = false;
 };
 
@@ -474,6 +476,7 @@
     }
 
     Act conv(const std::string &name, const Act &in0, const ConvOpt &o = ConvOpt());
+    bool conv_keeps_family(const std::string &name, const Act &in0, const ConvOpt &o, const ConvOpt &base, bool streaming) const;
 
     Act pool(const Act &x, int mode, int k) {
         Act out = act(x.B, x.N, x.H / k, x.W / k, x.C);
diff --git a/dffinthewild_amd/engine.py b/dffinthewild_amd/engine.py
--- a/dffinthewild_amd/engine.py
+++ b/dffinthewild_amd/engine.py
@@ -78,6 +78,9 @@
     lib.dffw_op_conv3d_ex.argtypes = [c_int, c_int, c_void_p, c_int, c_int, c_int, c_int, c_int, POINTER(c_float), c_int,
                                       POINTER(c_int), POINTER(c_int), POINTER(c_int), POINTER(c_int), c_int,
                                       POINTER(c_float), POINTER(c_float), c_void_p, c_int, c_void_p, c_void_p, POINTER(c_float), c_void_p, c_void_p]
+    lib.dffw_op_conv3d_cls_acc.argtypes = [c_int, c_int, c_void_p, c_int, c_int, c_int, c_int, c_int, POINTER(c_float), c_int,
+                                           POINTER(c_int), POINTER(c_int), POINTER(c_int), POINTER(c_int), c_int,
+                                           POINTER(c_float), POINTER(c_float), c_void_p, c_int, c_void_p, POINTER(c_float), c_void_p, c_void_p]
     lib.dffw_op_pool.argtypes = [c_int, c_int, c_int, c_int, c_void_p, c_int, c_int, c_int, c_int, c_int, c_void_p, c_void_p]
     lib.dffw_op_srd.argtypes = [c_int, c_int, c_void_p, c_int, c_int, c_int, c_int, c_int] + [POINTER(c_float)] * 6 + [c_void_p] * 3
     lib.dffw_op_efd.argtypes = [c_int, c_int, c_void_p, c_int, c_int, c_int, c_int, c_int] + [POINTER(c_float)] * 4 + [c_int, c_void_p, c_void_p]
@@ -177,7 +180,7 @@
 ABI_SYMBOLS = (
     "dffw_version", "dffw_last_error", "dffw_param_count", "dffw_param_info", "dffw_engine_create",
     "dffw_engine_destroy", "dffw_engine_precision", "dffw_workspace_bytes", "dffw_forward",
-    "dffw_forward_taps", "dffw_profile_enable", "dffw_profile_collect", "dffw_op_conv3d", "dffw_op_conv3d_ex", "dffw_op_pool", "dffw_op_regress",
+    "dffw_forward_taps", "dffw_profile_enable", "dffw_profile_collect", "dffw_op_conv3d", "dffw_op_conv3d_ex", "dffw_op_conv3d_cls_acc", "dffw_op_pool", "dffw_op_regress",
     "dffw_op_regress_heads",
     "dffw_op_fov_warp", "dffw_forward_e2e", "dffw_last_conv_kernel", "dffw_op_srd", "dffw_op_efd", "dffw_last_op_kernels",
     "dffw_op_of_block", "dffw_op_head_tail",
@@ -375,6 +378,7 @@
         "E2": (B, 32, N, H // 4, W // 4), "V3": (B, 32, N, H // 4, W // 4),
         "FS_volume": (B, 32, N, H // 8, W // 8), "conf": (B, N, H // 8, W // 8),
         "cost1": (B, N, H // 4, W // 4), "cost2": (B, N, H // 2, W // 2), "cost3": (B, N, H, W),
+        "x3": (B, 8, N, H, W),
     }
 
 
@@ -416,6 +420,30 @@
             _check(lib.dffw_op_conv3d_ex(*args, _ptr(y_pre), _f32(cw) if cw is not None else None, _ptr(score), _stream_ptr(dev)), "dffw_op_conv3d_ex")
             return y, y_pre, score
         _check(lib.dffw_op_conv3d(*args, _stream_ptr(dev)), "dffw_op_conv3d")
+    return y
+
+
+def op_conv3d_cls_acc(x, weight, cls_weight, score, *, stride=1, pad=0, transposed=False, bn=None, bias=None, residual=None, relu=0,
+                      precision="bf16x3", want_y=True):
+    B, Cin, N, H, W = x.shape
+    w = weight.detach().to("cpu", torch.float32).contiguous()
+    Cout = w.shape[1] if transposed else w.shape[0]
+    k = tuple(w.shape[2:])
+    s, p, d = _i3(stride), _i3(pad), _i3(1)
+    shape = conv3d_output_shape(x.shape, w.shape, stride, pad, transposed)
+    if tuple(score.shape) != (B,) + tuple(shape[2:]) or score.dtype != torch.float32 or not score.is_contiguous():
+        raise ValueError("score must be a contiguous float32 tensor of shape %r" % ((B,) + tuple(shape[2:]),))
+    bnh = torch.cat([t.detach().to("cpu", torch.float32).reshape(-1) for t in bn]).contiguous() if bn is not None else None
+    bh = bias.detach().to("cpu", torch.float32).contiguous() if bias is not None else None
+    y = torch.empty(shape, dtype=torch.float32, device=x.device) if want_y else None
+    x = x.contiguous()
+    res = residual.contiguous() if residual is not None else None
+    cw = cls_weight.detach().to("cpu", torch.float32).reshape(-1).contiguous()
+    dev = _dev(x)
+    with torch.cuda.device(dev):
+        _check(lib.dffw_op_conv3d_cls_acc(dev, PRECISIONS[precision], _ptr(x), B, Cin, N, H, W, _f32(w), Cout, (c_int * 3)(*k), s, p, d, int(transposed),
+                                          _f32(bnh) if bnh is not None else None, _f32(bh) if bh is not None else None, _ptr(res), relu, _ptr(y),
+                                          _f32(cw), _ptr(score), _stream_ptr(dev)), "dffw_op_conv3d_cls_acc")
     return y
 
 
diff --git a/include/dffw.h b/include/dffw.h
--- a/include/dffw.h
+++ b/include/dffw.h
@@ -85,6 +85,12 @@
                       const int pad[3], const int dilation[3], int transposed, const float *bn,
                       const float *conv_bias, const float *residual, int relu, float *y, float *y_pre,
                       const float *cls_weight, float *cls_score, void *hip_stream);
+
+int dffw_op_conv3d_cls_acc(int device, int precision, const float *x, int B, int Cin, int N, int H, int W,
+                           const float *weight, int Cout, const int kernel[3], const int stride[3],
+                           const int pad[3], const int dilation[3], int transposed, const float *bn,
+                           const float *conv_bias, const float *residual, int relu, float *y,
+                           const float *cls_weight, float *cls_score, void *hip_stream);
 
 int dffw_op_pool(int device, int precision, int mode, int k, const float *x, int B, int C, int N,
                  int H, int W, float *y, void *hip_stream);
```

Measured after the change: 4111 stacks/s, median of 6. Within noise of the previous version (+0.3%).
